# Geunwoo-Jeon/LarvaNet

Hardware: AMD Instinct MI355X
Metric: HR Mpixels/s (LarvaNet x4 multi-exit train step, 48x48 LR patches) (higher is better)
Workload: dtype f32; 1 GPU; LarvaNet x4 train_step_larva M4 B4,4,4,4 48ch, batch 16 of 3x48x48 -> 3x192x192 fp32 per GPU (BASELINE config 2); global_batch=16, parallelism=dp1, hip_graph=True

## Files before the change

### include/larva_hip.h

```cpp
#ifndef LARVA_HIP_H
#define LARVA_HIP_H

#include <stdint.h>

#ifdef __cplusplus
extern "C" {
#endif

int larva_abi_version(void);
const char* larva_error_string(int code);

long long larva_packed_weight_floats(int cout, int cin);
int larva_pack_weights(const float* w, float* wpk_fwd, float* wpk_bwd, int cout, int cin,
                       int w_cin_total, int w_cin_off, void* stream);

int larva_pack_weights_batch(const float* const* w, float* const* wpk_fwd, float* const* wpk_bwd,
                             const int* cout, const int* cin, const int* w_cin_total,
                             const int* w_cin_off, int njobs, void* stream);

int larva_step_prologue(const float* const* w, float* const* wpk_fwd, float* const* wpk_bwd, const int* cout,
                        const int* cin, const int* w_cin_total, const int* w_cin_off, int njobs, const float* x,
                        float* x16, float* base, int N, int C, int H, int W, void* stream);

int larva_conv3x3_fwd(const float* const* src, int n_src, int cin_per_src, const float* wpk,
                      const float* bias, const float* res0, const float* res1, const float* mask,
                      const float* base, float* out, int N, int cout, int H, int W, int relu,
                      int mode, void* stream);

int larva_conv3x3_fwd_pitched(const float* const* src, int n_src, int cin_per_src, const float* wpk,
                              const float* bias, const float* res0, const float* res1, const float* mask,
                              const float* base, float* out, int N, int cout, int H, int W, int pitch,
                              int relu, int mode, void* stream);

int larva_conv3x3_fwd_batch(int njobs, const float* const* src, int n_src, int cin_per_src,
                            const float* const* wpk, const float* const* bias, const float* const* res0,
                            const float* const* res1, const float* const* mask, const float* const* base,
                            float* const* out, int N, int cout, int H, int W, int pitch, int relu, int mode,
                            void* stream);

int larva_head_conv3_direct(const float* x, const float* w, const float* bias, float* out, int N, int cout,
                            int H, int W, int pitch, void* stream);

int larva_exit_l1_partials(int N, int H, int pitch);
int larva_conv3x3_exit_l1_batch(int njobs, const float* const* src, int n_src, int cin_per_src,
                                const float* const* wpk, const float* const* bias, const float* const* base,
                                const float* const* truth, float* const* out, float* const* grad,
                                float* const* partial, float gval, int N, int cout, int H, int W, int pitch,
                                void* stream);

int larva_strip_tile_table(int H, int W, int phase, unsigned* tab, int cap);
int larva_conv3x3_fwd_strips(const float* const* src, int n_src, int cin_per_src, const float* wpk,
                             const float* bias, const float* res0, const float* res1, const float* mask,
                             const float* base, float* out, int N, int cout, int H, int W, int pitch,
                             int relu, int mode, const unsigned* tile_tab, const unsigned* tile_tab_host,
                             int tiles_per_image, int plain_stores, void* stream);

int larva_conv3x3_fwd_tiled(const float* const* src, int n_src, int cin_per_src, const float* wpk,
                            const float* bias, const float* res0, const float* res1, const float* mask,
                            const float* base, float* out, int N, int cout, int H, int W, int pitch,
                            int relu, int mode, int tile_rows, void* stream);

long long larva_wgrad_partial_floats(int cout, int cin, int splits);
int larva_wgrad_cu_share(int cout, int cin);
int larva_conv3x3_wgrad(const float* const* dy, const float* const* x, float* const* partial,
                        float* const* dw, float* const* db, const int* cin_off,
                        const int* cin_valid, const int* w_cin_total, int njobs, int splits,
                        int N, int cout, int cin, int H, int W, void* stream);

int larva_wgrad_flat_max_splits(int njobs, int nwg, int tiles_per_layer);
int larva_conv3x3_wgrad_partial_flat(const float* const* dy, const float* const* x, float* const* partial,
                                     int njobs, int nwg, int N, int cout, int cin, int H, int W,
                                     int* splits_out, void* stream);
int larva_wgrad_flat_head_splits(int njobs, int nwg, int tiles_per_layer);
int larva_conv3x3_wgrad_partial_flat_head(const float* const* dy, const float* const* x, float* const* partial,
                                          int njobs, const float* head_dy, const float* head_x16, float* head_partial,
                                          int nwg, int N, int H, int W, int* splits_out, int* head_splits_out,
                                          void* stream);

int larva_conv3x3_wgrad_partial(const float* const* dy, const float* const* x, float* const* partial,
                                int njobs, int splits, int N, int cout, int cin, int H, int W,
                                int* splits_used, void* stream);
int larva_wgrad_reduce(const float* const* partial, float* const* dw, float* const* db,
                       const int* cin_off, const int* cin_valid, const int* w_cin_total,
                       const int* splits, const int* cout, const int* cin, int njobs, void* stream);

int larva_wgrad_reduce_with_loss(const float* const* partial, float* const* dw, float* const* db,
                                 const int* cin_off, const int* cin_valid, const int* w_cin_total,
                                 const int* splits, const int* cout, const int* cin, int njobs,
                                 const float* const* terms, const int* count, const float* scale, int nterms,
                                 float divisor, float* loss_out, void* stream);

int larva_bicubic4_fwd(const float* in, float* out, int N, int C, int H, int W, void* stream);
int larva_upsample4_fwd(const float* in, float* out, int N, int C, int H, int W, int mode, void* stream);

int larva_l1_workspace_floats(void);
int larva_l1_fwd(const float* a, const float* b, long long numel, float* partial, float* loss,
                 void* stream);
int larva_l1_bwd(const float* a, const float* b, const float* gout, long long numel, float* ga,
                 void* stream);
int larva_l1_bwd_unshuffle4(const float* a, const float* b, const float* gout, float gscale, float* ga, int N,
                            int C, int H, int W, void* stream);
int larva_sum_scalars(const float* const* terms, int n, float divisor, float* out, void* stream);
int larva_l1_partial(const float* a, const float* b, long long numel, float* partial, int* blocks_out,
                     void* stream);
int larva_loss_from_partials(const float* const* terms, const int* count, const float* scale, int n,
                             float divisor, float* out, void* stream);
int larva_loss_from_partials_to_host(const float* const* terms, const int* count, const float* scale, int n,
                                     float divisor, float* out, float* host_cell, void* stream);
int larva_loss_from_partials_to_host_seq(const float* const* terms, const int* count, const float* scale, int n,
                                         float divisor, float* out, float* host_cell, unsigned* dev_seq, void* stream);
int larva_host_cell_alloc(float** cell);
int larva_host_cell_free(float* cell);
int larva_l1_partial_grad(const float* a, const float* b, float gvalue, float gscale, float* partial,
                          int* blocks_out, float* grad, int N, int C, int H, int W, void* stream);
int larva_l1_partial_grad_batch(const float* const* a, const float* b, int n, float gvalue, float gscale,
                                float* const* partial, int* blocks_out, float* const* grad, int N, int C, int H,
                                int W, void* stream);

int larva_pixel_unshuffle4(const float* in, float* out, int N, int C, int H, int W, void* stream);

int larva_upsample_fwd(const float* in, float* out, int N, int C, int H, int W, int scale, int mode, void* stream);
int larva_pixel_shuffle_base(const float* y, const float* base, float* out, int N, int C, int cpad, int H, int W,
                             int pitch, int scale, void* stream);
int larva_pixel_unshuffle(const float* in, float* out, int N, int C, int cpad, int H, int W, int scale, void* stream);
int larva_l1_bwd_unshuffle(const float* a, const float* b, const float* gout, float gscale, float* ga, int N, int C,
                           int cpad, int H, int W, int scale, void* stream);
int larva_shuffle_l1_partial_grad(const float* y, const float* base, const float* truth, float gvalue, float gscale,
                                  float* partial, int* blocks_out, float* grad, float* out, int N, int C, int cpad, int H,
                                  int W, int scale, void* stream);

int larva_adamw_step(float* p, const float* g, float* m, float* v, const float* step_lr,
                     double beta1, double beta2, double eps, double weight_decay, float grad_scale,
                     long long n, void* stream);

int larva_adamw_step_host(float* p, const float* g, float* m, float* v, int step, double lr, double beta1,
                          double beta2, double eps, double weight_decay, float grad_scale, long long n,
                          void* stream);
int larva_adamw_step_host_copy(float* p, const float* g, float* m, float* v, int step, double lr, double beta1,
                               double beta2, double eps, double weight_decay, float grad_scale, long long n,
                               const float* copy_src, float* copy_dst, void* stream);

int larva_gather_patches(const unsigned char* data, const long long* offsets, const int* hw,
                         const int* draws, float* out, int B, int P, int mult, void* stream);

int larva_sqerr_u8(const float* out, const unsigned char* truth, int C, int H, int W, int TH, int TW,
                   unsigned long long* acc, void* stream);

int larva_u8_hwc_to_f32_chw(const unsigned char* in, float* out, int N, int H, int W, void* stream);
int larva_f32_chw_to_u8_hwc(const float* in, unsigned char* out, int N, int H, int W, void* stream);

long long larva_u8_metrics_workspace_bytes(int h, int w, int mode);
int larva_u8_metrics(const unsigned char* out, long long out_pitch, const unsigned char* truth, long long truth_pitch,
                     int y0, int x0, int h, int w, int mode, int want_ssim, void* workspace,
                     unsigned long long* result, void* stream);

long long larva_f16_packed_weight_halves(int cout, int cin);
int larva_f16_pack_weights(const float* w, uint16_t* wpk, int cout, int cin, void* stream);

int larva_f16_head(const float* x, const float* w, const float* bias, uint16_t* out, unsigned* flag, int N, int H,
                   int W, void* stream);

int larva_f16_conv3x3(const uint16_t* const* srcs, int nsrc, const uint16_t* wpk, const float* bias,
                      const uint16_t* res0, const uint16_t* res1, int relu, uint16_t* out, unsigned* flag, int N, int H,
                      int W, void* stream);

int larva_f16_conv3x3_shuffle_base(const uint16_t* src, const uint16_t* wpk, const float* bias, const float* base,
                                   float* out, int N, int H, int W, void* stream);

int larva_f16_conv3x3_shuffle_base_u8(const uint16_t* src, const uint16_t* wpk, const float* bias, const float* base,
                                      unsigned char* out, unsigned* flag, int N, int H, int W, void* stream);

int larva_dihedral_inputs_u8(const unsigned char* in, float* a, float* b, int N, int H, int W, void* stream);
int larva_dihedral_inputs_f32(const float* in, float* a, float* b, int N, int H, int W, void* stream);
int larva_dihedral_mean(const float* a, const float* b, float* out_f32, unsigned char* out_u8, int N, int H, int W,
                        void* stream);

#ifdef __cplusplus
}
#endif
#endif
```

### larvanet_amd/autograd.py

```python
import contextlib
import os

import numpy as np
import torch

from . import kernels as K

_WGRAD_WORKGROUPS = 256


class PaddedWidth:

    current = None

    def __init__(self, w):
        self.w = int(w)

    def __enter__(self):
        self._prev = PaddedWidth.current
        PaddedWidth.current = self.w
        return self

    def __exit__(self, *exc):
        PaddedWidth.current = self._prev
# ... 266 lines not shown
    def intact(self, module=None):
        return all(p.grad is view for p, view in self._pairs)

    def span(self, tensors):
        base = self.flat.data_ptr()
        lo, hi = self.flat.numel(), 0
        for t in tensors:
            off = (t.data_ptr() - base) // 4
            if off < 0 or off + t.numel() > self.flat.numel():
                return None
            lo, hi = min(lo, off), max(hi, off + t.numel())
        return (lo, hi) if hi > lo else None


def _targets(pc):
    if pc is not None and pc.grad_inplace and pc.weight.grad is not None and pc.bias.grad is not None:
        return pc.weight.grad, pc.bias.grad
    return None, None


def _splits(njobs, cout=48, cin=48):
    return max(1, _WGRAD_WORKGROUPS * K.wgrad_cu_share(cout, cin) // njobs)


class DeferredWgrad:

    active = False
    jobs_per_launch = 32
    _pending = {}

    @classmethod
    def push(cls, cout, cin, jobs):
        cls._pending.setdefault((cout, cin), []).extend(jobs)

    _late = []

    @classmethod
    def _launches(cls, split=False):
        pending, cls._pending = cls._pending, {}
        cap = max(1, min(cls.jobs_per_launch, K.max_wgrad_jobs())) if split else K.max_wgrad_jobs()
        out = []
        for (cout, cin), jobs in pending.items():
            jobs = sorted(jobs, key=lambda j: -j["dw"].data_ptr())
            out += [(cout, cin, jobs[i:i + cap]) for i in range(0, len(jobs), cap)]
        out.sort(key=lambda l: -max(j["dw"].data_ptr() for j in l[2]))
        return out

    pending_loss = None

    @classmethod
    def finish_loss(cls):
        job, cls.pending_loss = cls.pending_loss, None
        if job is not None:
            terms, scales, divisor, out = job
            out.copy_(K.loss_from_partials(terms, scales, divisor))

    @staticmethod
    def _issue(launches):
        reduce_jobs = []
        head = host = None
        heads = [l for l in launches if (l[0], l[1]) == (48, 16) and len(l[2]) == 1]
        hosts = [l for l in launches if (l[0], l[1]) == (48, 48)]
        if len(heads) == 1 and hosts and hosts[-1][2][0]["dy"].shape == heads[0][2][0]["dy"].shape:
            head, host = heads[0], hosts[-1]
        todo = [l for l in launches if l is not head]
        for launch in todo:
            cout, cin, chunk = launch
            extra = head[2][0] if launch is host else None
            res = K.conv3x3_wgrad_partial_flat(chunk, cout, cin, _WGRAD_WORKGROUPS, head=extra)
            if res is None and extra is not None:
                todo.append(head)
                extra = None
            if res is not None:
                reduce_jobs += [dict(j, partial=p, splits=s, cout=cout, cin=cin) for j, p, s in zip(chunk, *res)]
                if extra is not None:
                    reduce_jobs.append(dict(extra, partial=res[0][-1], splits=res[1][-1], cout=48, cin=16))
                continue
            parts, used = K.conv3x3_wgrad_partial(chunk, cout, cin, _splits(len(chunk), cout, cin))
            reduce_jobs += [dict(j, partial=p, splits=used, cout=cout, cin=cin) for j, p in zip(chunk, parts)]
        for i in range(0, len(reduce_jobs), 64):
            last = i + 64 >= len(reduce_jobs)
            loss, DeferredWgrad.pending_loss = (DeferredWgrad.pending_loss, None) if last else (None, DeferredWgrad.pending_loss)
            K.wgrad_reduce(reduce_jobs[i:i + 64], loss=loss)

    @classmethod
    def flush(cls, split=False):
        launches = cls._launches(split)
        n_early = max(1, len(launches) // 2) if split else len(launches)
        cls._issue(launches[:n_early])
        cls._late = launches[n_early:]
        if not split:
            return None
        return [t for _, _, chunk in launches[:n_early] for j in chunk for t in (j["dw"], j["db"]) if t is not None]

    @classmethod
    def has_late(cls):
        return bool(cls._late)

    @classmethod
    def late_targets(cls):
        return [t for _, _, chunk in cls._late for j in chunk for t in (j["dw"], j["db"]) if t is not None]

    @classmethod
    def flush_late(cls):
        late, cls._late = cls._late, []
        cls._issue(late)

    @classmethod
    def drop(cls):
        cls._pending = {}
        cls._late = []
        cls.pending_loss = None


class StepScope:

    depth = 0
    _padded = {}
    seed_grad = None
    early_loss = False

    @classmethod
    def padded_input(cls, shape, device):
        if cls.depth == 0:
            return torch.zeros(shape, device=device, dtype=torch.float32)
        key = (tuple(shape), str(device))
        buf = cls._padded.get(key)
        if buf is None:
            buf = cls._padded[key] = torch.zeros(shape, device=device, dtype=torch.float32)
        return buf

    def __init__(self, defer_wgrad=True, split_flush=False, joint_input_grads=True,
                 seed_grad=None, dual_chain=False, lazy_chain_joins=(False, False), early_loss=False):
        self.seed_grad_value = seed_grad
        self.early_loss_value = early_loss or False
        self.dual_chain = dual_chain
        self.lazy_chain_joins = lazy_chain_joins
        self.defer_wgrad = defer_wgrad
        self.split_flush = split_flush
        self.joint_input_grads = joint_input_grads
        self.early_targets = None

    def __enter__(self):
        gpu = torch.cuda.is_available()
        DeferredWgrad.active = bool(self.defer_wgrad) and gpu
        DeferredWgrad.drop()
        JointInputGrad.active = bool(self.joint_input_grads) and gpu
        JointInputGrad.reset()
        DualChain.enabled = bool(self.dual_chain) and gpu
        DualChain.lazy_fwd, DualChain.lazy_bwd = (bool(v) and DualChain.enabled for v in self.lazy_chain_joins)
        StepScope.depth += 1
        StepScope.seed_grad = self.seed_grad_value
        StepScope.early_loss = self.early_loss_value
        return self

    def __exit__(self, exc_type, *exc):
        try:
            DualChain.join()
            if exc_type is None:
                self.early_targets = DeferredWgrad.flush(split=self.split_flush)
                DeferredWgrad.finish_loss()
            else:
                DeferredWgrad.drop()
            if exc_type is None and JointInputGrad._parked:
                raise RuntimeError("larvanet_amd: an exit parked its input gradient but the next body never ran backward")
        finally:
            DualChain.reset()
            StepScope.depth -= 1
            StepScope.seed_grad = None
            StepScope.early_loss = False
            DeferredWgrad._pending = {}
            DualChain.enabled = DualChain.lazy_fwd = DualChain.lazy_bwd = False
            DeferredWgrad.active = False
            JointInputGrad.active = False
            JointInputGrad.reset()
        return False


def _wgrad(jobs, cout, cin, inplace=False):
    defer = inplace and DeferredWgrad.active
    out, batch = [], []
    for job in jobs:
        (dy, x, wshape, cin_off, cin_valid, dw_shared) = job[:6]
        db_shared = job[6] if len(job) > 6 else None
        dw = dw_shared if dw_shared is not None else torch.empty(wshape, device=dy.device, dtype=torch.float32)
        if db_shared is not None or not defer:
            db = db_shared if db_shared is not None else torch.empty((cout,), device=dy.device,
                                                                     dtype=torch.float32)
        else:
            db = None
        batch.append({"dy": dy, "x": x, "dw": dw, "db": db, "cin_off": cin_off, "cin_valid": cin_valid})
        out.append((dw, db))
    if defer:
        DeferredWgrad.push(cout, cin, batch)
        batch = []
    for i in range(0, len(batch), 16):
        chunk = batch[i:i + 16]
        K.conv3x3_wgrad(chunk, cout, cin, _splits(len(chunk), cout, cin))
    return out


LARGE_INFERENCE_PIXELS = 100000


def is_large_inference(n, h, w):
    return int(n) * int(h) * int(w) > LARGE_INFERENCE_PIXELS


def _head_direct_setting():
    v = os.environ.get("LARVA_HEAD_DIRECT", "auto")
    if v not in ("auto", "0", "1"):
        raise RuntimeError("larvanet_amd: LARVA_HEAD_DIRECT=%r (auto, 0 or 1)" % v)
    return {"0": False, "1": True}.get(v, "auto")


class HeadFn(torch.autograd.Function):

    direct = _head_direct_setting()
    rule_batch = None

    @staticmethod
    @contextlib.contextmanager
    def rule_batch_as(n):
        before, HeadFn.rule_batch = HeadFn.rule_batch, int(n)
        try:
            yield
        finally:
            HeadFn.rule_batch = before

    @staticmethod
    def forward(ctx, x, weight, bias, pc, x16=None, training=True):
        N, C, H, W = x.shape
        P = PaddedWidth.pitch_of(W) if _lw() is not None else W
        cout = int(weight.shape[0])
        training = bool(training) and bool(ctx.needs_input_grad[1] or ctx.needs_input_grad[2])
        want = HeadFn.direct if HeadFn.direct != "auto" else (not training and is_large_inference(HeadFn.rule_batch or N, H, W))
        use_direct = want and C == 3 and cout % 16 == 0
        if x16 is not None:
            pass
        elif training or not use_direct:
            x16 = StepScope.padded_input((N, 16, H, P), x.device)
            x16[:, :C, :, :W] = x
        if use_direct:
            out = K.head_conv3_direct(x, weight.detach(), bias.detach(), pitch=P)
        else:
            (fwd, _), = pc.get()
            out = DualChain.conv(x16, fwd, cout, forward=True, bias=bias.detach(), logical_w=_lw())
            DualChain.end_of_node(False)
        if x16 is not None:
            ctx.save_for_backward(x16)
        ctx.wshape = tuple(weight.shape)
        ctx.pc = pc
        return out

    @staticmethod
    def backward(ctx, dy):
        (x16,) = ctx.saved_tensors
        dy = dy.contiguous()
        cout, cin = ctx.wshape[0], ctx.wshape[1]
        tw, tb = _targets(ctx.pc)
        if not (tw is not None and DeferredWgrad.active):
            DualChain.join()
        (dw, db), = _wgrad([(dy, x16, ctx.wshape, 0, cin, tw, tb)], cout, 16, inplace=tw is not None)
        if tw is not None:
            return None, None, None, None, None, None
        return None, dw, db, None, None, None


class BodyFn(torch.autograd.Function):

    @staticmethod
    def forward(ctx, x, pcs, *params):
        nb = len(params) // 4
        keep = [x]
        fea = x
        for j in range(nb):
            w1, b1, w2, b2 = params[4 * j:4 * j + 4]
            (f1, _), = pcs[2 * j].get()
            (f2, _), = pcs[2 * j + 1].get()
            c = int(w1.shape[0])
            h = DualChain.conv(fea, f1, c, forward=True, bias=b1.detach(), relu=True, logical_w=_lw())
            if j == nb - 1:
                nxt = DualChain.conv(h, f2, c, forward=True, bias=b2.detach(), res0=fea, res1=x, logical_w=_lw())
            else:
                nxt = DualChain.conv(h, f2, c, forward=True, bias=b2.detach(), res0=fea, logical_w=_lw())
            keep.append(h)
            if j < nb - 1:
                keep.append(nxt)
            fea = nxt
        DualChain.end_of_node(False)
        ctx.save_for_backward(*keep)
        ctx.pcs = pcs
        ctx.nb = nb
        ctx.wshape = tuple(params[0].shape)
        return fea

    @staticmethod
    def backward(ctx, dy):
        nb, pcs = ctx.nb, ctx.pcs
        keep = ctx.saved_tensors[:2 * nb]
        dy = dy.contiguous()
        c = ctx.wshape[0]
        g = dy
        jobs = [None] * (2 * nb)
        dx = None
        for j in reversed(range(nb)):
            fea_j = keep[0] if j == 0 else keep[2 * j]
            h_j = keep[2 * j + 1]
            (_, bw1), = pcs[2 * j].get()
            (_, bw2), = pcs[2 * j + 1].get()
            dh = DualChain.conv(g, bw2, c, mask=h_j)
            jobs[2 * j + 1] = (g, h_j, ctx.wshape, 0, c) + _targets(pcs[2 * j + 1])
            jobs[2 * j] = (dh, fea_j, ctx.wshape, 0, c) + _targets(pcs[2 * j])
            if j > 0:
                g = DualChain.conv(dh, bw1, c, res0=g)
            else:
                dh_leg = JointInputGrad.take(keep[0], pcs[0])
                if dh_leg is None:
                    dx = DualChain.conv(dh, bw1, c, res0=g, res1=dy)
                else:
                    dx = DualChain.conv([dh, dh_leg], pcs[0].joint.arena(dh.device), c, res0=g, res1=dy)
        inplace = all(_targets(pc)[0] is not None for pc in pcs)
        if not (inplace and DeferredWgrad.active):
            DualChain.join()
        DualChain.end_of_node(True)
        grads = _wgrad(jobs, c, c, inplace=inplace)
        flat = []
        for pc, (dw, db) in zip(pcs, grads):
            flat += [None, None] if _targets(pc)[0] is not None else [dw, db]
        return (dx, None) + tuple(flat)


def _leg_forward(fea, base, pcs, params, scale, lw=None):
    w1, b1, w2, b2 = params
    (f1, _), = pcs[0].get()
    (f2, _), = pcs[1].get()
    h = K.conv3x3(fea, f1, int(w1.shape[0]), bias=b1.detach(), relu=True, logical_w=lw)
    if scale == 4:
        return h, K.conv3x3(h, f2, int(w2.shape[0]), bias=b2.detach(), shuffle=True, base=base, logical_w=lw)
    return h, K.conv3x3(h, f2, pcs[1].cout_pad, bias=pcs[1].padded_bias(), logical_w=lw)


def _leg_backward(ctx, fea, h, dyl):
    pcs = ctx.pcs
    c = ctx.wshape[0]
    (_, bw1), = pcs[0].get()
    (_, bw2), = pcs[1].get()
    dh = K.conv3x3(dyl, bw2, c, mask=h)
    dfea = K.conv3x3(dh, bw1, c)
    first = [(dh, fea, ctx.wshape, 0, c) + _targets(pcs[0])]
    if ctx.scale == 4:
        ((dw1, db1),), ((dw2, db2),) = _leg_wgrad(first, [(dyl, h, ctx.wshape2, 0, c) + _targets(pcs[1])], c, ctx.wshape2[0])
        if _targets(pcs[1])[0] is not None:
            dw2 = db2 = None
    else:
        ((dw1, db1),) = _wgrad(first, c, c, inplace=_targets(pcs[0])[0] is not None)
        dw2, db2 = padded_wgrad(dyl, h, pcs[1], ctx.wshape2)
    if _targets(pcs[0])[0] is not None:
        dw1 = db1 = None
    return dfea, dw1, db1, dw2, db2


def _leg_wgrad(first, second, c, c2):
    inplace = all(j[5] is not None for j in list(first) + list(second))
    if c2 == c:
        res = _wgrad([j for pair in zip(first, second) for j in pair], c, c, inplace=inplace)
        return res[0::2], res[1::2]
    return _wgrad(list(first), c, c, inplace=inplace), _wgrad(list(second), c2, c, inplace=inplace)


def padded_wgrad(dyl, h, pc, wshape):
    cp, cin, rows = pc.cout_pad, int(wshape[1]), int(wshape[0])
    dw = torch.empty((cp,) + tuple(wshape[1:]), device=dyl.device, dtype=torch.float32)
    db = torch.empty((cp,), device=dyl.device, dtype=torch.float32)
    K.conv3x3_wgrad([{"dy": dyl, "x": h, "dw": dw, "db": db, "cin_off": 0, "cin_valid": cin}], cp, cin,
                    _splits(1, cp, cin))
    tw, tb = _targets(pc)
    if tw is None:
        return dw[:rows], db[:rows]
    tw.copy_(dw[:rows])
    tb.copy_(db[:rows])
    return None, None


class LegFn(torch.autograd.Function):

    @staticmethod
    def forward(ctx, fea, base, pcs, scale, w1, b1, w2, b2):
        h, y = _leg_forward(fea, base, pcs, (w1, b1, w2, b2), scale, _lw())
        out = y if scale == 4 else K.pixel_shuffle_base(y, base, scale, logical_w=_lw())
        ctx.save_for_backward(fea, h)
        ctx.pcs, ctx.scale = pcs, scale
        ctx.wshape, ctx.wshape2 = tuple(w1.shape), tuple(w2.shape)
        return out

    @staticmethod
    def backward(ctx, dout):
        fea, h = ctx.saved_tensors
        dout = dout.contiguous()
        dyl = K.pixel_unshuffle4(dout) if ctx.scale == 4 else K.pixel_unshuffle(dout, ctx.scale, ctx.pcs[1].cout_pad)
        dfea, *dparams = _leg_backward(ctx, fea, h, dyl)
        return (dfea, None, None, None) + tuple(dparams)


class ExitFn(torch.autograd.Function):

    @staticmethod
    def forward(ctx, fea, base, truth, pcs, scale, divisor, w1, b1, w2, b2):
        h, y = _leg_forward(fea, base, pcs, (w1, b1, w2, b2), scale)
        ctx.gscale = 1.0 if divisor is None else float(np.float32(1.0) / np.float32(divisor))
        dyl = None
        fused = divisor is not None and StepScope.seed_grad is not None
        if scale == 4:
            out = y
            if fused:
                term, _, dyl = K.l1_partial_grad(out, truth, StepScope.seed_grad, ctx.gscale)
        elif fused:
            term, _, dyl, out = K.shuffle_l1_partial_grad(y, base, truth, StepScope.seed_grad, ctx.gscale, scale)
        else:
            out = K.pixel_shuffle_base(y, base, scale)
        if dyl is None:
            term = K.l1_fwd(out, truth) if divisor is None else K.l1_partial(out, truth)[0]
        ctx.have_dyl = dyl is not None
        ctx.save_for_backward(fea, h, *((dyl,) if dyl is not None else (out, truth)))
        ctx.pcs, ctx.scale = pcs, scale
        ctx.wshape, ctx.wshape2 = tuple(w1.shape), tuple(w2.shape)
        ctx.mark_non_differentiable(out)
        ctx.set_materialize_grads(False)
        return out, term

    @staticmethod
    def backward(ctx, _dout, gterm):
        if gterm is None:
            return (None,) * 10
        saved = ctx.saved_tensors
        fea, h = saved[:2]
        if ctx.have_dyl:
            dyl = saved[2]
        else:
            g0 = gterm.as_strided((), ()) if gterm.dim() else gterm.contiguous()
            out, truth = saved[2:4]
            dyl = K.l1_bwd_unshuffle4(out, truth, g0, ctx.gscale) if ctx.scale == 4 else \
                K.l1_bwd_unshuffle(out, truth, g0, ctx.scale, ctx.pcs[1].cout_pad, ctx.gscale)
        dfea, *dparams = _leg_backward(ctx, fea, h, dyl)
        return (dfea, None, None, None, None, None) + tuple(dparams)


def _conv_group(jobs, cout, **kw):
    outs = []
    for i in range(0, len(jobs), 4):
        chunk = jobs[i:i + 4]
        if len(chunk) == 1:
            j = chunk[0]
            outs.append(K.conv3x3(j["srcs"], j["wpk"], cout, bias=j.get("bias"), mask=j.get("mask"), base=j.get("base"),
                                  res0=j.get("res0"), res1=j.get("res1"), **kw))
        else:
            outs += K.conv3x3_batch(chunk, cout, **kw)
    return outs


class ExitsFn(torch.autograd.Function):

    @staticmethod
    def forward(ctx, base, truth, legs, divisor, *args):
        M = len(legs)
        feas, params = args[:M], args[M:]
        c = int(params[0].shape[0])
        c2 = int(params[2].shape[0])
        hs = _conv_group([{"srcs": feas[i], "wpk": legs[i][0].get()[0][0], "bias": params[4 * i + 1].detach()}
                          for i in range(M)], c, relu=True)
        ctx.gscale = float(np.float32(1.0) / np.float32(divisor))
        ctx.have_dyl = StepScope.seed_grad is not None
        shuffle_jobs = [{"srcs": hs[i], "wpk": legs[i][1].get()[0][0], "bias": params[4 * i + 3].detach(), "base": base}
                        for i in range(M)]
        outs, parts, third = [None] * M, [None] * M, [None] * M
        fused = ctx.have_dyl
        if fused:
            i = 0
            while i < M and fused:
                n = 3 if M - i == 5 else min(4, M - i)
                res = K.conv3x3_exit_l1_batch(shuffle_jobs[i:i + n], c2, truth, StepScope.seed_grad, ctx.gscale,
                                              [i + k == M - 1 for k in range(n)]) if n > 1 else None
                if res is None:
                    fused = False
                else:
                    outs[i:i + n], parts[i:i + n], third[i:i + n] = res
                    i += n
        if not fused:
            outs = _conv_group(shuffle_jobs, c2, shuffle=True)
            parts, third = [], []
            if ctx.have_dyl:
                for i in range(0, M, 8):
                    p8, _, g8 = K.l1_partial_grad_batch(outs[i:i + 8], truth, StepScope.seed_grad, ctx.gscale)
                    parts += p8
                    third += g8
            else:
                for out in outs:
                    part, _ = K.l1_partial(out, truth)
                    parts.append(part)
                    third.append(out)
        ctx.save_for_backward(truth, *feas, *hs, *third)
        ctx.legs, ctx.M = legs, M
        ctx.wshape, ctx.wshape2 = tuple(params[0].shape), tuple(params[2].shape)
        ctx.mark_non_differentiable(outs[-1])
        ctx.set_materialize_grads(False)
        return (outs[-1],) + tuple(parts)

    @staticmethod
    def backward(ctx, _dout, *gterms):
        M, legs = ctx.M, ctx.legs
        saved = ctx.saved_tensors
        truth, feas, hs, third = saved[0], saved[1:1 + M], saved[1 + M:1 + 2 * M], saved[1 + 2 * M:1 + 3 * M]
        c = ctx.wshape[0]
        live = [i for i in range(M) if gterms[i] is not None]
        dyls = {}
        for i in live:
            if ctx.have_dyl:
                dyls[i] = third[i]
            else:
                g0 = gterms[i].as_strided((), ())
                dyls[i] = K.l1_bwd_unshuffle4(third[i], truth, g0, ctx.gscale)
        dhs = dict(zip(live, _conv_group([{"srcs": dyls[i], "wpk": legs[i][1].get()[0][1], "mask": hs[i]} for i in live], c))) if live else {}
        dfeas = [None] * M
        grads = [None] * (4 * M)
        jobs1, jobs2 = [], []
        for i in live:
            pc1, pc2 = legs[i]
            if JointInputGrad.can_park(pc1):
                JointInputGrad.park(feas[i], dhs[i], pc1)
            else:
                dfeas[i] = DualChain.conv(dhs[i], pc1.get()[0][1], c)
            jobs1.append((dhs[i], feas[i], ctx.wshape, 0, c) + _targets(pc1))
            jobs2.append((dyls[i], hs[i], ctx.wshape2, 0, c) + _targets(pc2))
        DualChain.end_of_node(True)
        for which, res in enumerate(_leg_wgrad(jobs1, jobs2, c, ctx.wshape2[0]) if jobs1 else ()):
            for i, (dw, db) in zip(live, res):
                if _targets(legs[i][which])[0] is None:
                    grads[4 * i + 2 * which], grads[4 * i + 2 * which + 1] = dw, db
        return (None, None, None, None) + tuple(dfeas) + tuple(grads)


class LossTerm:

    __slots__ = ("tensor", "scale", "prescaled")

    def __init__(self, tensor, scale=1.0, prescaled=False):
        self.tensor, self.scale, self.prescaled = tensor, float(scale), bool(prescaled)


class MeanTermsFn(torch.autograd.Function):

    @staticmethod
    def forward(ctx, meta, *tensors):
        ctx.meta = meta
        ctx.shapes = [tuple(t.shape) for t in tensors]
        ts, scales = [t.contiguous() for t in tensors], [m[0] for m in meta]
        if (len(ts) <= 8 and DeferredWgrad.active and StepScope.depth > 0 and not StepScope.early_loss
                and DeferredWgrad.pending_loss is None):
            out = torch.empty((), device=ts[0].device, dtype=torch.float32)
            DeferredWgrad.pending_loss = (ts, scales, float(len(ts)), out)
            return out
        cell = StepScope.early_loss if isinstance(StepScope.early_loss, K.HostCell) else None
        if len(ts) <= 8:
            return K.loss_from_partials(ts, scales, float(len(ts)), host_cell=cell)
        groups = [K.loss_from_partials(ts[i:i + 8], scales[i:i + 8], 1.0) for i in range(0, len(ts), 8)]
        return K.loss_from_partials(groups, [1.0] * len(groups), float(len(ts)), host_cell=cell)

    @staticmethod
    def backward(ctx, g):
        n = len(ctx.meta)
        gm = None
        grads = []
        for (scale, prescaled), shape in zip(ctx.meta, ctx.shapes):
            if prescaled:
                grads.append(g.expand(shape))
            else:
                gm = g / n if gm is None else gm
                grads.append(gm if scale == 1.0 else gm * scale)
        return (None,) + tuple(grads)


def mean_of_terms(terms):
    terms = [t if isinstance(t, LossTerm) else LossTerm(t) for t in terms]
    return MeanTermsFn.apply([(t.scale, t.prescaled) for t in terms], *[t.tensor for t in terms])


class MergeFn(torch.autograd.Function):

    @staticmethod
    def forward(ctx, pc, weight, bias, *feats):
        packs = pc.get()
        cout = int(weight.shape[0])
        out = K.conv3x3(list(feats), packs[0][0], cout, bias=bias.detach(), logical_w=_lw())
        ctx.save_for_backward(*feats)
        ctx.pc = pc
        ctx.wshape = tuple(weight.shape)
        return out

    @staticmethod
    def backward(ctx, dy):
        feats = ctx.saved_tensors
        packs = ctx.pc.get()
        dy = dy.contiguous()
        cout = ctx.wshape[0]
        c = int(feats[0].shape[1])
        dfeats = [K.conv3x3(dy, packs[1 + i][1], c) for i in range(len(feats))]
        tw, tb = _targets(ctx.pc)
        dw = tw if tw is not None else torch.empty(ctx.wshape, device=dy.device, dtype=torch.float32)
        jobs = [(dy, f, ctx.wshape, i * c, c, dw, tb if i == 0 else None) for i, f in enumerate(feats)]
        res = _wgrad(jobs, cout, c, inplace=tw is not None)
        db = res[0][1]
        if tw is not None:
            return (None, None, None) + tuple(dfeats)
        return (None, dw, db) + tuple(dfeats)


class L1LossFn(torch.autograd.Function):

    @staticmethod
    def forward(ctx, out, truth):
        out = out.contiguous()
        truth = truth.contiguous()
        ctx.save_for_backward(out, truth)
        return K.l1_fwd(out, truth)

    @staticmethod
    def backward(ctx, g):
        out, truth = ctx.saved_tensors
        return K.l1_bwd(out, truth, g.contiguous()), None
```

### larvanet_amd/captured_step.py

```python
import contextlib

import torch

from .autograd import DeferredWgrad, DualChain


class LossCopy:

    def __init__(self):
        self.host = torch.empty((), dtype=torch.float32).pin_memory()
        self.stream = torch.cuda.Stream()
        self.done, self.fwd_done = torch.cuda.Event(), torch.cuda.Event()

    def start(self, loss):
        self.fwd_done.record()
        with torch.cuda.stream(self.stream):
            self.stream.wait_event(self.fwd_done)
            self.host.copy_(loss, non_blocking=True)
            self.done.record()

    def result(self):
        self.done.synchronize()
        return self.host.item()


class CapturedStep:

    def __init__(self, plugin, key, mode, handoff, input_tensor, truth_tensor):
        x, truth = input_tensor.clone(), truth_tensor.clone()
        side = torch.cuda.Stream()
        side.wait_stream(torch.cuda.current_stream())
        with torch.cuda.stream(side):
            for _ in range(2):
                plugin._zero_grad()
                plugin._step_body(x, truth)
                DeferredWgrad.flush_late()
        torch.cuda.current_stream().wait_stream(side)
        plugin._zero_grad()
        graph = torch.cuda.CUDAGraph()
        back = torch.cuda.CUDAGraph() if mode == "split" else None
        with contextlib.ExitStack() as capturing:
            capturing.enter_context(torch.cuda.graph(graph, capture_error_mode="thread_local"))

            def cut():
                DualChain.join()
                capturing.close()
                capturing.enter_context(torch.cuda.graph(back, pool=graph.pool(), capture_error_mode="thread_local"))
            loss, out, early_lo = plugin._step_body(x, truth, early_loss=handoff if mode == "poll" else bool(mode),
                                                    cut=cut if back is not None else None)
        late = None
        if DeferredWgrad.has_late():
            late = torch.cuda.CUDAGraph()
            with torch.cuda.graph(late, pool=graph.pool(), capture_error_mode="thread_local"):
                DeferredWgrad.flush_late()
        self.key, self.mode, self.handoff = key, mode, handoff
        self.static_in, self.static_truth = x, truth
        self.graph, self.back, self.late = graph, back, late
        self.loss, self.out, self.early_lo = loss, out, early_lo

    def stage(self, input_tensor, truth_tensor):
        for dst, src in ((self.static_in, input_tensor), (self.static_truth, truth_tensor)):
            if src.data_ptr() != dst.data_ptr():
                dst.copy_(src)

    def replay(self):
        if self.mode == "poll":
            self.handoff.expect()
        self.graph.replay()
        if self.back is not None:
            self.handoff.start(self.loss)
            self.back.replay()
        return self.loss, self.out, self.late.replay if self.late is not None else None

    def buffers(self, input_shape, truth_shape):
        fits = tuple(self.static_in.shape) == tuple(input_shape) and tuple(self.static_truth.shape) == tuple(truth_shape)
        return (self.static_in, self.static_truth) if fits else None
```

### larvanet_amd/csrc/conv3x3_mfma.hip

```cpp
#include "larva_common.h"
#include "larva_bicubic.h"
#include <hip/hip_ext.h>
#include <cstdlib>
#include <type_traits>

#ifndef LARVA_DIAG
#define LARVA_DIAG 0
#endif
constexpr int kWgPerCu = 2;
constexpr int kOperandDepth = 2;


#ifndef LARVA_DIAG_ONLY48
#define LARVA_DIAG_ONLY48 0
#endif

namespace larva {

#if defined(LARVA_DIAG) && (LARVA_DIAG & 32)
__device__ unsigned long long* g_stamps = nullptr;
#if LARVA_DIAG & 512
constexpr int kDiagWgPerSlot = 256;
__device__ int g_slot_of_launch = 0;
__device__ __forceinline__ void stamp_slot(unsigned long long* area, int k) {
  if (!area || threadIdx.x != 0 || blockIdx.x >= kDiagWgPerSlot) return;
  const int idx = k == 0 ? 0 : k == 2 ? 1 : k == 3 ? 2 : k == 5 ? 3
                  : !(LARVA_DIAG & 2048) ? -1 : k == 6 ? 5 : k == 7 ? 6 : k == 14 ? 7 : k == 15 ? 8 : k == 1 ? 9 : -1;
  if (idx < 0) return;
  unsigned long long* p = area + (size_t)blockIdx.x * 16;
  p[idx] = __builtin_amdgcn_s_memrealtime();
  if (k == 0) {
    const unsigned hw = __builtin_amdgcn_s_getreg((31 << 11) | 4);
    const unsigned xcc = __builtin_amdgcn_s_getreg((31 << 11) | 20);
    p[4] = (unsigned long long)hw | ((unsigned long long)xcc << 32);
  }
}
#define stamp(k) stamp_slot(a.diag_area, (k))
#else
__device__ __forceinline__ void stamp(int k) {
  if (g_stamps && threadIdx.x == 0)
    g_stamps[blockIdx.x * 16 + k] = (LARVA_DIAG & 64) ? __builtin_amdgcn_s_memtime() : __builtin_amdgcn_s_memrealtime();
}
#endif
#else
__device__ __forceinline__ void stamp(int) {}
#endif

constexpr int kCh = 8;

template <int ROWS_, int COLS_>
struct TileGeo {
  static constexpr int ROWS = ROWS_, COLS = COLS_;
  static constexpr int HALO = ROWS + 2;
  static constexpr int PC = COLS / 16;
  static constexpr int RS = COLS + 8;
  static constexpr int PS = ((HALO * RS + 15) / 32) * 32 + 16;
  static_assert(COLS % 16 == 0 && PS >= HALO * RS && PS % 32 == 16, "tile geometry");
};
using GeoWide = TileGeo<kTileRows, kTileCols>;
using GeoWide4 = TileGeo<4, kTileCols>;
using GeoS5 = TileGeo<5, 16>;
using GeoS4 = TileGeo<4, 16>;
static_assert(GeoWide::RS == kRS && GeoWide::PS == 304, "the 3 x 48 tile of larva_common.h");

struct ConvArgs {
  const float* src[kMaxSrc];
  const float* wpk;
  const float* bias;
  const float* res0;
  const float* res1;
  const float* mask;
  const float* base;
  float* out;
  int cin_per_src;
  int n_chunks;
  int N, H, W;
  int pitch;
  int tiles_x, tiles_y;
  int nwg;
  const unsigned* tile_tab;
  const float* truth;
  float* grad;
  float* partial;
  int plain_stores;
  int tab_n;
  alignas(64) int tab16[32];
  float gval;
  unsigned long long magic_tx, magic_ty, magic_cps;
#if LARVA_DIAG & 512
  unsigned long long* diag_area;
#endif
};

__host__ __device__ __forceinline__ unsigned long long div_magic(int d) { return ((1ull << 40) + d - 1) / (unsigned)d; }
__device__ __forceinline__ int div_by_magic(int n, unsigned long long magic) {
  return (int)(((unsigned long long)(unsigned)n * magic) >> 40);
}

enum Epi : int {
  kEpiPlain = 0,
  kEpiRelu = 1,
  kEpiMask = 2,
  kEpiRes1 = 3,
  kEpiRes2 = 4,
  kEpiShuffle = 5,
  kEpiShuffleBase = 6,
  kEpiShuffleL1 = 7,
  kEpiCount = 8
};

template <int COUT, typename G = GeoWide>
struct ConvCfg {
  static constexpr int CT = COUT / 16;
  static constexpr int CS = cout_stride(COUT);
  static constexpr int PS = G::PS;
  static constexpr int IN_PIECES = (kCh * PS + 255) / 256;
  static constexpr int IN_FLOATS = IN_PIECES * 256;
  static constexpr int IN_SLOTS_PER_PLANE = PS / 4;
  static constexpr int W_USED = 9 * kCh * CS;
  static constexpr int W_PIECES = (W_USED + 255) / 256;
  static constexpr int W_FLOATS = W_PIECES * 256;
  static constexpr int PIECES = IN_PIECES + W_PIECES;
  static constexpr int NPW = (PIECES + 3) / 4;
  static constexpr int STAGE_FLOATS = IN_FLOATS + W_FLOATS;
  static constexpr int STEPS = 9 * (kCh / 4);
  static constexpr int NST = 3;
  static constexpr int AHEAD = NST - 1;
  static constexpr size_t LDS_BYTES_DMA = NST * STAGE_FLOATS * sizeof(float);
  static constexpr bool LOADER = 2 * PIECES <= 63;
  static constexpr int THREADS_DMA = LOADER ? 320 : 256;
  static constexpr size_t LDS_BYTES_REG = 2 * STAGE_FLOATS * sizeof(float);
  static constexpr int RIN_SLOTS = kCh * G::HALO * (G::RS / 4);
  static constexpr int RIN_ITERS = (RIN_SLOTS + 255) / 256;
  static constexpr int RW_SLOTS = W_USED / 4;
  static constexpr int RW_ITERS = (RW_SLOTS + 255) / 256;
  static_assert(kCh * PS <= IN_FLOATS, "input planes must fit their pieces");
};

template <int COUT, typename G>
struct DmaPlan {
  unsigned voff[ConvCfg<COUT, G>::NPW];
};

template <int COUT, typename G, bool WEIGHTS>
__device__ __forceinline__ void make_plan(const ConvArgs& a, int wave, int lane, int y0, int x0,
                                          DmaPlan<COUT, G>& pl) {
  using C = ConvCfg<COUT, G>;
#pragma unroll
  for (int i = 0; i < C::NPW; ++i) {
    const int p = min(wave + 4 * i, C::PIECES - 1);
    const bool isw = p >= C::IN_PIECES;
    if constexpr (WEIGHTS) {
      if (4 * i + 3 < C::IN_PIECES) continue;
      const int ws = (p - C::IN_PIECES) * 64 + lane;
// ... 90 lines not shown
    const int nstage = (stage + C::AHEAD) % C::NST;
    const unsigned dst = lds_addr_of(smem + nstage * C::STAGE_FLOATS);
    const ChunkSrc cs = chunk_src<COUT, G>(a, min(chunk + C::AHEAD, last), n);
#pragma unroll
    for (int p = 0; p < C::PIECES; ++p)
      lds_dma16_buf(p < C::IN_PIECES ? cs.img : cs.wgt, pl.voff[p], 0, dst + 1024u * (unsigned)p);
    stage = stage == C::NST - 1 ? 0 : stage + 1;
  }
  asm volatile("s_waitcnt vmcnt(0)" ::: "memory");
}

template <int COUT, typename G>
struct RegStaging {
  f32x4 in[ConvCfg<COUT, G>::RIN_ITERS];
  f32x4 w[ConvCfg<COUT, G>::RW_ITERS];
};

template <int COUT, typename G>
__device__ __forceinline__ void reg_load(const ConvArgs& a, const ChunkSrc& cs, int y0, int x0, int tid,
                                         RegStaging<COUT, G>& st) {
  using C = ConvCfg<COUT, G>;
  const size_t plane = (size_t)a.H * a.pitch;
#pragma unroll
  for (int i = 0; i < C::RIN_ITERS; ++i) {
    const int s = min(tid + i * 256, C::RIN_SLOTS - 1);
    const int ci = s / (G::HALO * (G::RS / 4));
    const int rem = s - ci * (G::HALO * (G::RS / 4));
    const int r = rem / (G::RS / 4);
    const int q = rem - r * (G::RS / 4);
    const int gy = y0 - 1 + r, gx = x0 - 4 + 4 * q;
    const bool row_ok = gy >= 0 && gy < a.H;
    const float* row = cs.img_ptr + (size_t)ci * plane + (size_t)min(max(gy, 0), a.H - 1) * a.pitch;
    f32x4 v;
#pragma unroll
    for (int e = 0; e < 4; ++e) {
      const int x = gx + e;
      const float t = row[min(max(x, 0), a.W - 1)];
      v[e] = (row_ok && x >= 0 && x < a.W) ? t : 0.f;
    }
    st.in[i] = v;
  }
#pragma unroll
  for (int i = 0; i < C::RW_ITERS; ++i) {
    const int s = min(tid + i * 256, C::RW_SLOTS - 1);
    const float* p = cs.wgt_ptr + 4 * s;
    st.w[i] = f32x4{p[0], p[1], p[2], p[3]};
  }
}

template <int COUT, typename G>
__device__ __forceinline__ void reg_store(float* stage, int tid, const RegStaging<COUT, G>& st) {
  using C = ConvCfg<COUT, G>;
#pragma unroll
  for (int i = 0; i < C::RIN_ITERS; ++i) {
    const int s = tid + i * 256;
    if (s < C::RIN_SLOTS) {
      const int ci = s / (G::HALO * (G::RS / 4));
      const int rem = s - ci * (G::HALO * (G::RS / 4));
      const int r = rem / (G::RS / 4);
      const int q = rem - r * (G::RS / 4);
      *reinterpret_cast<f32x4*>(stage + ci * C::PS + r * G::RS + 4 * q) = st.in[i];
    }
  }
#pragma unroll
  for (int i = 0; i < C::RW_ITERS; ++i) {
    const int s = tid + i * 256;
    if (s < C::RW_SLOTS) *reinterpret_cast<f32x4*>(stage + C::IN_FLOATS + 4 * s) = st.w[i];
  }
}

template <int COUT, typename G, int NCT, int PG0, int NPG>
__device__ __forceinline__ void read_operands(const float* const (&a_base)[NCT], const float* b_base, int step,
                                              float (&av)[NCT], float (&bv)[NPG]) {
  using C = ConvCfg<COUT, G>;
  if constexpr ((LARVA_DIAG & 128) != 0) {
#pragma unroll
    for (int c = 0; c < NCT; ++c) av[c] = (float)step;
#pragma unroll
    for (int p = 0; p < NPG; ++p) bv[p] = (float)(step + p);
    return;
  }
  const int tap = step / (kCh / 4), kk = step % (kCh / 4);
  const int ky = tap / 3, kx = tap % 3;
#pragma unroll
  for (int c = 0; c < NCT; ++c) av[c] = a_base[c][(tap * kCh + kk * 4) * C::CS];
#pragma unroll
  for (int p = 0; p < NPG; ++p) {
    const int pg = PG0 + p, prow = pg / G::PC, pcol = pg % G::PC;
    bv[p] = b_base[kk * 4 * C::PS + (prow + ky) * G::RS + pcol * 16 + kx];
  }
}

template <int NMF, int NRD, int M>
__device__ __forceinline__ void shadow_groups() {
  if constexpr (M < NMF) {
    __builtin_amdgcn_sched_group_barrier(0x8, 1, 0);
    constexpr int share = (NRD + NMF - 1 - M) / NMF;
    if constexpr (share > 0) __builtin_amdgcn_sched_group_barrier(0x100, share, 0);
    shadow_groups<NMF, NRD, M + 1>();
  }
}

template <int COUT, typename G, int NCT, int PG0, int NPG, bool SWAP>
__device__ __forceinline__ void mfma_chunk(const float* stage, int ct0, int lane, f32x4 (&acc)[NCT][NPG],
                                           const float* wstage = nullptr) {
  using C = ConvCfg<COUT, G>;
  const int lr = lane & 15, lq = lane >> 4;
  const float* const wrows = wstage ? wstage : stage + C::IN_FLOATS;
  const float* a_base[NCT];
#pragma unroll
  for (int c = 0; c < NCT; ++c)
    a_base[c] = wrows + lq * C::CS + lr + (cout_swizzled(COUT) ? (((ct0 + c) ^ (lq & 1)) * 16) : (ct0 + c) * 16);
  const float* b_base = stage + lq * C::PS + lr + 3;
  constexpr int D = kOperandDepth;
  float av[D + 1][NCT], bv[D + 1][NPG];
#pragma unroll
  for (int d = 0; d < D; ++d)
    if (d < C::STEPS) read_operands<COUT, G, NCT, PG0, NPG>(a_base, b_base, d, av[d], bv[d]);
#pragma unroll
  for (int step = 0; step < C::STEPS; ++step) {
    __builtin_amdgcn_sched_barrier(0);
    if (step + D < C::STEPS)
      read_operands<COUT, G, NCT, PG0, NPG>(a_base, b_base, step + D, av[(step + D) % (D + 1)], bv[(step + D) % (D + 1)]);
    constexpr int NMF = NCT * NPG;
    constexpr int NRD = NCT + NPG;
#pragma unroll
    for (int m = 0; m < NMF; ++m) {
      const float wv = av[step % (D + 1)][m / NPG], xv = bv[step % (D + 1)][m % NPG];
      acc[m / NPG][m % NPG] = __builtin_amdgcn_mfma_f32_16x16x4f32(SWAP ? xv : wv, SWAP ? wv : xv, acc[m / NPG][m % NPG], 0, 0, 0);
    }
    shadow_groups<NMF, NRD, 0>();
    __builtin_amdgcn_sched_barrier(0);
  }
}

template <int KEEP, int PIECES, int AUX>
__device__ __forceinline__ void wait_and_barrier() {
  static_assert(KEEP == PIECES + AUX, "a ring wait keeps exactly the next chunk's pieces and the operand loads in flight");
  asm volatile("; LARVA_RING pieces=%1 aux=%2\n\ts_waitcnt vmcnt(%0)\n\ts_barrier" ::"n"(KEEP), "n"(PIECES), "n"(AUX) : "memory");
  __builtin_amdgcn_sched_barrier(0);
}

template <typename G>
__device__ __forceinline__ void decode_tile(const ConvArgs& a, int vb, int& n, int& y0, int& x0) {
  const int tile = xcd_remap(vb, a.nwg);
  const int t2 = div_by_magic(tile, a.magic_tx);
  const int tx = tile - t2 * a.tiles_x;
  n = div_by_magic(t2, a.magic_ty);
  const int ty = t2 - n * a.tiles_y;
  x0 = tx * G::COLS;
  y0 = ty * G::ROWS;
}

template <int COUT, typename G, bool VEC, int EPI, int NCT, int PG0, int NPG, bool PERSIST = false>
__device__ __forceinline__ void run_role(const ConvArgs& a, float* smem, int ct0, int wave, int n, int y0, int x0, int tid) {
  using C = ConvCfg<COUT, G>;
  static_assert(!VEC || C::LOADER, "the 16-byte path runs with a loader wave (2 * PIECES <= 63 for every instantiated shape)");
  static_assert(!PERSIST || VEC, "persistent tiles: the loader-wave path");
  const int lane = tid & 63;
  const int lr = lane & 15, lq = lane >> 4;
  float* const out_ptr = a.out;
  struct { int H, W, pitch, plain; } k = {a.H, a.W, a.pitch, a.plain_stores};
  asm volatile("" : "+s"(k.H), "+s"(k.W), "+s"(k.pitch), "+s"(k.plain));

  constexpr bool kShuffleEpi = (EPI == kEpiShuffle || EPI == kEpiShuffleBase || EPI == kEpiShuffleL1);
  constexpr bool kPixMajor = VEC && !kShuffleEpi;
  f32x4 bias[NCT];
#pragma unroll
  for (int c = 0; c < NCT; ++c) bias[c] = f32x4{0.f, 0.f, 0.f, 0.f};
  auto load_bias = [&]() {
    if (a.bias) {
#pragma unroll
      for (int c = 0; c < NCT; ++c)
#pragma unroll
        for (int r = 0; r < 4; ++r) bias[c][r] = a.bias[(ct0 + c) * 16 + (kPixMajor ? lr : lq * 4 + r)];
    }
  };

  constexpr int NAUX = (EPI == kEpiMask || EPI == kEpiRes1 || EPI == kEpiShuffleBase)
                           ? 1 : ((EPI == kEpiRes2 || EPI == kEpiShuffleL1) ? 2 : 0);
  f32x4 aux[NAUX > 0 ? NAUX : 1][NAUX > 0 ? NCT : 1][NAUX > 0 ? NPG : 1];
  constexpr int NU = NCT * NPG;
  constexpr int kEarlyPairs = PERSIST && COUT == 48 ? (NAUX * NU < 7 ? NAUX * NU : 7) : NAUX * NU;
  constexpr int kLatePart = 4, kEarlyAll = 5;
  auto load_aux = [&](int part = -1) {
#pragma unroll
    for (int c = 0; c < NCT; ++c)
#pragma unroll
      for (int p = 0; p < NPG; ++p) {
        const int pg = PG0 + p, prow = pg / G::PC, pcol = pg % G::PC;
        const int y = min(y0 + prow, a.H - 1), x = min(x0 + pcol * 16 + lr, a.W - 1);
        auto want = [&](int op) {
          const int q = op * NU + c * NPG + p;
          return part < 0 ? true : part == kLatePart ? q >= kEarlyPairs : q < kEarlyPairs;
        };
        if constexpr (kShuffleEpi) {
          const int HH = 4 * a.H, WW = 4 * a.W;
          const size_t idx = (((size_t)n * C::CT + (ct0 + c)) * HH + (4 * y + lq)) * WW + 4 * x;
          if (want(0)) aux[0][c][p] = *reinterpret_cast<const f32x4*>(a.base + idx);
          if constexpr (EPI == kEpiShuffleL1) {
            if (want(1)) aux[1][c][p] = *reinterpret_cast<const f32x4*>(a.truth + idx);
          }
        } else if constexpr (kPixMajor && (PERSIST || G::COLS == 16)) {
          const unsigned plane = (unsigned)a.H * (unsigned)a.pitch;
          const unsigned lane_off = 4u * ((unsigned)lr * plane + (unsigned)lq * 4u);
          const int soff = __builtin_amdgcn_readfirstlane(
              (int)(4u * ((unsigned)((ct0 + c) * 16) * plane + (unsigned)(y0 + prow) * (unsigned)a.pitch + (unsigned)(x0 + pcol * 16))));
          auto image = [&](const float* t) {
            const unsigned long long b = reinterpret_cast<unsigned long long>(t + (size_t)n * COUT * plane);
            const unsigned lo = (unsigned)__builtin_amdgcn_readfirstlane((int)(unsigned)b);
            const unsigned hi = (unsigned)__builtin_amdgcn_readfirstlane((int)(unsigned)(b >> 32));
            return __builtin_amdgcn_make_buffer_rsrc(reinterpret_cast<void*>(((unsigned long long)hi << 32) | lo), 0,
                                                     (int)(COUT * plane * 4u), 0x00020000);
          };
          if constexpr (EPI == kEpiMask) {
            if (want(0)) aux[0][c][p] = __builtin_bit_cast(f32x4, __builtin_amdgcn_raw_buffer_load_b128(image(a.mask), lane_off, soff, 0));
          }
          if constexpr (EPI == kEpiRes1 || EPI == kEpiRes2) {
            if (want(0)) aux[0][c][p] = __builtin_bit_cast(f32x4, __builtin_amdgcn_raw_buffer_load_b128(image(a.res0), lane_off, soff, 0));
          }
          if constexpr (EPI == kEpiRes2) {
            if (want(1)) aux[1][c][p] = __builtin_bit_cast(f32x4, __builtin_amdgcn_raw_buffer_load_b128(image(a.res1), lane_off, soff, 0));
          }
        } else if constexpr (kPixMajor) {
          const size_t plane = (size_t)a.H * a.pitch;
          const int xb = min(x0 + pcol * 16 + lq * 4, a.pitch - 4);
          const size_t idx = ((size_t)n * COUT + (ct0 + c) * 16 + lr) * plane + (size_t)y * a.pitch + xb;
          if constexpr (EPI == kEpiMask) {
            if (want(0)) aux[0][c][p] = *reinterpret_cast<const f32x4*>(a.mask + idx);
          }
          if constexpr (EPI == kEpiRes1 || EPI == kEpiRes2) {
            if (want(0)) aux[0][c][p] = *reinterpret_cast<const f32x4*>(a.res0 + idx);
          }
          if constexpr (EPI == kEpiRes2) {
            if (want(1)) aux[1][c][p] = *reinterpret_cast<const f32x4*>(a.res1 + idx);
          }
        } else {
          const size_t plane = (size_t)a.H * a.pitch;
          const size_t idx0 = ((size_t)n * COUT + (ct0 + c) * 16 + lq * 4) * plane + (size_t)y * a.pitch + x;
#pragma unroll
          for (int r = 0; r < 4; ++r) {
            if constexpr (EPI == kEpiMask) aux[0][c][p][r] = a.mask[idx0 + r * plane];
            if constexpr (EPI == kEpiRes1 || EPI == kEpiRes2) aux[0][c][p][r] = a.res0[idx0 + r * plane];
            if constexpr (EPI == kEpiRes2) aux[1][c][p][r] = a.res1[idx0 + r * plane];
          }
        }
      }
  };
  constexpr bool kAuxLate = VEC && !kShuffleEpi && !(LARVA_DIAG & 6) && NAUX > 0 && !PERSIST;
  constexpr int kAuxLoads = kAuxLate ? NAUX * NCT * NPG : 0;
  auto load_early = [&]() {
    load_bias();
    if constexpr (NAUX > 0 && !kAuxLate && !(LARVA_DIAG & 4)) load_aux();
  };
  int pstage = 0;
  for (int vb = blockIdx.x;; vb += gridDim.x) {
  if constexpr (PERSIST) {
    if (vb >= a.nwg) break;
    decode_tile<G>(a, vb, n, y0, x0);
  }
  if constexpr (!VEC || (LARVA_DIAG & 2)) load_early();

  f32x4 acc[NCT][NPG];
#pragma unroll
  for (int c = 0; c < NCT; ++c)
#pragma unroll
    for (int p = 0; p < NPG; ++p) acc[c][p] = f32x4{0.f, 0.f, 0.f, 0.f};

  if constexpr (PERSIST) {
    load_bias();
    const int my_chunk = a.n_chunks >= 4 ? (wave & 3) : 0;
    __builtin_amdgcn_sched_barrier(0);
    for (int chunk = 0; chunk < a.n_chunks; ++chunk) {
      asm volatile("s_barrier" ::: "memory");
      __builtin_amdgcn_sched_barrier(0);
      if constexpr (NAUX > 0) {
        if (chunk == my_chunk) load_aux(kEarlyAll);
        __builtin_amdgcn_sched_barrier(0);
      }
      mfma_chunk<COUT, G, NCT, PG0, NPG, kPixMajor>(smem + pstage * C::STAGE_FLOATS, ct0, lane, acc);
      pstage = pstage == C::NST - 1 ? 0 : pstage + 1;
    }
    asm volatile("s_waitcnt vmcnt(0)" ::: "memory");
    __builtin_amdgcn_sched_barrier(0);
    if constexpr (kEarlyPairs < NAUX * NU) {
      load_aux(kLatePart);
      __builtin_amdgcn_sched_barrier(0);
    }
  } else if constexpr (VEC) {
    DmaPlan<COUT, G> pl;
    const int last = a.n_chunks - 1;
    if constexpr (!(LARVA_DIAG & 2)) {
      const ChunkSrc cs0 = chunk_src<COUT, G>(a, 0, n);
      const unsigned st0 = lds_addr_of(smem), st1 = lds_addr_of(smem + C::STAGE_FLOATS);
      stamp(6);
      make_plan<COUT, G, true>(a, wave, lane, y0, x0, pl);
#pragma unroll
      for (int i = 0; i < C::NPW; ++i)
        if (wave + 4 * i >= C::IN_PIECES) dma_piece<COUT, G>(pl, i, wave, cs0, st0);
      __builtin_amdgcn_sched_barrier(0);
      stamp(7);
      load_early();
      stamp(14);
      make_plan<COUT, G, false>(a, wave, lane, y0, x0, pl);
#pragma unroll
      for (int i = 0; i < C::NPW; ++i)
        if (wave + 4 * i < C::IN_PIECES) dma_piece<COUT, G>(pl, i, wave, cs0, st0);
      stamp(15);
      const ChunkSrc cs1 = chunk_src<COUT, G>(a, min(1, last), n);
#pragma unroll
      for (int i = 0; i < C::NPW; ++i) dma_piece<COUT, G>(pl, i, wave, cs1, st1);
      if constexpr (kAuxLate) {
        __builtin_amdgcn_sched_barrier(0);
        load_aux();
        __builtin_amdgcn_sched_barrier(0);
      }
    }
    stamp(1);
    int stage = 0;
    for (int chunk = 0; chunk <= last; ++chunk) {
      if constexpr ((LARVA_DIAG & 256) != 0) {
      } else if (chunk == 0) wait_and_barrier<((LARVA_DIAG & 2) ? 0 : C::NPW) + kAuxLoads, ((LARVA_DIAG & 2) ? 0 : C::NPW), kAuxLoads>();
      else wait_and_barrier<kAuxLoads, 0, kAuxLoads>();
      if (chunk == 0) stamp(2);
      stamp(8 + (chunk < 7 ? chunk : 7));
      if constexpr (!(LARVA_DIAG & 1)) mfma_chunk<COUT, G, NCT, PG0, NPG, kPixMajor>(smem + stage * C::STAGE_FLOATS, ct0, lane, acc);
      stage = stage == C::NST - 1 ? 0 : stage + 1;
    }
    asm volatile("s_waitcnt vmcnt(0)" ::: "memory");
    stamp(3);
  } else {
    RegStaging<COUT, G> st;
    if constexpr (!(LARVA_DIAG & 2)) {
      reg_load<COUT, G>(a, chunk_src<COUT, G>(a, 0, n), y0, x0, tid, st);
      reg_store<COUT, G>(smem, tid, st);
    }
    __syncthreads();
    for (int chunk = 0; chunk < a.n_chunks; ++chunk) {
      float* cur = smem + (chunk & 1) * C::STAGE_FLOATS;
      float* nxt = smem + ((chunk & 1) ^ 1) * C::STAGE_FLOATS;
      const bool more = chunk + 1 < a.n_chunks;
      if constexpr (!(LARVA_DIAG & 2)) {
        if (more) reg_load<COUT, G>(a, chunk_src<COUT, G>(a, chunk + 1, n), y0, x0, tid, st);
      }
      if constexpr (!(LARVA_DIAG & 1)) mfma_chunk<COUT, G, NCT, PG0, NPG, kPixMajor>(cur, ct0, lane, acc);
      if constexpr (!(LARVA_DIAG & 2)) {
        if (more) reg_store<COUT, G>(nxt, tid, st);
      }
      __syncthreads();
    }
  }

  if constexpr ((LARVA_DIAG & 4) != 0) {
#pragma unroll
    for (int c = 0; c < NCT; ++c)
#pragma unroll
      for (int p = 0; p < NPG; ++p) asm volatile("" ::"v"(acc[c][p]));
    return;
  }

  if constexpr (EPI == kEpiShuffleL1) {
    const int HH = 4 * k.H, WW = 4 * k.W;
    const size_t plane = (size_t)k.H * k.pitch;
    const float g = a.gval;
    float s = 0.f;
#pragma unroll
    for (int c = 0; c < NCT; ++c)
#pragma unroll
      for (int p = 0; p < NPG; ++p) {
        const int pg = PG0 + p, prow = pg / G::PC, pcol = pg % G::PC;
        const int y = y0 + prow, x = x0 + pcol * 16 + lr;
        const f32x4 v = (acc[c][p] + bias[c]) + aux[0][c][p];
        if (y < k.H && x < k.W) {
          if (out_ptr) {
            const size_t idx = (((size_t)n * C::CT + (ct0 + c)) * HH + (4 * y + lq)) * WW + 4 * x;
            __builtin_nontemporal_store(v, reinterpret_cast<f32x4*>(out_ptr + idx));
          }
          const f32x4 d = v - aux[1][c][p];
          s += fabsf(d[0]) + fabsf(d[1]) + fabsf(d[2]) + fabsf(d[3]);
          const size_t idx0 = ((size_t)n * COUT + (ct0 + c) * 16 + lq * 4) * plane + (size_t)y * k.pitch + x;
#pragma unroll
          for (int r = 0; r < 4; ++r)
            __builtin_nontemporal_store(d[r] > 0.f ? g : (d[r] < 0.f ? -g : 0.f), &a.grad[idx0 + r * plane]);
        }
      }
#pragma unroll
    for (int o = 32; o > 0; o >>= 1) s += __shfl_xor(s, o);
    if (lane == 0) a.partial[4 * blockIdx.x + wave] = s;
  } else if constexpr (EPI == kEpiShuffle || EPI == kEpiShuffleBase) {
    const int HH = 4 * k.H, WW = 4 * k.W;
#pragma unroll
    for (int c = 0; c < NCT; ++c)
#pragma unroll
      for (int p = 0; p < NPG; ++p) {
        const int pg = PG0 + p, prow = pg / G::PC, pcol = pg % G::PC;
        const int y = y0 + prow, x = x0 + pcol * 16 + lr;
        const size_t idx = (((size_t)n * C::CT + (ct0 + c)) * HH + (4 * y + lq)) * WW + 4 * x;
        f32x4 v = acc[c][p] + bias[c];
        if constexpr (EPI == kEpiShuffleBase) v += aux[0][c][p];
        if (y < k.H && x < k.W) __builtin_nontemporal_store(v, reinterpret_cast<f32x4*>(out_ptr + idx));
      }
  } else if constexpr (kPixMajor) {
    const size_t plane = (size_t)k.H * k.pitch;
    auto store_all = [&](auto plain_tag, auto interior_tag) {
      constexpr bool kPlain = decltype(plain_tag)::value;
      constexpr bool kInterior = decltype(interior_tag)::value;
#pragma unroll
      for (int c = 0; c < NCT; ++c)
#pragma unroll
        for (int p = 0; p < NPG; ++p) {
          const int pg = PG0 + p, prow = pg / G::PC, pcol = pg % G::PC;
          const int y = y0 + prow, xb = x0 + pcol * 16 + lq * 4;
          const size_t idx = ((size_t)n * COUT + (ct0 + c) * 16 + lr) * plane + (size_t)y * k.pitch + xb;
          f32x4 v = acc[c][p] + bias[c];
          if (kInterior || (y < k.H && xb < k.pitch)) {
#pragma unroll
            for (int r = 0; r < 4; ++r) {
              float o = v[r];
              if constexpr (EPI == kEpiRelu) o = fmaxf(o, 0.f);
              if constexpr (EPI == kEpiMask) o = (aux[0][c][p][r] > 0.f) ? o : 0.f;
              if constexpr (EPI == kEpiRes1 || EPI == kEpiRes2) o += aux[0][c][p][r];
              if constexpr (EPI == kEpiRes2) o += aux[1][c][p][r];
              v[r] = (kInterior || xb + r < k.W) ? o : 0.f;
            }
            if constexpr (kPlain) *reinterpret_cast<f32x4*>(out_ptr + idx) = v;
            else __builtin_nontemporal_store(v, reinterpret_cast<f32x4*>(out_ptr + idx));
          }
        }
    };
    constexpr bool kFastPath = EPI == kEpiPlain || EPI == kEpiRelu || EPI == kEpiRes1;
    const bool interior = kFastPath && y0 + G::ROWS <= k.H && x0 + G::COLS <= k.W;
    auto store_policy = [&](auto plain_tag) {
      if constexpr (kFastPath) {
        if (interior) {
          store_all(plain_tag, std::true_type{});
          return;
        }
      }
      store_all(plain_tag, std::false_type{});
    };
    if constexpr ((LARVA_DIAG & 16) != 0) {
      store_policy(std::true_type{});
    } else if constexpr (G::COLS == 16) {
      if (k.plain) store_policy(std::true_type{});
      else store_policy(std::false_type{});
    } else {
      store_policy(std::false_type{});
    }
  } else {
    const size_t plane = (size_t)k.H * k.pitch;
#pragma unroll
    for (int c = 0; c < NCT; ++c)
#pragma unroll
      for (int p = 0; p < NPG; ++p) {
        const int pg = PG0 + p, prow = pg / G::PC, pcol = pg % G::PC;
        const int y = y0 + prow, x = x0 + pcol * 16 + lr;
        const size_t idx0 = ((size_t)n * COUT + (ct0 + c) * 16 + lq * 4) * plane + (size_t)y * k.pitch + x;
        const f32x4 v = acc[c][p] + bias[c];
        if (y < k.H && x < k.pitch) {
          const bool real = x < k.W;
#pragma unroll
          for (int r = 0; r < 4; ++r) {
            float o = v[r];
            if constexpr (EPI == kEpiRelu) o = fmaxf(o, 0.f);
            if constexpr (EPI == kEpiMask) o = (aux[0][c][p][r] > 0.f) ? o : 0.f;
            if constexpr (EPI == kEpiRes1 || EPI == kEpiRes2) o += aux[0][c][p][r];
            if constexpr (EPI == kEpiRes2) o += aux[1][c][p][r];
            o = real ? o : 0.f;
            if constexpr ((LARVA_DIAG & 16) != 0) out_ptr[idx0 + r * plane] = o;
            else __builtin_nontemporal_store(o, &out_ptr[idx0 + r * plane]);
          }
        }
      }
  }
#if LARVA_DIAG & 32
  stamp(4);
  asm volatile("s_waitcnt vmcnt(0)" ::: "memory");
  stamp(5);
#endif
  if constexpr (!PERSIST) break;
  }
}

__device__ __forceinline__ void fetch_args(const ConvArgs& a) {
  asm volatile("" ::"s"(a.src[0]), "s"(a.wpk), "s"(a.bias), "s"(a.out), "s"(a.cin_per_src), "s"(a.n_chunks), "s"(a.N),
               "s"(a.H), "s"(a.W), "s"(a.pitch), "s"(a.tiles_x), "s"(a.tiles_y), "s"(a.magic_tx), "s"(a.magic_ty),
               "s"(a.magic_cps), "s"(a.nwg), "s"(a.tile_tab), "s"(a.plain_stores), "s"(a.tab_n),
               "s"(a.tab16[0]), "s"(a.tab16[16]));
}

template <int COUT, bool VEC, int EPI, typename G = GeoWide>
__device__ __forceinline__ void conv_tile(const ConvArgs& a, float* smem) {
  if constexpr ((LARVA_DIAG & 8) != 0) return;
  stamp(0);
  fetch_args(a);
  const int tile = xcd_remap(blockIdx.x, a.nwg);
  const int t2 = div_by_magic(tile, a.magic_tx);
  const int tx = tile - t2 * a.tiles_x;
  const int n = div_by_magic(t2, a.magic_ty);
  const int ty = t2 - n * a.tiles_y;
  const int x0 = tx * G::COLS, y0 = ty * G::ROWS;
  const int tid = threadIdx.x;
  const int wave = __builtin_amdgcn_readfirstlane(tid >> 6);
  __builtin_amdgcn_s_setprio(1);

  if constexpr (VEC) {
    if (wave == 4) {
      if constexpr (!(LARVA_DIAG & 2)) run_loader<COUT, G>(a, smem, tid & 63, n, y0, x0);
      return;
    }
  }
  if constexpr (G::ROWS == 4) {
    static_assert(VEC && (COUT == 48 || COUT == 32), "4 x 48 tiles: the 16-byte path at 48 / 32 channels");
    if constexpr (COUT == 48) {
      if (wave < 3) run_role<COUT, G, VEC, EPI, 1, 0, 9>(a, smem, wave, wave, n, y0, x0, tid);
      else run_role<COUT, G, VEC, EPI, 3, 9, 3>(a, smem, 0, wave, n, y0, x0, tid);
    } else {
      if (wave < 2) run_role<COUT, G, VEC, EPI, 1, 0, 6>(a, smem, wave, wave, n, y0, x0, tid);
      else run_role<COUT, G, VEC, EPI, 1, 6, 6>(a, smem, wave - 2, wave, n, y0, x0, tid);
    }
  } else if constexpr (COUT == 48) {
    if (wave < 3) run_role<COUT, G, VEC, EPI, 1, 0, 7>(a, smem, wave, wave, n, y0, x0, tid);
    else run_role<COUT, G, VEC, EPI, 3, 7, 2>(a, smem, 0, wave, n, y0, x0, tid);
  } else if constexpr (COUT == 32) {
    if (wave < 2) run_role<COUT, G, VEC, EPI, 1, 0, 5>(a, smem, wave, wave, n, y0, x0, tid);
    else run_role<COUT, G, VEC, EPI, 1, 5, 4>(a, smem, wave - 2, wave, n, y0, x0, tid);
  } else {
    static_assert(COUT == 64, "unsupported channel count");
    run_role<COUT, G, VEC, EPI, 1, 0, 9>(a, smem, wave, wave, n, y0, x0, tid);
  }
}

template <int COUT, bool VEC, int EPI>
__global__ __launch_bounds__(VEC ? ConvCfg<COUT>::THREADS_DMA : 256, VEC ? kWgPerCu : 1) void conv3x3_mfma_kernel(ConvArgs a) {
  extern __shared__ __attribute__((aligned(16))) float smem[];
  conv_tile<COUT, VEC, EPI>(a, smem);
}

template <int COUT, int EPI>
__global__ __launch_bounds__((ConvCfg<COUT, GeoWide4>::THREADS_DMA), kWgPerCu) void conv3x3_mfma_rows4_kernel(ConvArgs a) {
  extern __shared__ __attribute__((aligned(16))) float smem[];
  conv_tile<COUT, true, EPI, GeoWide4>(a, smem);
}
static_assert(2 * ConvCfg<48, GeoWide4>::LDS_BYTES_DMA <= 160 * 1024, "two 4 x 48 workgroups per CU");

template <int COUT, typename G>
__device__ __forceinline__ void run_loader_persist(const ConvArgs& a, float* smem, int lane) {
  using C = ConvCfg<COUT, G>;
  static_assert(C::NST == 3 && 2 * C::PIECES <= 63, "three stages, two chunks in flight");
  LoaderPlan<COUT, G> pl;
  int vb_i = blockIdx.x, n_i, y0, x0, c_i = 0, s_i = 0;
  decode_tile<G>(a, vb_i, n_i, y0, x0);
  make_loader_plan<COUT, G>(a, lane, y0, x0, pl);
  bool more = true;
  auto issue = [&]() {
    const ChunkSrc cs = chunk_src<COUT, G>(a, c_i, n_i);
    const unsigned dst = lds_addr_of(smem + s_i * C::STAGE_FLOATS);
#pragma unroll
    for (int p = 0; p < C::PIECES; ++p)
      lds_dma16_buf(p < C::IN_PIECES ? cs.img : cs.wgt, pl.voff[p], 0, dst + 1024u * (unsigned)p);
    s_i = s_i == C::NST - 1 ? 0 : s_i + 1;
    if (++c_i == a.n_chunks) {
      c_i = 0;
      vb_i += gridDim.x;
      more = vb_i < a.nwg;
      if (more) {
        decode_tile<G>(a, vb_i, n_i, y0, x0);
        make_loader_plan<COUT, G>(a, lane, y0, x0, pl);
      }
    }
  };
  int ahead = 0;
  issue();
  ++ahead;
  if (more) {
    issue();
    ++ahead;
  }
  while (ahead > 0) {
    if (ahead == 2) asm volatile("s_waitcnt vmcnt(%0)" ::"n"(C::PIECES) : "memory");
    else asm volatile("s_waitcnt vmcnt(0)" ::: "memory");
    asm volatile("s_barrier" ::: "memory");
    __builtin_amdgcn_sched_barrier(0);
    --ahead;
    if (more) {
      issue();
      ++ahead;
    }
  }
}

template <int COUT, int EPI>
__global__ __launch_bounds__((ConvCfg<COUT>::THREADS_DMA), kWgPerCu) void conv3x3_mfma_persist_kernel(ConvArgs a) {
  extern __shared__ __attribute__((aligned(16))) float smem[];
  using G = GeoWide;
  stamp(0);
  fetch_args(a);
  const int tid = threadIdx.x;
  const int wave = __builtin_amdgcn_readfirstlane(tid >> 6);
  __builtin_amdgcn_s_setprio(1);
  if (wave == 4) {
    run_loader_persist<COUT, G>(a, smem, tid & 63);
    return;
  }
  if constexpr (COUT == 48) {
    if (wave < 3) run_role<COUT, G, true, EPI, 1, 0, 7, true>(a, smem, wave, wave, 0, 0, 0, tid);
    else run_role<COUT, G, true, EPI, 3, 7, 2, true>(a, smem, 0, wave, 0, 0, 0, tid);
  } else if constexpr (COUT == 32) {
    if (wave < 2) run_role<COUT, G, true, EPI, 1, 0, 5, true>(a, smem, wave, wave, 0, 0, 0, tid);
    else run_role<COUT, G, true, EPI, 1, 5, 4, true>(a, smem, wave - 2, wave, 0, 0, 0, tid);
  } else {
    static_assert(COUT == 64, "unsupported channel count");
    run_role<COUT, G, true, EPI, 1, 0, 9, true>(a, smem, wave, wave, 0, 0, 0, tid);
  }
}

template <int COUT, int EPI, typename G>
__device__ __forceinline__ void strip_roles(const ConvArgs& a, float* smem, int wave, int n, int y0, int x0, int tid) {
  static_assert(ConvCfg<COUT, G>::LOADER, "the strip kernel is launched with a loader wave");
  static_assert(COUT == 48 || COUT == 32 || COUT == 64, "strip tiles: 32, 48 or 64 output channels");
  if (wave == 4) {
    run_loader<COUT, G>(a, smem, tid & 63, n, y0, x0);
    return;
  }
  if constexpr (COUT == 64) {
    run_role<COUT, G, true, EPI, 1, 0, G::ROWS>(a, smem, wave, wave, n, y0, x0, tid);
  } else if constexpr (COUT == 48) {
    if (wave < 3) run_role<COUT, G, true, EPI, 1, 0, G::ROWS - 1>(a, smem, wave, wave, n, y0, x0, tid);
    else run_role<COUT, G, true, EPI, 3, G::ROWS - 1, 1>(a, smem, 0, wave, n, y0, x0, tid);
  } else if constexpr (G::ROWS == 5) {
    if (wave < 2) run_role<COUT, G, true, EPI, 1, 0, 3>(a, smem, wave, wave, n, y0, x0, tid);
    else if (wave == 2) run_role<COUT, G, true, EPI, 2, 3, 1>(a, smem, 0, wave, n, y0, x0, tid);
    else run_role<COUT, G, true, EPI, 2, 4, 1>(a, smem, 0, wave, n, y0, x0, tid);
  } else {
    if (wave < 2) run_role<COUT, G, true, EPI, 1, 0, 2>(a, smem, wave, wave, n, y0, x0, tid);
    else run_role<COUT, G, true, EPI, 1, 2, 2>(a, smem, wave - 2, wave, n, y0, x0, tid);
  }
}

template <int COUT, int EPI>
__global__ __launch_bounds__(320, kWgPerCu) void conv3x3_mfma_strip_kernel(ConvArgs a) {
  extern __shared__ __attribute__((aligned(16))) float smem[];
  stamp(0);
  fetch_args(a);
  const int tile = xcd_remap(blockIdx.x, a.nwg);
  const int n = div_by_magic(tile, a.magic_tx);
  const int slot = tile - n * a.tiles_x;
  unsigned e;
  if (a.tab_n) {
    const unsigned pair = (unsigned)a.tab16[slot >> 1];
    const unsigned h = (slot & 1) ? pair >> 16 : pair & 0xffffu;
    e = (h & 0xffu) | (((h >> 8) & 0x7fu) << 16) | ((h >> 15) << 31);
  } else {
    e = a.tile_tab[slot];
  }
  const int y0 = (int)(e & 0xfffu), x0 = (int)((e >> 12) & 0xfffu);
  const int tid = threadIdx.x;
  const int wave = __builtin_amdgcn_readfirstlane(tid >> 6);
  __builtin_amdgcn_s_setprio(1);
  if (e >> 31) strip_roles<COUT, EPI, GeoS5>(a, smem, wave, n, y0, x0, tid);
  else strip_roles<COUT, EPI, GeoS4>(a, smem, wave, n, y0, x0, tid);
}
template <int COUT>
constexpr size_t kStripLdsBytes = ConvCfg<COUT, GeoS5>::LDS_BYTES_DMA > ConvCfg<COUT, GeoS4>::LDS_BYTES_DMA ? ConvCfg<COUT, GeoS5>::LDS_BYTES_DMA
                                                                                                            : ConvCfg<COUT, GeoS4>::LDS_BYTES_DMA;
static_assert(kWgPerCu * kStripLdsBytes<48> <= 160 * 1024 && kWgPerCu * kStripLdsBytes<64> <= 160 * 1024, "strip workgroups per CU");

constexpr int kMaxConvJobs = 4;
struct ConvBatch {
  ConvArgs job[kMaxConvJobs];
};

template <int COUT, int EPI>
__global__ __launch_bounds__(ConvCfg<COUT>::THREADS_DMA, kWgPerCu) void conv3x3_mfma_batch_kernel(ConvBatch b) {
  extern __shared__ __attribute__((aligned(16))) float smem[];
  conv_tile<COUT, true, EPI>(b.job[blockIdx.y], smem);
}

constexpr int kMaxPackJobs = 64;

struct PackJob {
  const float* w;
  float* fwd;
  float* bwd;
  int cout, cin, w_cin_total, w_cin_off;
};

struct PackBatch {
  PackJob job[kMaxPackJobs];
};

__host__ __device__ constexpr int packed_floats(int cout, int cin) {
  return (cin / kCh) * 9 * kCh * cout_stride(cout);
}

constexpr int kPackTileCols = 64;
constexpr int kPackLd = kPackTileCols + 1;
constexpr int kPackTileFloats = 9 * kCh * kPackLd;

__host__ __device__ constexpr int pack_slots(int cout, int cin) { return cin / kCh + cout / kCh; }

__device__ __forceinline__ void pack_block(const PackJob& j, int slot, float* __restrict__ tile) {
  const int nfc = j.cin / kCh;
  const bool fwd = slot < nfc;
  const int chunk = fwd ? slot : slot - nfc;
  float* __restrict__ out = fwd ? j.fwd : j.bwd;
  if ((!fwd && chunk >= j.cout / kCh) || !out) return;
  const int cols = fwd ? j.cout : j.cin;
  const int cs = cout_stride(cols);
  const int tid = threadIdx.x;
  out += (size_t)chunk * 72 * cs;
  for (int c0 = 0; c0 < cs; c0 += kPackTileCols) {
    const int ncol = min(kPackTileCols, cols - c0);
    if (fwd) {
      for (int idx = tid; idx < ncol * 72; idx += 256) {
        const int c = idx / 72, r = idx - c * 72, k = r / 9, tap = r - k * 9;
        const int cin_abs = j.w_cin_off + chunk * kCh + k;
        tile[(tap * kCh + k) * kPackLd + c] =
            cin_abs < j.w_cin_total ? j.w[((size_t)(c0 + c) * j.w_cin_total + cin_abs) * 9 + tap] : 0.f;
      }
    } else {
      const int row = ncol * 9;
      for (int idx = tid; idx < kCh * row; idx += 256) {
        const int k = idx / row, rem = idx - k * row, c = rem / 9, tap = rem - c * 9;
        tile[((8 - tap) * kCh + k) * kPackLd + c] =
            j.w_cin_off + c0 + c < j.w_cin_total
                ? j.w[((size_t)(chunk * kCh + k) * j.w_cin_total + j.w_cin_off + c0) * 9 + rem] : 0.f;
      }
    }
    __syncthreads();
    const int wcols = min(kPackTileCols, cs - c0);
    const bool swz = cout_swizzled(cols);
    for (int idx = tid; idx < 72 * wcols; idx += 256) {
      const int r = idx / wcols, c = idx - r * wcols;
      const int col = swz ? ((c0 + c) ^ ((r & 1) << 4)) : c0 + c;
      out[r * cs + col] = c < ncol ? tile[r * kPackLd + c] : 0.f;
    }
    __syncthreads();
  }
}

__global__ __launch_bounds__(256) void pack_weights_batch_kernel(PackBatch b) {
  __shared__ float tile[kPackTileFloats];
  pack_block(b.job[blockIdx.y], blockIdx.x, tile);
}

constexpr int kPrologueBlocks = 192;
constexpr int kProloguePadSlices = 2, kPrologueBicSlices = 8;
struct PrologueArgs {
  PackBatch packs;
  int npack, slots;
  const float* x;
  float* x16;
  float* base;
  int N, C, H, W;
};

__global__ __launch_bounds__(256) void step_prologue_kernel(PrologueArgs a) {
  __shared__ float tile[kPackTileFloats];
  int blk = blockIdx.x;
  if (blk < a.npack * a.slots) {
    const int job = blk / a.slots;
    pack_block(a.packs.job[job], blk - job * a.slots, tile);
    return;
  }
  blk -= a.npack * a.slots;
  constexpr int nthr = kPrologueBlocks * 256;
  const int slice = blk / kPrologueBlocks, tid = (blk - slice * kPrologueBlocks) * 256 + threadIdx.x;
  const int nbic = a.base ? kPrologueBicSlices : 0;
  if (slice < nbic) {
    bicubic4_body(a.x, a.base, a.N * a.C, a.H, a.W, (long long)slice * nthr + tid, (long long)nthr * kPrologueBicSlices);
  } else {
    const int plane = a.H * a.W, per_img = a.C * plane, total = a.N * per_img;
    for (int i = (slice - nbic) * nthr + tid; i < total; i += nthr * kProloguePadSlices) {
      const int n = i / per_img, r = i - n * per_img;
      a.x16[(size_t)n * 16 * plane + r] = a.x[i];
    }
  }
}

struct LaunchTiming {
  hipEvent_t start, stop;
};

template <auto Kernel, typename Args>
static hipError_t launch(dim3 grid, dim3 block, size_t lds, hipStream_t stream, const LaunchTiming* tm, const Args& a) {
  static PerDeviceOnce lds_set;
  if (const hipError_t e = ensure_dynamic_lds(lds_set, reinterpret_cast<const void*>(Kernel), lds); e != hipSuccess) return e;
  if (tm)
    hipExtLaunchKernelGGL(Kernel, grid, block, lds, stream, tm->start, tm->stop, 0, a);
  else
    hipLaunchKernelGGL(Kernel, grid, block, lds, stream, a);
  return hipGetLastError();
}

template <int... E>
struct EpiSet {
  static constexpr bool has(int epi) { return ((epi == E) || ...); }
};
using EpiAll = EpiSet<kEpiPlain, kEpiRelu, kEpiMask, kEpiRes1, kEpiRes2, kEpiShuffle, kEpiShuffleBase>;
using EpiBatch48 = EpiSet<kEpiPlain, kEpiRelu, kEpiMask, kEpiRes1, kEpiRes2, kEpiShuffle, kEpiShuffleBase, kEpiShuffleL1>;
using EpiInference = EpiSet<kEpiPlain, kEpiRelu, kEpiRes1, kEpiRes2, kEpiShuffle, kEpiShuffleBase>;
using EpiRows4 = EpiInference;
using EpiPersist = EpiInference;

template <int... E, typename F>
static hipError_t with_epi(EpiSet<E...>, int epi, hipError_t absent, F&& f) {
  hipError_t r = absent;
  (void)((epi == E && (r = f(std::integral_constant<int, E>{}), true)) || ...);
  return r;
}

template <typename F>
static hipError_t with_cout(int cout, hipError_t absent, F&& f) {
  switch (cout) {
#if !LARVA_DIAG_ONLY48
    case 32: return f(std::integral_constant<int, 32>{});
    case 64: return f(std::integral_constant<int, 64>{});
#endif
    case 48: return f(std::integral_constant<int, 48>{});
    default: return absent;
  }
}

static int conv_slots() { return kWgPerCu * device_cu_count(); }

template <int COUT>
static hipError_t launch_conv(const ConvArgs& a, bool vec, int epi, hipStream_t stream, const LaunchTiming* tm) {
  using C = ConvCfg<COUT>;
// ... 118 lines not shown
int larva_diag_next_slot(void) { return g_diag_next_slot; }
#endif

static int conv_build(const float* const* src, int n_src, int cin_per_src, const float* wpk, const float* bias,
                      const float* res0, const float* res1, const float* mask, const float* base, float* out,
                      int N, int H, int W, int pitch, int relu, int mode, ConvArgs& a, bool& aligned, int& epi) {
  if (pitch == 0) pitch = W;
  if (pitch < W) return (int)hipErrorInvalidValue;
  if (n_src < 1 || n_src > kMaxSrc || cin_per_src % kCh || cin_per_src <= 0 || N <= 0 || H <= 0 || W <= 0)
    return (int)hipErrorInvalidValue;
  if (mode != 0 && mode != 1) return (int)hipErrorInvalidValue;
  if ((long long)cin_per_src * H * pitch >= (1ll << 31)) return (int)hipErrorInvalidValue;
  if (!wpk || !out) return (int)hipErrorInvalidValue;
  a = ConvArgs{};
#if LARVA_DIAG & 512
  {
    const int slot = diag_take_slot();
    a.diag_area = (slot >= 0 && g_diag_host_base) ? g_diag_host_base + (size_t)slot * kDiagWgPerSlot * 16 : nullptr;
  }
#endif
  aligned = (pitch % 4 == 0) && ((reinterpret_cast<uintptr_t>(wpk) & 15) == 0);
  for (int i = 0; i < n_src; ++i) {
    if (!src[i]) return (int)hipErrorInvalidValue;
    a.src[i] = src[i];
    aligned = aligned && ((reinterpret_cast<uintptr_t>(src[i]) & 15) == 0);
  }
  aligned = aligned && (((reinterpret_cast<uintptr_t>(out) | reinterpret_cast<uintptr_t>(res0) |
                          reinterpret_cast<uintptr_t>(res1) | reinterpret_cast<uintptr_t>(mask)) & 15) == 0);
  a.wpk = wpk; a.bias = bias; a.res0 = res0; a.res1 = res1; a.mask = mask; a.base = base;
  a.out = out;
  a.cin_per_src = cin_per_src;
  a.n_chunks = n_src * cin_per_src / kCh;
  a.N = N; a.H = H; a.W = W; a.pitch = pitch;
  a.tiles_x = (pitch + kTileCols - 1) / kTileCols;
  a.tiles_y = (H + kTileRows - 1) / kTileRows;
  if ((long long)N * a.tiles_x * a.tiles_y >= (1ll << 20)) return (int)hipErrorInvalidValue;
  a.magic_tx = div_magic(a.tiles_x);
  a.magic_ty = div_magic(a.tiles_y);
  a.magic_cps = div_magic(cin_per_src / kCh);
  a.nwg = N * a.tiles_x * a.tiles_y;
  if (mode == 1) {
    if (relu || mask || res0 || res1) return (int)hipErrorInvalidValue;
    epi = base ? kEpiShuffleBase : kEpiShuffle;
  } else {
    if (base) return (int)hipErrorInvalidValue;
    const int code = (relu ? 1 : 0) | (mask ? 2 : 0) | (res0 ? 4 : 0) | (res1 ? 8 : 0);
    switch (code) {
      case 0: epi = kEpiPlain; break;
      case 1: epi = kEpiRelu; break;
      case 2: epi = kEpiMask; break;
      case 4: epi = kEpiRes1; break;
      case 12: epi = kEpiRes2; break;
      default: return (int)hipErrorInvalidValue;
    }
  }
  return 0;
}

static int conv_tile_rows(int N, int H, int pitch, int cout, int epi, bool aligned, int forced) {
  const bool can4 = aligned && (cout == 48 || cout == 32) && EpiRows4::has(epi);
  if (forced == 3 || !can4) return 3;
  if (forced == 4) return 4;
  const long long tiles3 = (long long)N * ((pitch + kTileCols - 1) / kTileCols) * ((H + 2) / 3);
  return (cout == 32 && tiles3 > conv_slots()) ? 4 : 3;
}

static int conv_dispatch(const float* const* src, int n_src, int cin_per_src, const float* wpk,
                         const float* bias, const float* res0, const float* res1, const float* mask,
                         const float* base, float* out, int N, int cout, int H, int W, int pitch, int relu,
                         int mode, void* stream, const LaunchTiming* tm, int tile_rows = 0) {
  ConvArgs a;
  bool aligned;
  int epi;
  const int rc = conv_build(src, n_src, cin_per_src, wpk, bias, res0, res1, mask, base, out, N, H, W, pitch, relu,
                            mode, a, aligned, epi);
  if (rc) return rc;
  hipStream_t s = (hipStream_t)stream;
  if (tile_rows != 0 && tile_rows != 3 && tile_rows != 4) return (int)hipErrorInvalidValue;
  if (conv_tile_rows(N, H, a.pitch, cout, epi, aligned, tile_rows) == 4) {
    a.tiles_y = (H + 3) / 4;
    a.magic_ty = div_magic(a.tiles_y);
    a.nwg = N * a.tiles_x * a.tiles_y;
    return (int)with_cout(cout, hipErrorInvalidValue, [&](auto c) {
      if constexpr (decltype(c)::value == 64) return hipErrorNotSupported;
      else return launch_rows4<decltype(c)::value>(a, epi, s, tm);
    });
  }
  if (tile_rows == 4) return (int)hipErrorNotSupported;
  const char* pe = getenv("LARVA_PERSIST");
  const bool persist_on = !(pe && pe[0] == '0');
  if (persist_on && aligned && a.nwg > conv_slots()) {
    const hipError_t e = with_cout(cout, hipErrorNotSupported, [&](auto c) {
      return launch_persist<decltype(c)::value>(a, epi, s, tm);
    });
    if (e != hipErrorNotSupported) return (int)e;
  }
  return (int)with_cout(cout, hipErrorInvalidValue, [&](auto c) {
    return launch_conv<decltype(c)::value>(a, aligned, epi, s, tm);
  });
}

int larva_conv3x3_fwd(const float* const* src, int n_src, int cin_per_src, const float* wpk,
                      const float* bias, const float* res0, const float* res1, const float* mask,
                      const float* base, float* out, int N, int cout, int H, int W, int relu,
                      int mode, void* stream) {
  return conv_dispatch(src, n_src, cin_per_src, wpk, bias, res0, res1, mask, base, out, N, cout, H, W, 0, relu,
                       mode, stream, nullptr);
}

int larva_conv3x3_fwd_pitched(const float* const* src, int n_src, int cin_per_src, const float* wpk,
                              const float* bias, const float* res0, const float* res1, const float* mask,
                              const float* base, float* out, int N, int cout, int H, int W, int pitch,
                              int relu, int mode, void* stream) {
  return conv_dispatch(src, n_src, cin_per_src, wpk, bias, res0, res1, mask, base, out, N, cout, H, W, pitch,
                       relu, mode, stream, nullptr);
}

int larva_conv3x3_fwd_tiled(const float* const* src, int n_src, int cin_per_src, const float* wpk,
                            const float* bias, const float* res0, const float* res1, const float* mask,
                            const float* base, float* out, int N, int cout, int H, int W, int pitch,
                            int relu, int mode, int tile_rows, void* stream) {
  return conv_dispatch(src, n_src, cin_per_src, wpk, bias, res0, res1, mask, base, out, N, cout, H, W, pitch,
                       relu, mode, stream, nullptr, tile_rows);
}

int larva_conv3x3_fwd_batch(int njobs, const float* const* src, int n_src, int cin_per_src,
                            const float* const* wpk, const float* const* bias, const float* const* res0,
                            const float* const* res1, const float* const* mask, const float* const* base,
                            float* const* out, int N, int cout, int H, int W, int pitch, int relu, int mode,
                            void* stream) {
  if (njobs < 2 || njobs > kMaxConvJobs || !src || !wpk || !out) return (int)hipErrorInvalidValue;
  ConvBatch b{};
  int epi0 = -1;
  for (int j = 0; j < njobs; ++j) {
    bool aligned;
    int epi;
    const int rc = conv_build(src + (size_t)j * n_src, n_src, cin_per_src, wpk[j], bias ? bias[j] : nullptr,
                              res0 ? res0[j] : nullptr, res1 ? res1[j] : nullptr, mask ? mask[j] : nullptr,
                              base ? base[j] : nullptr, out[j], N, H, W, pitch, relu, mode, b.job[j], aligned, epi);
    if (rc) return rc;
    if (!aligned) return (int)hipErrorNotSupported;
    if (j > 0 && epi != epi0) return (int)hipErrorInvalidValue;
    epi0 = epi;
  }
  return (int)with_cout(cout, hipErrorInvalidValue, [&](auto c) {
    return launch_batch<decltype(c)::value>(b, njobs, epi0, (hipStream_t)stream);
  });
}

int larva_exit_l1_partials(int N, int H, int pitch) {
  return 4 * N * ((pitch + kTileCols - 1) / kTileCols) * ((H + kTileRows - 1) / kTileRows);
}

int larva_conv3x3_exit_l1_batch(int njobs, const float* const* src, int n_src, int cin_per_src,
                                const float* const* wpk, const float* const* bias, const float* const* base,
                                const float* const* truth, float* const* out, float* const* grad,
                                float* const* partial, float gval, int N, int cout, int H, int W, int pitch,
                                void* stream) {
  if (njobs < 2 || njobs > kMaxConvJobs || !src || !wpk || !base || !truth || !out || !grad || !partial)
    return (int)hipErrorInvalidValue;
  if (cout != 48) return (int)hipErrorNotSupported;
  ConvBatch b{};
  for (int j = 0; j < njobs; ++j) {
    bool aligned;
    int epi;
    if (!base[j] || !truth[j] || !grad[j] || !partial[j]) return (int)hipErrorInvalidValue;
    const int rc = conv_build(src + (size_t)j * n_src, n_src, cin_per_src, wpk[j], bias ? bias[j] : nullptr, nullptr,
                              nullptr, nullptr, base[j], grad[j], N, H, W, pitch, 0, 1, b.job[j], aligned, epi);
    if (rc) return rc;
    if (!aligned || ((reinterpret_cast<uintptr_t>(truth[j]) | reinterpret_cast<uintptr_t>(base[j])) & 15))
      return (int)hipErrorNotSupported;
    b.job[j].out = out[j];
    b.job[j].truth = truth[j];
    b.job[j].grad = grad[j];
    b.job[j].partial = partial[j];
    b.job[j].gval = gval;
  }
  return (int)launch_batch<48>(b, njobs, kEpiShuffleL1, (hipStream_t)stream);
}

int larva_strip_tile_table(int H, int W, int phase, unsigned* tab, int cap) {
  if (H <= 0 || W <= 0 || H >= 4096 || W >= 4096 || !tab || cap < 0) return -1;
  int n5 = 0, n4 = 0;
  for (int pass = 0; pass < 2; ++pass) {
    int fives = 0, fours = 0, i5 = 0, i4 = 0;
    for (int x0 = 0; x0 < W; x0 += 16) {
      int best_a = -1, best_gap = 1 << 30;
      for (int a5 = 0; 5 * a5 <= H; ++a5) {
        if ((H - 5 * a5) % 4) continue;
        const int b4 = (H - 5 * a5) / 4;
        const int gap = (fives + a5) - (fours + b4);
        const int g = gap < 0 ? -gap : gap;
        if (g < best_gap) { best_gap = g; best_a = a5; }
      }
      if (best_a < 0) return -2;
      const int a5 = best_a, b4 = (H - 5 * a5) / 4;
      fives += a5; fours += b4;
      if (pass == 0) continue;
      int y = 0, ra = a5, rb = b4;
      while (ra > 0 || rb > 0) {
        const bool five = ra > 0 && (rb == 0 || (long long)ra * b4 >= (long long)rb * a5);
        const int k = five ? i5++ : i4++;
        const int mine = five ? n5 : n4, other = five ? n4 : n5;
        const bool first = five == (phase == 0);
        int slot;
        if (k < other) slot = 2 * k + (first ? 0 : 1);
        else slot = 2 * other + (k - other);
        (void)mine;
        if (slot < cap) tab[slot] = (unsigned)y | ((unsigned)x0 << 12) | (five ? 0x80000000u : 0u);
        y += five ? 5 : 4;
        if (five) --ra; else --rb;
      }
    }
    n5 = fives; n4 = fours;
  }
  return n5 + n4;
}

static int strips_dispatch(const float* const* src, int n_src, int cin_per_src, const float* wpk,
                           const float* bias, const float* res0, const float* res1, const float* mask,
                           const float* base, float* out, int N, int cout, int H, int W, int pitch,
                           int relu, int mode, const unsigned* tile_tab, const unsigned* tile_tab_host,
                           int tiles_per_image, int plain_stores, void* stream, const LaunchTiming* tm) {
  if (cout != 48 && cout != 32 && cout != 64) return (int)hipErrorNotSupported;
  if (!tile_tab || tiles_per_image < 1) return (int)hipErrorInvalidValue;
  ConvArgs a;
  bool aligned;
  int epi;
  const int rc = conv_build(src, n_src, cin_per_src, wpk, bias, res0, res1, mask, base, out, N, H, W, pitch, relu,
                            mode, a, aligned, epi);
  if (rc) return rc;
  if (!aligned) return (int)hipErrorNotSupported;
  if ((long long)N * tiles_per_image >= (1ll << 20)) return (int)hipErrorInvalidValue;
  if ((long long)cout * H * a.pitch * 4 >= (1ll << 31)) return (int)hipErrorNotSupported;
  a.tile_tab = tile_tab;
  if (tile_tab_host && tiles_per_image <= 64 && H <= 256 && pitch <= 2048) {
    a.tab_n = tiles_per_image;
    for (int t = 0; t < tiles_per_image; ++t) {
      const unsigned e = tile_tab_host[t];
      const unsigned y0 = e & 0xfffu, x0 = (e >> 12) & 0xfffu;
      if (y0 > 255u || (x0 & 15u) || (x0 >> 4) > 127u) { a.tab_n = 0; break; }
      const unsigned h = y0 | ((x0 >> 4) << 8) | ((e >> 31) << 15);
      a.tab16[t >> 1] |= (int)(h << ((t & 1) * 16));
    }
  }
  a.plain_stores = plain_stores ? 1 : 0;
  a.tiles_x = tiles_per_image;
  a.tiles_y = 1;
  a.magic_tx = div_magic(tiles_per_image);
  a.magic_ty = div_magic(1);
  a.nwg = N * tiles_per_image;
  return (int)with_cout(cout, hipErrorNotSupported, [&](auto c) {
    return launch_strip<decltype(c)::value>(a, epi, (hipStream_t)stream, tm);
  });
}

int larva_conv3x3_fwd_strips(const float* const* src, int n_src, int cin_per_src, const float* wpk,
                             const float* bias, const float* res0, const float* res1, const float* mask,
                             const float* base, float* out, int N, int cout, int H, int W, int pitch,
                             int relu, int mode, const unsigned* tile_tab, const unsigned* tile_tab_host,
                             int tiles_per_image, int plain_stores, void* stream) {
  return strips_dispatch(src, n_src, cin_per_src, wpk, bias, res0, res1, mask, base, out, N, cout, H, W, pitch, relu, mode,
                         tile_tab, tile_tab_host, tiles_per_image, plain_stores, stream, nullptr);
}

#if LARVA_DIAG & 32
int larva_diag_set_stamps(unsigned long long* buf) {
#if LARVA_DIAG & 512
  g_diag_host_base = buf;
#endif
  return (int)hipMemcpyToSymbol(HIP_SYMBOL(larva::g_stamps), &buf, sizeof(buf));
}
#endif

}
```

### larvanet_amd/csrc/larva_loss.h

```cpp
#pragma once
#include "larva_common.h"

namespace larva {

struct TermList {
  const float* p[8];
  int count[8];
  float scale[8];
  int n;
};

__device__ __forceinline__ void loss_terms_block(const TermList& l, float divisor, float* __restrict__ out,
                                                 float* __restrict__ host_cell = nullptr, unsigned* __restrict__ dev_seq = nullptr) {
  unsigned long long seq = 0ull;
  if (host_cell && threadIdx.x == 0) {
    if (dev_seq) seq = dev_seq[0];
    else seq = __hip_atomic_load(reinterpret_cast<unsigned long long*>(host_cell), __ATOMIC_RELAXED, __HIP_MEMORY_SCOPE_SYSTEM) >> 32;
  }
  float sv[8];
#pragma unroll
  for (int i = 0; i < 8; ++i) {
    float s_ = 0.f;
    if (i < l.n)
      for (int k = threadIdx.x; k < l.count[i]; k += 256) s_ += l.p[i][k];
    sv[i] = s_;
  }
#pragma unroll
  for (int i = 0; i < 8; ++i)
#pragma unroll
    for (int o = 32; o > 0; o >>= 1) sv[i] += __shfl_xor(sv[i], o);
  __shared__ float wsa[8][4];
  if ((threadIdx.x & 63) == 0) {
#pragma unroll
    for (int i = 0; i < 8; ++i) wsa[i][threadIdx.x >> 6] = sv[i];
  }
  __syncthreads();
  float total = 0.f;
  for (int i = 0; i < l.n; ++i) total += ((wsa[i][0] + wsa[i][1]) + (wsa[i][2] + wsa[i][3])) * l.scale[i];
  if (threadIdx.x == 0) {
    const float v = total / divisor;
    out[0] = v;
    if (host_cell) {
      if (dev_seq) dev_seq[0] = (unsigned)(seq + 1ull);
      __hip_atomic_store(reinterpret_cast<unsigned long long*>(host_cell),
                         ((seq + 1ull) << 32) | (unsigned long long)__float_as_uint(v), __ATOMIC_RELAXED,
                         __HIP_MEMORY_SCOPE_SYSTEM);
    }
  }
}

}
```

### larvanet_amd/csrc/larva_pointwise.hip

```cpp
#include "larva_common.h"
#include "larva_bicubic.h"
#include "larva_loss.h"

namespace larva {

__global__ void bicubic4_kernel(const float* __restrict__ in, float* __restrict__ out, int planes,
                                int H, int W) {
  bicubic4_body(in, out, planes, H, W, (long long)blockIdx.x * blockDim.x + threadIdx.x,
                (long long)gridDim.x * blockDim.x);
}

__global__ __launch_bounds__(256) void bicubic4_block_kernel(const float* __restrict__ in, float* __restrict__ out,
                                                              unsigned planes, unsigned H, unsigned W) {
  const unsigned total = planes * H * W;
  const unsigned i = blockIdx.x * 256u + threadIdx.x;
  if (i >= total) return;
  const unsigned x = i % W, t2 = i / W, y = t2 % H, p = t2 / H;
  const float* src = in + (size_t)p * H * W;
  int col[5];
#pragma unroll
  for (int c = 0; c < 5; ++c) col[c] = min(max((int)x - 2 + c, 0), (int)W - 1);
  float v[5][5];
#pragma unroll
  for (int r = 0; r < 5; ++r) {
// ... 401 lines not shown
  return x;
}

struct AdamwBetas {
  float beta2, omb1, omb2;
};

__device__ __forceinline__ void adamw_update(float& param, float& mi, float& vi, float grad, const AdamwCoef& c,
                                             const AdamwBetas& b, float eps) {
  mi = __fmaf_rn(b.omb1, rounded(grad - mi), mi);
  vi = __fmaf_rn(rounded(b.omb2 * grad), grad, rounded(vi * b.beta2));
  const float denom = rounded(__fdiv_rn(__fsqrt_rn(vi), c.bc2_sqrt)) + eps;
  param = rounded(param * c.decay) + rounded(__fdiv_rn(rounded(-c.step_size * mi), denom));
}

__global__ __launch_bounds__(256) void adamw_kernel(float* __restrict__ p, const float* __restrict__ g,
                                                    float* __restrict__ m, float* __restrict__ v,
                                                    const float* __restrict__ step_lr, AdamwCoef coef, double beta1,
                                                    double beta2, float eps, float wd, float gscale, long long n, int vec,
                                                    const float* __restrict__ copy_src, float* __restrict__ copy_dst) {
  if (copy_dst && blockIdx.x == 0 && threadIdx.x == 0) copy_dst[0] = copy_src[0];
  if (step_lr) coef = adamw_coef_device(step_lr[0], step_lr[1], beta1, beta2, wd);
  const AdamwBetas bt{(float)beta2, (float)(1.0 - beta1), (float)(1.0 - beta2)};
  const long long n4 = vec ? n >> 2 : 0;
  for (long long i = (long long)blockIdx.x * blockDim.x + threadIdx.x; i < n4; i += (long long)gridDim.x * blockDim.x) {
    f32x4 pp = reinterpret_cast<f32x4*>(p)[i], mm = reinterpret_cast<f32x4*>(m)[i], vv = reinterpret_cast<f32x4*>(v)[i];
    const f32x4 gg = reinterpret_cast<const f32x4*>(g)[i];
#pragma unroll
    for (int e = 0; e < 4; ++e) {
      float pe = pp[e], me = mm[e], ve = vv[e];
      adamw_update(pe, me, ve, __fmul_rn(gg[e], gscale), coef, bt, eps);
      pp[e] = pe; mm[e] = me; vv[e] = ve;
    }
    reinterpret_cast<f32x4*>(p)[i] = pp;
    reinterpret_cast<f32x4*>(m)[i] = mm;
    reinterpret_cast<f32x4*>(v)[i] = vv;
  }
  for (long long i = (n4 << 2) + (long long)blockIdx.x * blockDim.x + threadIdx.x; i < n;
       i += (long long)gridDim.x * blockDim.x) {
    float pp = p[i], mm = m[i], vv = v[i];
    adamw_update(pp, mm, vv, __fmul_rn(g[i], gscale), coef, bt, eps);
    p[i] = pp; m[i] = mm; v[i] = vv;
  }
}

static int adamw_vec_ok(const void* p, const void* g, const void* m, const void* v) {
  return ((reinterpret_cast<uintptr_t>(p) | reinterpret_cast<uintptr_t>(g) | reinterpret_cast<uintptr_t>(m) |
           reinterpret_cast<uintptr_t>(v)) & 15) == 0;
}

__global__ void gather_patches_kernel(const unsigned char* __restrict__ data,
                                      const long long* __restrict__ offsets, const int* __restrict__ hw,
                                      const int* __restrict__ draws, float* __restrict__ out, int B, int P,
                                      int mult) {
  const long long total = (long long)B * 3 * P * P;
  for (long long idx = (long long)blockIdx.x * blockDim.x + threadIdx.x; idx < total;
       idx += (long long)gridDim.x * blockDim.x) {
    const int j = (int)(idx % P);
    long long t = idx / P;
    const int i = (int)(t % P); t /= P;
    const int c = (int)(t % 3);
    const int b = (int)(t / 3);
    const int* d = draws + 5 * b;
    const int img = d[0], x0 = d[1] * mult, y0 = d[2] * mult, k = d[3] & 3, flip = d[4];
    const int H = hw[2 * img], W = hw[2 * img + 1];
    const int jj = flip ? P - 1 - j : j;
    int si, sj;
    if (k == 0) { si = i; sj = jj; }
    else if (k == 1) { si = jj; sj = P - 1 - i; }
    else if (k == 2) { si = P - 1 - i; sj = P - 1 - jj; }
    else { si = P - 1 - jj; sj = i; }
    out[idx] = (float)data[offsets[img] + ((long long)c * H + (y0 + si)) * W + (x0 + sj)];
  }
}

__global__ __launch_bounds__(256) void sqerr_u8_kernel(const float* __restrict__ out,
                                                       const unsigned char* __restrict__ truth, int C, int H,
                                                       int W, int TH, int TW,
                                                       unsigned long long* __restrict__ acc) {
  const long long total = (long long)C * H * W;
  unsigned long long s = 0;
  for (long long i = (long long)blockIdx.x * blockDim.x + threadIdx.x; i < total;
       i += (long long)gridDim.x * blockDim.x) {
    const int x = (int)(i % W);
    const long long t = i / W;
    const int y = (int)(t % H);
    const int c = (int)(t / H);
    const float q = fminf(fmaxf(rintf(out[i]), 0.f), 255.f);
    const int d = (int)truth[((size_t)c * TH + y) * TW + x] - (int)q;
    s += (unsigned long long)(d * d);
  }
#pragma unroll
  for (int o = 32; o > 0; o >>= 1) s += __shfl_xor(s, o);
  if ((threadIdx.x & 63) == 0) atomicAdd(acc, s);
}

static inline int grid_for(long long work, int block) {
  long long g = (work + block - 1) / block;
  if (g > 2048) g = 2048;
  if (g < 1) g = 1;
  return (int)g;
}

template <bool VEC>
__global__ __launch_bounds__(256) void u8_hwc_to_f32_chw_kernel(const unsigned char* __restrict__ in,
                                                                float* __restrict__ out, long long HW,
                                                                long long total) {
  for (long long i = (long long)blockIdx.x * blockDim.x + threadIdx.x; i < total;
       i += (long long)gridDim.x * blockDim.x) {
    if constexpr (VEC) {
      const long long per = HW >> 2, n = i / per, q = i - n * per;
      const unsigned* src = reinterpret_cast<const unsigned*>(in) + 3 * i;
      const unsigned d0 = src[0], d1 = src[1], d2 = src[2];
      const unsigned b[12] = {d0 & 255u, (d0 >> 8) & 255u, (d0 >> 16) & 255u, d0 >> 24,
                              d1 & 255u, (d1 >> 8) & 255u, (d1 >> 16) & 255u, d1 >> 24,
                              d2 & 255u, (d2 >> 8) & 255u, (d2 >> 16) & 255u, d2 >> 24};
      float* dst = out + n * 3 * HW + 4 * q;
#pragma unroll
      for (int c = 0; c < 3; ++c)
        *reinterpret_cast<f32x4*>(dst + c * HW) = f32x4{(float)b[c], (float)b[3 + c], (float)b[6 + c], (float)b[9 + c]};
    } else {
      const long long n = i / HW, p = i - n * HW;
      const unsigned char* src = in + 3 * i;
      float* dst = out + n * 3 * HW + p;
#pragma unroll
      for (int c = 0; c < 3; ++c) dst[c * HW] = (float)src[c];
    }
  }
}

template <bool VEC>
__global__ __launch_bounds__(256) void f32_chw_to_u8_hwc_kernel(const float* __restrict__ in,
                                                                unsigned char* __restrict__ out, long long HW,
                                                                long long total) {
  for (long long i = (long long)blockIdx.x * blockDim.x + threadIdx.x; i < total;
       i += (long long)gridDim.x * blockDim.x) {
    if constexpr (VEC) {
      const long long per = HW >> 2, n = i / per, q = i - n * per;
      const float* src = in + n * 3 * HW + 4 * q;
      const f32x4 r = *reinterpret_cast<const f32x4*>(src);
      const f32x4 g = *reinterpret_cast<const f32x4*>(src + HW);
      const f32x4 b = *reinterpret_cast<const f32x4*>(src + 2 * HW);
      *reinterpret_cast<rgb4_bytes*>(out + 12 * i) = pack_rgb4(r, g, b);
    } else {
      const long long n = i / HW, p = i - n * HW;
      const float* src = in + n * 3 * HW + p;
      unsigned char* dst = out + 3 * i;
#pragma unroll
      for (int c = 0; c < 3; ++c) dst[c] = (unsigned char)quantize_u8(src[c * HW]);
    }
  }
}

static inline bool u8_vec_ok(const void* a, const void* b, long long HW) {
  return HW % 4 == 0 && ((reinterpret_cast<uintptr_t>(a) | reinterpret_cast<uintptr_t>(b)) & 15u) == 0;
}

}

using namespace larva;

extern "C" {

int larva_bicubic4_fwd(const float* in, float* out, int N, int C, int H, int W, void* stream) {
  if (!in || !out || N <= 0 || C <= 0 || H <= 0 || W <= 0) return (int)hipErrorInvalidValue;
  const long long px = (long long)N * C * H * W;
  if (px < (1ll << 31) - 256 && !(reinterpret_cast<uintptr_t>(out) & 15)) {
    hipLaunchKernelGGL(bicubic4_block_kernel, dim3((unsigned)((px + 255) / 256)), dim3(256), 0, (hipStream_t)stream, in, out,
                       (unsigned)(N * C), (unsigned)H, (unsigned)W);
    return (int)hipGetLastError();
  }
  const long long work = (long long)N * C * 4 * H * W;
  hipLaunchKernelGGL(bicubic4_kernel, dim3(grid_for(work, 256)), dim3(256), 0, (hipStream_t)stream, in, out,
                     N * C, H, W);
  return (int)hipGetLastError();
}

int larva_upsample4_fwd(const float* in, float* out, int N, int C, int H, int W, int mode, void* stream) {
  if (mode == 0) return larva_bicubic4_fwd(in, out, N, C, H, W, stream);
  if (!in || !out || N <= 0 || C <= 0 || H <= 0 || W <= 0 || mode != 1 || (reinterpret_cast<uintptr_t>(out) & 15))
    return (int)hipErrorInvalidValue;
  const long long work = (long long)N * C * 4 * H * W;
  hipLaunchKernelGGL(bilinear4_kernel, dim3(grid_for(work, 256)), dim3(256), 0, (hipStream_t)stream, in, out, N * C, H, W);
  return (int)hipGetLastError();
}

int larva_head_conv3_direct(const float* x, const float* w, const float* bias, float* out, int N, int cout,
                            int H, int W, int pitch, void* stream) {
  if (pitch == 0) pitch = W;
  if (!x || !w || !out || N <= 0 || cout <= 0 || cout % kHeadCoutsPerThread || H <= 0 || W <= 0 || pitch < W)
    return (int)hipErrorInvalidValue;
  const long long total = (long long)N * H * pitch;
  if (total >= (1ll << 31) - 256 || (long long)N * 3 * H * W >= (1ll << 31)) return (int)hipErrorInvalidValue;
  if (pitch % 4 == 0 && cout % kHead4Couts == 0 && !(reinterpret_cast<uintptr_t>(out) & 15)) {
    hipLaunchKernelGGL(head_conv3_direct4_kernel, dim3((unsigned)((total / 4 + 255) / 256), cout / kHead4Couts), dim3(256), 0,
                       (hipStream_t)stream, x, w, bias, out, N, cout, H, W, pitch);
    return (int)hipGetLastError();
  }
  hipLaunchKernelGGL(head_conv3_direct_kernel, dim3((unsigned)((total + 255) / 256), cout / kHeadCoutsPerThread), dim3(256),
                     0, (hipStream_t)stream, x, w, bias, out, N, cout, H, W, pitch);
  return (int)hipGetLastError();
}

int larva_l1_workspace_floats(void) { return kL1Blocks; }

int larva_l1_fwd(const float* a, const float* b, long long numel, float* workspace, float* loss,
                 void* stream) {
  if (!a || !b || !workspace || !loss || numel <= 0) return (int)hipErrorInvalidValue;
  if ((reinterpret_cast<uintptr_t>(a) | reinterpret_cast<uintptr_t>(b)) & 15) return (int)hipErrorInvalidValue;
  int blocks = grid_for(numel / 4, 256);
  if (blocks > kL1Blocks) blocks = kL1Blocks;
  hipLaunchKernelGGL(l1_partial_kernel, dim3(blocks), dim3(256), 0, (hipStream_t)stream, a, b, numel, workspace);
  hipLaunchKernelGGL(l1_finish_kernel, dim3(1), dim3(256), 0, (hipStream_t)stream, workspace, blocks,
                     1.0f / (float)numel, loss);
  return (int)hipGetLastError();
}

int larva_l1_partial(const float* a, const float* b, long long numel, float* partial, int* blocks_out,
                     void* stream) {
  if (!a || !b || !partial || !blocks_out || numel <= 0) return (int)hipErrorInvalidValue;
  if ((reinterpret_cast<uintptr_t>(a) | reinterpret_cast<uintptr_t>(b)) & 15) return (int)hipErrorInvalidValue;
  int blocks = grid_for(numel / 4, 256);
  if (blocks > kL1Blocks) blocks = kL1Blocks;
  *blocks_out = blocks;
  hipLaunchKernelGGL(l1_partial_kernel, dim3(blocks), dim3(256), 0, (hipStream_t)stream, a, b, numel, partial);
  return (int)hipGetLastError();
}

int larva_l1_partial_grad(const float* a, const float* b, float gvalue, float gscale, float* partial,
                          int* blocks_out, float* grad, int N, int C, int H, int W, void* stream) {
  if (!a || !b || !partial || !blocks_out || !grad || N <= 0 || C <= 0 || H <= 0 || W <= 0)
    return (int)hipErrorInvalidValue;
  if ((reinterpret_cast<uintptr_t>(a) | reinterpret_cast<uintptr_t>(b)) & 15) return (int)hipErrorInvalidValue;
  const long long numel = (long long)N * C * 16 * H * W;
  int blocks = grid_for(numel / 4, 256);
  if (blocks > kL1Blocks) blocks = kL1Blocks;
  *blocks_out = blocks;
  const float g = (gvalue * gscale) * (1.0f / (float)numel);
  hipLaunchKernelGGL(l1_partial_grad_kernel, dim3(blocks), dim3(256), 0, (hipStream_t)stream, a, b, numel, g, partial,
                     grad, H, W);
  return (int)hipGetLastError();
}

int larva_l1_partial_grad_batch(const float* const* a, const float* b, int n, float gvalue, float gscale,
                                float* const* partial, int* blocks_out, float* const* grad, int N, int C, int H,
                                int W, void* stream) {
  if (!a || !b || !partial || !blocks_out || !grad || n < 1 || n > 8 || N <= 0 || C <= 0 || H <= 0 || W <= 0)
    return (int)hipErrorInvalidValue;
  L1Jobs jobs{};
  uintptr_t bits = reinterpret_cast<uintptr_t>(b);
  for (int i = 0; i < n; ++i) {
    if (!a[i] || !partial[i] || !grad[i]) return (int)hipErrorInvalidValue;
    jobs.a[i] = a[i]; jobs.partial[i] = partial[i]; jobs.grad[i] = grad[i];
    bits |= reinterpret_cast<uintptr_t>(a[i]);
  }
  if (bits & 15) return (int)hipErrorInvalidValue;
  const long long numel = (long long)N * C * 16 * H * W;
  int blocks = grid_for(numel / 4, 256);
  if (blocks > kL1Blocks) blocks = kL1Blocks;
  *blocks_out = blocks;
  const float g = (gvalue * gscale) * (1.0f / (float)numel);
  hipLaunchKernelGGL(l1_partial_grad_batch_kernel, dim3(blocks, n), dim3(256), 0, (hipStream_t)stream, jobs, b, numel,
                     g, H, W);
  return (int)hipGetLastError();
}

int larva_loss_from_partials_to_host_seq(const float* const* terms, const int* count, const float* scale, int n,
                                         float divisor, float* out, float* host_cell, unsigned* dev_seq, void* stream) {
  if (!terms || !count || !scale || n < 1 || n > 8 || !out || (dev_seq && !host_cell)) return (int)hipErrorInvalidValue;
  TermList l{};
  for (int i = 0; i < n; ++i) {
    if (!terms[i] || count[i] < 1) return (int)hipErrorInvalidValue;
    l.p[i] = terms[i];
    l.count[i] = count[i];
    l.scale[i] = scale[i];
  }
  l.n = n;
  hipLaunchKernelGGL(loss_from_partials_kernel, dim3(1), dim3(256), 0, (hipStream_t)stream, l, divisor, out, host_cell, dev_seq);
  return (int)hipGetLastError();
}

int larva_loss_from_partials_to_host(const float* const* terms, const int* count, const float* scale, int n,
                                     float divisor, float* out, float* host_cell, void* stream) {
  return larva_loss_from_partials_to_host_seq(terms, count, scale, n, divisor, out, host_cell, nullptr, stream);
}

int larva_loss_from_partials(const float* const* terms, const int* count, const float* scale, int n,
                             float divisor, float* out, void* stream) {
  return larva_loss_from_partials_to_host(terms, count, scale, n, divisor, out, nullptr, stream);
}

int larva_host_cell_alloc(float** cell) {
  if (!cell) return (int)hipErrorInvalidValue;
  void* p = nullptr;
  hipError_t e = hipHostMalloc(&p, 64, hipHostMallocCoherent | hipHostMallocMapped);
  if (e != hipSuccess) return (int)e;
  *cell = static_cast<float*>(p);
  (*cell)[0] = __builtin_nanf("");
  reinterpret_cast<unsigned*>(p)[1] = 0u;
  return 0;
}

int larva_host_cell_free(float* cell) {
  if (!cell) return 0;
  (void)hipDeviceSynchronize();
  return (int)hipHostFree(cell);
}

int larva_l1_bwd_unshuffle4(const float* a, const float* b, const float* gout, float gscale, float* ga, int N,
                            int C, int H, int W, void* stream) {
  if (!a || !b || !gout || !ga || N <= 0 || C <= 0 || H <= 0 || W <= 0) return (int)hipErrorInvalidValue;
  if ((reinterpret_cast<uintptr_t>(a) | reinterpret_cast<uintptr_t>(b)) & 15) return (int)hipErrorInvalidValue;
  const long long work = (long long)N * C * 4 * H * W;
  const float inv = 1.0f / (float)(work * 4);
  hipLaunchKernelGGL(l1_bwd_unshuffle4_kernel, dim3(grid_for(work, 256)), dim3(256), 0, (hipStream_t)stream, a, b,
                     gout, gscale, inv, ga, N * C, H, W);
  return (int)hipGetLastError();
}


int larva_sum_scalars(const float* const* terms, int n, float divisor, float* out, void* stream) {
  if (!terms || n < 1 || n > 8 || !out) return (int)hipErrorInvalidValue;
  ScalarList l{};
  for (int i = 0; i < n; ++i) {
    if (!terms[i]) return (int)hipErrorInvalidValue;
    l.p[i] = terms[i];
  }
  l.n = n;
  hipLaunchKernelGGL(sum_scalars_kernel, dim3(1), dim3(64), 0, (hipStream_t)stream, l, divisor, out);
  return (int)hipGetLastError();
}

int larva_l1_bwd(const float* a, const float* b, const float* gout, long long numel, float* ga,
                 void* stream) {
  if (!a || !b || !gout || !ga || numel <= 0) return (int)hipErrorInvalidValue;
  if ((reinterpret_cast<uintptr_t>(a) | reinterpret_cast<uintptr_t>(b) | reinterpret_cast<uintptr_t>(ga)) & 15)
    return (int)hipErrorInvalidValue;
  hipLaunchKernelGGL(l1_bwd_kernel, dim3(grid_for(numel / 4, 256)), dim3(256), 0, (hipStream_t)stream, a, b,
                     gout, 1.0f / (float)numel, numel, ga);
  return (int)hipGetLastError();
}

int larva_pixel_unshuffle4(const float* in, float* out, int N, int C, int H, int W, void* stream) {
  if (!in || !out || N <= 0 || C <= 0 || H <= 0 || W <= 0) return (int)hipErrorInvalidValue;
  const long long work = (long long)N * C * 4 * H * W;
  hipLaunchKernelGGL(pixel_unshuffle4_kernel, dim3(grid_for(work, 256)), dim3(256), 0, (hipStream_t)stream, in,
                     out, N * C, H, W);
  return (int)hipGetLastError();
}

int larva_adamw_step(float* p, const float* g, float* m, float* v, const float* step_lr, double beta1,
                     double beta2, double eps, double weight_decay, float grad_scale, long long n,
                     void* stream) {
  if (!p || !g || !m || !v || !step_lr || n <= 0) return (int)hipErrorInvalidValue;
  hipLaunchKernelGGL(adamw_kernel, dim3(grid_for((n + 3) / 4, 256)), dim3(256), 0, (hipStream_t)stream, p, g, m, v,
                     step_lr, AdamwCoef{}, beta1, beta2, (float)eps, (float)weight_decay, grad_scale, n, adamw_vec_ok(p, g, m, v),
                     (const float*)nullptr,
                     (float*)nullptr);
  return (int)hipGetLastError();
}

int larva_adamw_step_host_copy(float* p, const float* g, float* m, float* v, int step, double lr, double beta1,
                               double beta2, double eps, double weight_decay, float grad_scale, long long n,
                               const float* copy_src, float* copy_dst, void* stream);

int larva_adamw_step_host(float* p, const float* g, float* m, float* v, int step, double lr, double beta1,
                          double beta2, double eps, double weight_decay, float grad_scale, long long n,
                          void* stream) {
  return larva_adamw_step_host_copy(p, g, m, v, step, lr, beta1, beta2, eps, weight_decay, grad_scale, n, nullptr, nullptr,
                                    stream);
}

int larva_adamw_step_host_copy(float* p, const float* g, float* m, float* v, int step, double lr, double beta1,
                               double beta2, double eps, double weight_decay, float grad_scale, long long n,
                               const float* copy_src, float* copy_dst, void* stream) {
  if (!p || !g || !m || !v || n <= 0 || step < 1 || (copy_dst && !copy_src)) return (int)hipErrorInvalidValue;
  const double bc1 = 1.0 - pow(beta1, (double)step), bc2 = 1.0 - pow(beta2, (double)step);
  const AdamwCoef coef{(float)(lr / bc1), (float)sqrt(bc2), (float)(1.0 - lr * weight_decay)};
  hipLaunchKernelGGL(adamw_kernel, dim3(grid_for((n + 3) / 4, 256)), dim3(256), 0, (hipStream_t)stream, p, g, m, v,
                     (const float*)nullptr, coef, beta1, beta2, (float)eps, (float)weight_decay, grad_scale, n, adamw_vec_ok(p, g, m, v),
                     copy_src, copy_dst);
  return (int)hipGetLastError();
}

int larva_gather_patches(const unsigned char* data, const long long* offsets, const int* hw,
                         const int* draws, float* out, int B, int P, int mult, void* stream) {
  if (!data || !offsets || !hw || !draws || !out || B <= 0 || P <= 0 || mult <= 0) return (int)hipErrorInvalidValue;
  hipLaunchKernelGGL(gather_patches_kernel, dim3(grid_for((long long)B * 3 * P * P, 256)), dim3(256), 0,
                     (hipStream_t)stream, data, offsets, hw, draws, out, B, P, mult);
  return (int)hipGetLastError();
}

int larva_sqerr_u8(const float* out, const unsigned char* truth, int C, int H, int W, int TH, int TW,
                   unsigned long long* acc, void* stream) {
  if (!out || !truth || !acc || C <= 0 || H <= 0 || W <= 0 || TH < H || TW < W) return (int)hipErrorInvalidValue;
  hipLaunchKernelGGL(sqerr_u8_kernel, dim3(grid_for((long long)C * H * W, 256)), dim3(256), 0, (hipStream_t)stream,
                     out, truth, C, H, W, TH, TW, acc);
  return (int)hipGetLastError();
}

static bool image_shape_ok(int N, int H, int W) {
  return N > 0 && H > 0 && W > 0 && (long long)N * H * W * 3 < (1ll << 40);
}

int larva_u8_hwc_to_f32_chw(const unsigned char* in, float* out, int N, int H, int W, void* stream) {
  if (!in || !out || !image_shape_ok(N, H, W)) return (int)hipErrorInvalidValue;
  const long long HW = (long long)H * W;
  if (u8_vec_ok(in, out, HW)) {
    const long long total = N * (HW / 4);
    hipLaunchKernelGGL(u8_hwc_to_f32_chw_kernel<true>, dim3(grid_for(total, 256)), dim3(256), 0, (hipStream_t)stream, in,
                       out, HW, total);
  } else {
    const long long total = N * HW;
    hipLaunchKernelGGL(u8_hwc_to_f32_chw_kernel<false>, dim3(grid_for(total, 256)), dim3(256), 0, (hipStream_t)stream, in,
                       out, HW, total);
  }
  return (int)hipGetLastError();
}

// ... 21 lines not shown
```

### larvanet_amd/hip_lib.py

```python
import ctypes
import os

_HERE = os.path.dirname(os.path.abspath(__file__))
LIB_PATH = os.path.join(_HERE, "csrc", "liblarva_hip.so")

_c_float_p = ctypes.c_void_p
_c_pp = ctypes.POINTER(ctypes.c_void_p)
_c_int_p = ctypes.POINTER(ctypes.c_int)

SIGNATURES = {
    "larva_abi_version": (ctypes.c_int, []),
    "larva_error_string": (ctypes.c_char_p, [ctypes.c_int]),
    "larva_packed_weight_floats": (ctypes.c_longlong, [ctypes.c_int, ctypes.c_int]),
    "larva_pack_weights": (ctypes.c_int, [_c_float_p, _c_float_p, _c_float_p, ctypes.c_int, ctypes.c_int,
                                          ctypes.c_int, ctypes.c_int, ctypes.c_void_p]),
    "larva_pack_weights_batch": (ctypes.c_int, [_c_pp, _c_pp, _c_pp, _c_int_p, _c_int_p, _c_int_p, _c_int_p,
                                                ctypes.c_int, ctypes.c_void_p]),
    "larva_step_prologue": (ctypes.c_int, [_c_pp, _c_pp, _c_pp, _c_int_p, _c_int_p, _c_int_p, _c_int_p, ctypes.c_int,
                                           _c_float_p, _c_float_p, _c_float_p, ctypes.c_int, ctypes.c_int, ctypes.c_int,
                                           ctypes.c_int, ctypes.c_void_p]),
    "larva_conv3x3_fwd": (ctypes.c_int, [_c_pp, ctypes.c_int, ctypes.c_int, _c_float_p, _c_float_p,
                                         _c_float_p, _c_float_p, _c_float_p, _c_float_p, _c_float_p,
                                         ctypes.c_int, ctypes.c_int, ctypes.c_int, ctypes.c_int,
                                         ctypes.c_int, ctypes.c_int, ctypes.c_void_p]),
    "larva_conv3x3_fwd_pitched": (ctypes.c_int, [_c_pp, ctypes.c_int, ctypes.c_int, _c_float_p, _c_float_p,
                                                 _c_float_p, _c_float_p, _c_float_p, _c_float_p, _c_float_p,
                                                 ctypes.c_int, ctypes.c_int, ctypes.c_int, ctypes.c_int,
                                                 ctypes.c_int, ctypes.c_int, ctypes.c_int, ctypes.c_void_p]),
    "larva_conv3x3_fwd_batch": (ctypes.c_int, [ctypes.c_int, _c_pp, ctypes.c_int, ctypes.c_int, _c_pp, _c_pp, _c_pp, _c_pp,
                                               _c_pp, _c_pp, _c_pp, ctypes.c_int, ctypes.c_int, ctypes.c_int,
                                               ctypes.c_int, ctypes.c_int, ctypes.c_int, ctypes.c_int, ctypes.c_void_p]),
    "larva_conv3x3_fwd_tiled": (ctypes.c_int, [_c_pp, ctypes.c_int, ctypes.c_int, _c_float_p, _c_float_p,
                                               _c_float_p, _c_float_p, _c_float_p, _c_float_p, _c_float_p,
                                               ctypes.c_int, ctypes.c_int, ctypes.c_int, ctypes.c_int,
                                               ctypes.c_int, ctypes.c_int, ctypes.c_int, ctypes.c_int, ctypes.c_void_p]),
    "larva_conv3x3_fwd_strips": (ctypes.c_int, [_c_pp, ctypes.c_int, ctypes.c_int, _c_float_p, _c_float_p,
                                                _c_float_p, _c_float_p, _c_float_p, _c_float_p, _c_float_p,
                                                ctypes.c_int, ctypes.c_int, ctypes.c_int, ctypes.c_int,
                                                ctypes.c_int, ctypes.c_int, ctypes.c_int, ctypes.c_void_p,
                                                ctypes.POINTER(ctypes.c_uint), ctypes.c_int, ctypes.c_int, ctypes.c_void_p]),
    "larva_head_conv3_direct": (ctypes.c_int, [_c_float_p, _c_float_p, _c_float_p, _c_float_p, ctypes.c_int, ctypes.c_int,
                                               ctypes.c_int, ctypes.c_int, ctypes.c_int, ctypes.c_void_p]),
    "larva_exit_l1_partials": (ctypes.c_int, [ctypes.c_int, ctypes.c_int, ctypes.c_int]),
    "larva_conv3x3_exit_l1_batch": (ctypes.c_int, [ctypes.c_int, _c_pp, ctypes.c_int, ctypes.c_int, _c_pp, _c_pp, _c_pp, _c_pp,
                                                   _c_pp, _c_pp, _c_pp, ctypes.c_float, ctypes.c_int, ctypes.c_int,
                                                   ctypes.c_int, ctypes.c_int, ctypes.c_int, ctypes.c_void_p]),
    "larva_strip_tile_table": (ctypes.c_int, [ctypes.c_int, ctypes.c_int, ctypes.c_int, ctypes.POINTER(ctypes.c_uint),
                                              ctypes.c_int]),
    "larva_wgrad_partial_floats": (ctypes.c_longlong, [ctypes.c_int, ctypes.c_int, ctypes.c_int]),
    "larva_conv3x3_wgrad": (ctypes.c_int, [_c_pp, _c_pp, _c_pp, _c_pp, _c_pp, _c_int_p, _c_int_p, _c_int_p,
                                           ctypes.c_int, ctypes.c_int, ctypes.c_int, ctypes.c_int,
                                           ctypes.c_int, ctypes.c_int, ctypes.c_int, ctypes.c_void_p]),
    "larva_conv3x3_wgrad_partial": (ctypes.c_int, [_c_pp, _c_pp, _c_pp, ctypes.c_int, ctypes.c_int, ctypes.c_int,
                                                   ctypes.c_int, ctypes.c_int, ctypes.c_int, ctypes.c_int,
                                                   _c_int_p, ctypes.c_void_p]),
    "larva_wgrad_flat_head_splits": (ctypes.c_int, [ctypes.c_int, ctypes.c_int, ctypes.c_int]),
    "larva_conv3x3_wgrad_partial_flat_head": (ctypes.c_int, [_c_pp, _c_pp, _c_pp, ctypes.c_int, _c_float_p, _c_float_p,
                                                             _c_float_p, ctypes.c_int, ctypes.c_int, ctypes.c_int,
                                                             ctypes.c_int, _c_int_p, _c_int_p, ctypes.c_void_p]),
    "larva_wgrad_flat_max_splits": (ctypes.c_int, [ctypes.c_int, ctypes.c_int, ctypes.c_int]),
    "larva_conv3x3_wgrad_partial_flat": (ctypes.c_int, [_c_pp, _c_pp, _c_pp, ctypes.c_int, ctypes.c_int, ctypes.c_int,
                                                        ctypes.c_int, ctypes.c_int, ctypes.c_int, ctypes.c_int,
                                                        _c_int_p, ctypes.c_void_p]),
    "larva_wgrad_reduce": (ctypes.c_int, [_c_pp, _c_pp, _c_pp, _c_int_p, _c_int_p, _c_int_p, _c_int_p, _c_int_p,
                                          _c_int_p, ctypes.c_int, ctypes.c_void_p]),
    "larva_wgrad_reduce_with_loss": (ctypes.c_int, [_c_pp, _c_pp, _c_pp, _c_int_p, _c_int_p, _c_int_p, _c_int_p, _c_int_p,
                                                    _c_int_p, ctypes.c_int, _c_pp, _c_int_p, _c_float_p, ctypes.c_int,
                                                    ctypes.c_float, _c_float_p, ctypes.c_void_p]),
    "larva_adamw_step_host_copy": (ctypes.c_int, [_c_float_p, _c_float_p, _c_float_p, _c_float_p, ctypes.c_int,
                                                  ctypes.c_double, ctypes.c_double, ctypes.c_double, ctypes.c_double,
                                                  ctypes.c_double, ctypes.c_float, ctypes.c_longlong, _c_float_p, _c_float_p,
                                                  ctypes.c_void_p]),
    "larva_upsample4_fwd": (ctypes.c_int, [_c_float_p, _c_float_p, ctypes.c_int, ctypes.c_int, ctypes.c_int,
                                           ctypes.c_int, ctypes.c_int, ctypes.c_void_p]),
    "larva_bicubic4_fwd": (ctypes.c_int, [_c_float_p, _c_float_p, ctypes.c_int, ctypes.c_int, ctypes.c_int,
                                          ctypes.c_int, ctypes.c_void_p]),
    "larva_l1_workspace_floats": (ctypes.c_int, []),
    "larva_l1_fwd": (ctypes.c_int, [_c_float_p, _c_float_p, ctypes.c_longlong, _c_float_p, _c_float_p,
                                    ctypes.c_void_p]),
    "larva_l1_bwd": (ctypes.c_int, [_c_float_p, _c_float_p, _c_float_p, ctypes.c_longlong, _c_float_p,
                                    ctypes.c_void_p]),
    "larva_l1_bwd_unshuffle4": (ctypes.c_int, [_c_float_p, _c_float_p, _c_float_p, ctypes.c_float, _c_float_p,
                                               ctypes.c_int, ctypes.c_int, ctypes.c_int, ctypes.c_int, ctypes.c_void_p]),
    "larva_l1_partial": (ctypes.c_int, [_c_float_p, _c_float_p, ctypes.c_longlong, _c_float_p, _c_int_p,
                                        ctypes.c_void_p]),
    "larva_l1_partial_grad": (ctypes.c_int, [_c_float_p, _c_float_p, ctypes.c_float, ctypes.c_float, _c_float_p,
                                             _c_int_p, _c_float_p, ctypes.c_int, ctypes.c_int, ctypes.c_int,
                                             ctypes.c_int, ctypes.c_void_p]),
    "larva_l1_partial_grad_batch": (ctypes.c_int, [_c_pp, _c_float_p, ctypes.c_int, ctypes.c_float, ctypes.c_float, _c_pp,
                                                   _c_int_p, _c_pp, ctypes.c_int, ctypes.c_int, ctypes.c_int,
                                                   ctypes.c_int, ctypes.c_void_p]),
    "larva_loss_from_partials_to_host": (ctypes.c_int, [_c_pp, _c_int_p, _c_float_p, ctypes.c_int, ctypes.c_float,
                                                        _c_float_p, _c_float_p, ctypes.c_void_p]),
    "larva_loss_from_partials_to_host_seq": (ctypes.c_int, [_c_pp, _c_int_p, _c_float_p, ctypes.c_int, ctypes.c_float,
                                                            _c_float_p, _c_float_p, ctypes.c_void_p, ctypes.c_void_p]),
    "larva_host_cell_alloc": (ctypes.c_int, [ctypes.POINTER(ctypes.c_void_p)]),
    "larva_host_cell_free": (ctypes.c_int, [_c_float_p]),
    "larva_loss_from_partials": (ctypes.c_int, [_c_pp, _c_int_p, _c_float_p, ctypes.c_int, ctypes.c_float,
                                                _c_float_p, ctypes.c_void_p]),
    "larva_sum_scalars": (ctypes.c_int, [_c_pp, ctypes.c_int, ctypes.c_float, _c_float_p, ctypes.c_void_p]),
    "larva_upsample_fwd": (ctypes.c_int, [_c_float_p, _c_float_p, ctypes.c_int, ctypes.c_int, ctypes.c_int, ctypes.c_int,
                                          ctypes.c_int, ctypes.c_int, ctypes.c_void_p]),
    "larva_pixel_shuffle_base": (ctypes.c_int, [_c_float_p, _c_float_p, _c_float_p, ctypes.c_int, ctypes.c_int, ctypes.c_int,
                                                ctypes.c_int, ctypes.c_int, ctypes.c_int, ctypes.c_int, ctypes.c_void_p]),
    "larva_pixel_unshuffle": (ctypes.c_int, [_c_float_p, _c_float_p, ctypes.c_int, ctypes.c_int, ctypes.c_int, ctypes.c_int,
                                             ctypes.c_int, ctypes.c_int, ctypes.c_void_p]),
    "larva_l1_bwd_unshuffle": (ctypes.c_int, [_c_float_p, _c_float_p, _c_float_p, ctypes.c_float, _c_float_p, ctypes.c_int,
                                              ctypes.c_int, ctypes.c_int, ctypes.c_int, ctypes.c_int, ctypes.c_int,
                                              ctypes.c_void_p]),
    "larva_shuffle_l1_partial_grad": (ctypes.c_int, [_c_float_p, _c_float_p, _c_float_p, ctypes.c_float, ctypes.c_float,
                                                     _c_float_p, _c_int_p, _c_float_p, _c_float_p, ctypes.c_int, ctypes.c_int,
                                                     ctypes.c_int, ctypes.c_int, ctypes.c_int, ctypes.c_int, ctypes.c_void_p]),
    "larva_pixel_unshuffle4": (ctypes.c_int, [_c_float_p, _c_float_p, ctypes.c_int, ctypes.c_int,
                                              ctypes.c_int, ctypes.c_int, ctypes.c_void_p]),
    "larva_wgrad_cu_share": (ctypes.c_int, [ctypes.c_int, ctypes.c_int]),
    "larva_adamw_step_host": (ctypes.c_int, [_c_float_p, _c_float_p, _c_float_p, _c_float_p, ctypes.c_int,
                                             ctypes.c_double, ctypes.c_double, ctypes.c_double, ctypes.c_double,
                                             ctypes.c_double, ctypes.c_float, ctypes.c_longlong, ctypes.c_void_p]),
    "larva_gather_patches": (ctypes.c_int, [ctypes.c_void_p, ctypes.c_void_p, ctypes.c_void_p, ctypes.c_void_p,
                                            _c_float_p, ctypes.c_int, ctypes.c_int, ctypes.c_int, ctypes.c_void_p]),
    "larva_sqerr_u8": (ctypes.c_int, [_c_float_p, ctypes.c_void_p, ctypes.c_int, ctypes.c_int, ctypes.c_int,
                                      ctypes.c_int, ctypes.c_int, ctypes.c_void_p, ctypes.c_void_p]),
    "larva_adamw_step": (ctypes.c_int, [_c_float_p, _c_float_p, _c_float_p, _c_float_p, _c_float_p,
                                        ctypes.c_double, ctypes.c_double, ctypes.c_double, ctypes.c_double,
                                        ctypes.c_float, ctypes.c_longlong, ctypes.c_void_p]),
    "larva_f16_packed_weight_halves": (ctypes.c_longlong, [ctypes.c_int, ctypes.c_int]),
    "larva_f16_pack_weights": (ctypes.c_int, [_c_float_p, ctypes.c_void_p, ctypes.c_int, ctypes.c_int, ctypes.c_void_p]),
    "larva_f16_head": (ctypes.c_int, [_c_float_p, _c_float_p, _c_float_p, ctypes.c_void_p, ctypes.c_void_p, ctypes.c_int,
                                      ctypes.c_int, ctypes.c_int, ctypes.c_void_p]),
    "larva_f16_conv3x3": (ctypes.c_int, [_c_pp, ctypes.c_int, ctypes.c_void_p, _c_float_p, ctypes.c_void_p, ctypes.c_void_p,
                                         ctypes.c_int, ctypes.c_void_p, ctypes.c_void_p, ctypes.c_int, ctypes.c_int,
                                         ctypes.c_int, ctypes.c_void_p]),
    "larva_f16_conv3x3_shuffle_base": (ctypes.c_int, [ctypes.c_void_p, ctypes.c_void_p, _c_float_p, _c_float_p, _c_float_p,
                                                      ctypes.c_int, ctypes.c_int, ctypes.c_int, ctypes.c_void_p]),
    "larva_f16_conv3x3_shuffle_base_u8": (ctypes.c_int, [ctypes.c_void_p, ctypes.c_void_p, _c_float_p, _c_float_p,
                                                         ctypes.c_void_p, ctypes.c_void_p, ctypes.c_int, ctypes.c_int,
                                                         ctypes.c_int, ctypes.c_void_p]),
    "larva_u8_hwc_to_f32_chw": (ctypes.c_int, [ctypes.c_void_p, _c_float_p, ctypes.c_int, ctypes.c_int, ctypes.c_int,
                                               ctypes.c_void_p]),
    "larva_f32_chw_to_u8_hwc": (ctypes.c_int, [_c_float_p, ctypes.c_void_p, ctypes.c_int, ctypes.c_int, ctypes.c_int,
                                               ctypes.c_void_p]),
    "larva_u8_metrics_workspace_bytes": (ctypes.c_longlong, [ctypes.c_int, ctypes.c_int, ctypes.c_int]),
    "larva_u8_metrics": (ctypes.c_int, [ctypes.c_void_p, ctypes.c_longlong, ctypes.c_void_p, ctypes.c_longlong, ctypes.c_int,
                                        ctypes.c_int, ctypes.c_int, ctypes.c_int, ctypes.c_int, ctypes.c_int,
                                        ctypes.c_void_p, ctypes.c_void_p, ctypes.c_void_p]),
    "larva_dihedral_inputs_u8": (ctypes.c_int, [ctypes.c_void_p, _c_float_p, _c_float_p, ctypes.c_int, ctypes.c_int,
                                                ctypes.c_int, ctypes.c_void_p]),
    "larva_dihedral_inputs_f32": (ctypes.c_int, [_c_float_p, _c_float_p, _c_float_p, ctypes.c_int, ctypes.c_int,
                                                 ctypes.c_int, ctypes.c_void_p]),
    "larva_dihedral_mean": (ctypes.c_int, [_c_float_p, _c_float_p, _c_float_p, ctypes.c_void_p, ctypes.c_int, ctypes.c_int,
                                           ctypes.c_int, ctypes.c_void_p]),
}

_lib = None


def load():
    global _lib
    if _lib is not None:
        return _lib
    path = os.environ.get("LARVA_HIP_LIB") or LIB_PATH
    if not os.path.exists(path):
        raise RuntimeError(
            "larvanet_amd: %s is missing. Build it with `python -m larvanet_amd.build` "
            "(hipcc --offload-arch=gfx950); there is no CPU or PyTorch fallback." % path)
    import torch
    lib = ctypes.CDLL(path)
    for name, (res, args) in SIGNATURES.items():
        fn = getattr(lib, name)
        fn.restype = res
        fn.argtypes = args
    _lib = lib
    return lib


def check(code, what):
    if code != 0:
        lib = load()
        msg = lib.larva_error_string(code)
        raise RuntimeError("larvanet_amd: %s failed: hip error %d (%s)" %
                           (what, code, msg.decode() if msg else "?"))


def ptr_array(ptrs):
    arr = (ctypes.c_void_p * len(ptrs))()
    for i, p in enumerate(ptrs):
        arr[i] = p
    return arr


def int_array(vals):
    return (ctypes.c_int * len(vals))(*vals)
```

### larvanet_amd/kernels.py

```python
import ctypes
import os
import struct

import torch

from . import hip_lib

_SUPPORTED_COUT = (32, 48, 64)


def _stream():
    return torch.cuda.current_stream().cuda_stream


def _chk_tensor(t, name, shape, dtype, last=None):
    if not isinstance(t, torch.Tensor) or not t.is_cuda:
        raise RuntimeError("larvanet_amd: %s must be a tensor on a HIP device (no CPU path exists)" % name)
    kind = str(dtype).replace("torch.", "")
    if last is None:
        if t.dtype != dtype:
            raise RuntimeError("larvanet_amd: %s must be %s, got %s" % (name, kind, t.dtype))
        if not t.is_contiguous():
            raise RuntimeError("larvanet_amd: %s must be contiguous" % name)
    else:
# ... 61 lines not shown
    lib = hip_lib.load()
    for i in range(0, len(jobs), 64):
        code = lib.larva_pack_weights_batch(*_pack_job_args(jobs[i:i + 64]), _stream())
        hip_lib.check(code, "larva_pack_weights_batch")


_STRIP_TABLES = {}


def strip_tile_table(H, P, device, phase=0):
    key = (int(H), int(P), str(device), int(phase))
    hit = _STRIP_TABLES.get(key)
    if hit is None:
        lib = hip_lib.load()
        cap = 4 * ((H + 3) // 4) * ((P + 15) // 16) + 16
        buf = (ctypes.c_uint * cap)()
        n = int(lib.larva_strip_tile_table(int(H), int(P), int(phase), buf, cap))
        if n <= 0 or n > cap:
            hit = False
        else:
            if torch.cuda.is_current_stream_capturing():
                raise RuntimeError("larvanet_amd: strip-tile table for %dx%d requested during stream capture "
                                   "(run the step once outside the capture first)" % (H, P))
            import numpy as np
            hit = (torch.from_numpy(np.frombuffer(buf, dtype=np.int32, count=n).copy()).to(device), n, buf)
        _STRIP_TABLES[key] = hit
    return hit or None


def step_prologue(jobs, x, x16, base):
    lib = hip_lib.load()
    if len(jobs) > 64:
        raise RuntimeError("larvanet_amd: at most 64 pack jobs per prologue launch")
    N, C, H, W = (int(v) for v in x.shape)
    _chk(x, "x")
    _chk(x16, "x16", (N, 16, H, W))
    _chk(base, "base", (N, C, 4 * H, 4 * W))
    code = lib.larva_step_prologue(*_pack_job_args(jobs), x.data_ptr(), x16.data_ptr(), base.data_ptr(), N, C, H, W, _stream())
    hip_lib.check(code, "larva_step_prologue")


def conv3x3(srcs, wpk, cout, bias=None, relu=False, mask=None, res0=None, res1=None,
            shuffle=False, base=None, out=None, logical_w=None, images=None, strips=False, plain_stores=False,
            tile_rows=0):
    lib = hip_lib.load()
    if isinstance(srcs, torch.Tensor):
        srcs = [srcs]
    if not 1 <= len(srcs) <= 8:
        raise RuntimeError("larvanet_amd: 1..8 source tensors")
    if cout not in _SUPPORTED_COUT:
        raise RuntimeError("larvanet_amd: cout must be one of %s" % (_SUPPORTED_COUT,))
    N, cps, H, P = (int(v) for v in srcs[0].shape)
    W = P if logical_w is None else int(logical_w)
    if not 0 < W <= P:
        raise RuntimeError("larvanet_amd: logical width %d does not fit the row pitch %d" % (W, P))
    if cps % 8:
        raise RuntimeError("larvanet_amd: input channels per tensor must be a multiple of 8")
    ptrs = [_chk(s, "src[%d]" % i, (N, cps, H, P)) for i, s in enumerate(srcs)]
    cin = cps * len(srcs)
    _chk(wpk, "wpk", (packed_weight_floats(cout, cin),))
    full = (N, cout, H, P)
    hr = (N, cout // 16, 4 * H, 4 * W)
    if out is None:
        out = torch.empty(hr if shuffle else full, device=srcs[0].device, dtype=torch.float32)
    _chk(out, "out", hr if shuffle else full)
    lo, hi = (0, N) if images is None else (int(images[0]), int(images[1]))
    if not 0 <= lo < hi <= N:
        raise RuntimeError("larvanet_amd: image range [%d, %d) outside the batch of %d" % (lo, hi, N))

    def at(ptr, per_image_floats):
        return None if ptr is None else ptr + 4 * lo * per_image_floats

    lr_img, hr_img = H * P, 16 * H * W
    args = (hip_lib.ptr_array([at(p, cps * lr_img) for p in ptrs]), len(srcs), cps, wpk.data_ptr(),
            _opt(bias, "bias", (cout,)), at(_opt(res0, "res0", full), cout * lr_img),
            at(_opt(res1, "res1", full), cout * lr_img), at(_opt(mask, "mask", full), cout * lr_img),
            at(_opt(base, "base", hr), (cout // 16) * hr_img),
            at(out.data_ptr(), (cout // 16) * hr_img if shuffle else cout * lr_img),
            hi - lo, cout, H, W, P, 1 if relu else 0, 1 if shuffle else 0)
    if strips and cout in (48, 32, 64):
        tab = strip_tile_table(H, P, out.device, phase=1 if strips == 2 else 0)
        if tab is not None:
            code = lib.larva_conv3x3_fwd_strips(*args, tab[0].data_ptr(), tab[2], tab[1], 1 if plain_stores else 0, _stream())
            if code != 801:
                hip_lib.check(code, "larva_conv3x3_fwd_strips")
                return out
    if tile_rows:
        code = lib.larva_conv3x3_fwd_tiled(*args, int(tile_rows), _stream())
    else:
        code = lib.larva_conv3x3_fwd_pitched(*args, _stream())
    hip_lib.check(code, "larva_conv3x3_fwd")
    return out


def conv3x3_batch(jobs, cout, relu=False, shuffle=False, logical_w=None):
    lib = hip_lib.load()
    if not 2 <= len(jobs) <= 4:
        raise RuntimeError("larvanet_amd: 2..4 conv jobs per batched launch")
    norm = []
    for j in jobs:
        srcs = j["srcs"]
        norm.append(dict(j, srcs=[srcs] if isinstance(srcs, torch.Tensor) else list(srcs)))
    n_src = len(norm[0]["srcs"])
    N, cps, H, P = (int(v) for v in norm[0]["srcs"][0].shape)
    W = P if logical_w is None else int(logical_w)
    if cout not in _SUPPORTED_COUT or cps % 8 or not 0 < W <= P or not 1 <= n_src <= 8:
        raise RuntimeError("larvanet_amd: unsupported batched conv shape")
    cin = cps * n_src
    full, hr = (N, cout, H, P), (N, cout // 16, 4 * H, 4 * W)
    names = ("bias", "res0", "res1", "mask", "base")
    used = {k: norm[0].get(k) is not None for k in names}
    src_ptrs, cols, outs = [], {k: [] for k in names}, []
    for j in norm:
        if len(j["srcs"]) != n_src or any((j.get(k) is not None) != used[k] for k in names):
            raise RuntimeError("larvanet_amd: batched conv jobs must share one shape and one fusion")
        src_ptrs += [_chk(t, "src", (N, cps, H, P)) for t in j["srcs"]]
        _chk(j["wpk"], "wpk", (packed_weight_floats(cout, cin),))
        for k, shape in (("bias", (cout,)), ("res0", full), ("res1", full), ("mask", full), ("base", hr)):
            if used[k]:
                cols[k].append(_chk(j[k], k, shape))
        outs.append(torch.empty(hr if shuffle else full, device=j["srcs"][0].device, dtype=torch.float32))

    def arr(k):
        return hip_lib.ptr_array(cols[k]) if used[k] else None

    common = (len(norm), hip_lib.ptr_array(src_ptrs), n_src, cps, hip_lib.ptr_array([j["wpk"].data_ptr() for j in norm]),
              arr("bias"), arr("res0"), arr("res1"), arr("mask"), arr("base"),
              hip_lib.ptr_array([o.data_ptr() for o in outs]), N, cout, H, W, P, 1 if relu else 0, 1 if shuffle else 0)
    code = lib.larva_conv3x3_fwd_batch(*common, _stream())
    if code == 801:
        return [conv3x3(j["srcs"], j["wpk"], cout, bias=j.get("bias"), relu=relu, mask=j.get("mask"),
                        res0=j.get("res0"), res1=j.get("res1"), shuffle=shuffle, base=j.get("base"), out=o,
                        logical_w=logical_w)
                for j, o in zip(norm, outs)]
    hip_lib.check(code, "larva_conv3x3_fwd_batch")
    return outs


def head_conv3_direct(x, w, bias=None, pitch=None):
    lib = hip_lib.load()
    N, C, H, W = (int(v) for v in x.shape)
    cout = int(w.shape[0])
    if C != 3 or tuple(w.shape[1:]) != (3, 3, 3) or cout % 16:
        raise RuntimeError("larvanet_amd: the direct head conv takes a 3-channel image and [cout][3][3][3] weights")
    _chk(x, "x")
    _chk(w, "w")
    P = W if pitch is None else int(pitch)
    out = torch.empty((N, cout, H, P), device=x.device, dtype=torch.float32)
    hip_lib.check(lib.larva_head_conv3_direct(x.data_ptr(), w.data_ptr(), _opt(bias, "bias", (cout,)), out.data_ptr(),
                                              N, cout, H, W, P, _stream()), "larva_head_conv3_direct")
    return out


def conv3x3_exit_l1_batch(jobs, cout, truth, gvalue, gscale, want_image):
    lib = hip_lib.load()
    if not 2 <= len(jobs) <= 4 or cout != 48:
        return None
    norm = [dict(j, srcs=[j["srcs"]] if isinstance(j["srcs"], torch.Tensor) else list(j["srcs"])) for j in jobs]
    n_src = len(norm[0]["srcs"])
    N, cps, H, P = (int(v) for v in norm[0]["srcs"][0].shape)
    hr = (N, cout // 16, 4 * H, 4 * P)
    _chk(truth, "truth", hr)
    numel = float(truth.numel())
    import numpy as np
    gval = float((np.float32(gvalue) * np.float32(gscale)) * (np.float32(1.0) / np.float32(numel)))
    npart = int(lib.larva_exit_l1_partials(N, H, P))
    src_ptrs, outs, grads, parts = [], [], [], []
    for j, want in zip(norm, want_image):
        if len(j["srcs"]) != n_src:
            raise RuntimeError("larvanet_amd: batched exits must share one shape")
        src_ptrs += [_chk(t, "src", (N, cps, H, P)) for t in j["srcs"]]
        _chk(j["wpk"], "wpk", (packed_weight_floats(cout, cps * n_src),))
        _chk(j["bias"], "bias", (cout,))
        _chk(j["base"], "base", hr)
        outs.append(torch.empty(hr, device=truth.device, dtype=torch.float32) if want else None)
        grads.append(torch.empty((N, cout, H, P), device=truth.device, dtype=torch.float32))
        parts.append(torch.empty(npart, device=truth.device, dtype=torch.float32))
    code = lib.larva_conv3x3_exit_l1_batch(
        len(norm), hip_lib.ptr_array(src_ptrs), n_src, cps, hip_lib.ptr_array([j["wpk"].data_ptr() for j in norm]),
        hip_lib.ptr_array([j["bias"].data_ptr() for j in norm]), hip_lib.ptr_array([j["base"].data_ptr() for j in norm]),
        hip_lib.ptr_array([truth.data_ptr()] * len(norm)), hip_lib.ptr_array([None if o is None else o.data_ptr() for o in outs]),
        hip_lib.ptr_array([g.data_ptr() for g in grads]), hip_lib.ptr_array([p.data_ptr() for p in parts]),
        gval, N, cout, H, P, P, _stream())
    if code == 801:
        return None
    hip_lib.check(code, "larva_conv3x3_exit_l1_batch")
    return outs, parts, grads


def wgrad_partial_floats(cout, cin, splits):
    return int(hip_lib.load().larva_wgrad_partial_floats(cout, cin, splits))


def max_wgrad_jobs():
    return 64


def wgrad_cu_share(cout, cin):
    return int(hip_lib.load().larva_wgrad_cu_share(int(cout), int(cin)))


def conv3x3_wgrad(jobs, cout, cin, splits):
    lib = hip_lib.load()
    if not 1 <= len(jobs) <= max_wgrad_jobs():
        raise RuntimeError("larvanet_amd: 1..%d wgrad jobs per call" % max_wgrad_jobs())
    N, _, H, W = (int(v) for v in jobs[0]["dy"].shape)
    dys, xs, parts, dws, dbs, offs, valids, totals, keep = [], [], [], [], [], [], [], [], []
    nfl = wgrad_partial_floats(cout, cin, splits)
    for j in jobs:
        dys.append(_chk(j["dy"], "dy", (N, cout, H, W)))
        xs.append(_chk(j["x"], "x", (N, cin, H, W)))
        dw = j["dw"]
        _chk(dw, "dw")
        if dw.dim() != 4 or int(dw.shape[0]) != cout or tuple(dw.shape[2:]) != (3, 3):
            raise RuntimeError("larvanet_amd: dw must be [cout][cin_total][3][3]")
        total = int(dw.shape[1])
        off = int(j.get("cin_off", 0))
        valid = int(j.get("cin_valid", cin))
        if off < 0 or valid < 1 or valid > cin or off + valid > total:
            raise RuntimeError("larvanet_amd: wgrad channel slice out of range")
        part = j.get("partial")
        if part is None:
            part = torch.empty(nfl, device=dw.device, dtype=torch.float32)
        _chk(part, "partial", (nfl,))
        keep.append(part)
        parts.append(part.data_ptr())
        dws.append(dw.data_ptr())
        dbs.append(_opt(j.get("db"), "db", (cout,)))
        offs.append(off)
        valids.append(valid)
        totals.append(total)
    code = lib.larva_conv3x3_wgrad(
        hip_lib.ptr_array(dys), hip_lib.ptr_array(xs), hip_lib.ptr_array(parts), hip_lib.ptr_array(dws),
        hip_lib.ptr_array(dbs), hip_lib.int_array(offs), hip_lib.int_array(valids), hip_lib.int_array(totals),
        len(jobs), splits, N, cout, cin, H, W, _stream())
    hip_lib.check(code, "larva_conv3x3_wgrad")
    return keep


def conv3x3_wgrad_partial(jobs, cout, cin, splits):
    lib = hip_lib.load()
    if not 1 <= len(jobs) <= 64:
        raise RuntimeError("larvanet_amd: 1..64 wgrad jobs per call")
    N, _, H, W = (int(v) for v in jobs[0]["dy"].shape)
    splits = max(1, min(int(splits), N * ((H + 2) // 3) * ((W + 47) // 48)))
    nfl = wgrad_partial_floats(cout, cin, splits)
    dys = [_chk(j["dy"], "dy", (N, cout, H, W)) for j in jobs]
    xs = [_chk(j["x"], "x", (N, cin, H, W)) for j in jobs]
    parts = [torch.empty(nfl, device=jobs[0]["dy"].device, dtype=torch.float32) for _ in jobs]
    used = ctypes.c_int(0)
    code = lib.larva_conv3x3_wgrad_partial(
        hip_lib.ptr_array(dys), hip_lib.ptr_array(xs), hip_lib.ptr_array([p.data_ptr() for p in parts]),
        len(jobs), splits, N, cout, cin, H, W, ctypes.byref(used), _stream())
    hip_lib.check(code, "larva_conv3x3_wgrad_partial")
    return parts, int(used.value)


def conv3x3_wgrad_partial_flat(jobs, cout, cin, nwg, head=None):
    lib = hip_lib.load()
    if not 1 <= len(jobs) <= 64 or (cout, cin) not in ((48, 48), (32, 32), (64, 64)) or (head is not None and cout != 48):
        return None
    N, _, H, W = (int(v) for v in jobs[0]["dy"].shape)
    if W % 4:
        return None
    tiles = N * ((H + 2) // 3) * ((W + 47) // 48)
    cap = int(lib.larva_wgrad_flat_max_splits(len(jobs), int(nwg), tiles))
    nfl = wgrad_partial_floats(cout, cin, cap)
    dys = [_chk(j["dy"], "dy", (N, cout, H, W)) for j in jobs]
    xs = [_chk(j["x"], "x", (N, cin, H, W)) for j in jobs]
    dev = jobs[0]["dy"].device
    parts = [torch.empty(nfl, device=dev, dtype=torch.float32) for _ in jobs]
    used = (ctypes.c_int * len(jobs))()
    if head is None:
        code = lib.larva_conv3x3_wgrad_partial_flat(
            hip_lib.ptr_array(dys), hip_lib.ptr_array(xs), hip_lib.ptr_array([p.data_ptr() for p in parts]),
            len(jobs), int(nwg), N, cout, cin, H, W, used, _stream())
    else:
        hcap = int(lib.larva_wgrad_flat_head_splits(len(jobs), int(nwg), tiles))
        hper = wgrad_partial_floats(48, 16, 1)
        hpart = torch.empty(hper * hcap, device=dev, dtype=torch.float32)
        hused = ctypes.c_int(0)
        code = lib.larva_conv3x3_wgrad_partial_flat_head(
            hip_lib.ptr_array(dys), hip_lib.ptr_array(xs), hip_lib.ptr_array([p.data_ptr() for p in parts]), len(jobs),
            _chk(head["dy"], "head dy", (N, 48, H, W)), _chk(head["x"], "head x", (N, 16, H, W)), hpart.data_ptr(),
            int(nwg), N, H, W, used, ctypes.byref(hused), _stream())
    if code == 801:
        return None
    hip_lib.check(code, "larva_conv3x3_wgrad_partial_flat")
    splits = [int(v) for v in used]
    per = wgrad_partial_floats(cout, cin, 1)
    out = [p[:per * s] for p, s in zip(parts, splits)]
    if head is not None:
        out.append(hpart[:hper * int(hused.value)])
        splits.append(int(hused.value))
    return out, splits


def _loss_terms(terms, scales):
    ptrs, counts = [], []
    for t in terms:
        _chk(t, "term")
        if t.dim() > 1:
            raise RuntimeError("larvanet_amd: a loss term is a scalar or a vector of partial sums")
        ptrs.append(t.data_ptr())
        counts.append(max(1, int(t.numel())))
    sc = (ctypes.c_float * len(terms))(*[float(v) for v in scales])
    return hip_lib.ptr_array(ptrs), hip_lib.int_array(counts), sc


def wgrad_reduce(jobs, cout=None, cin=None, loss=None):
    lib = hip_lib.load()
    if not 1 <= len(jobs) <= 64:
        raise RuntimeError("larvanet_amd: 1..64 reduce jobs per call")
    parts, dws, dbs, offs, valids, totals, splits, couts, cins = [], [], [], [], [], [], [], [], []
    for j in jobs:
        co, ci = int(j.get("cout", cout)), int(j.get("cin", cin))
        dw = j["dw"]
        _chk(dw, "dw")
        if dw.dim() != 4 or int(dw.shape[0]) != co or tuple(dw.shape[2:]) != (3, 3):
            raise RuntimeError("larvanet_amd: dw must be [cout][cin_total][3][3]")
        total = int(dw.shape[1])
        off = int(j.get("cin_off", 0))
        valid = int(j.get("cin_valid", ci))
        if off < 0 or valid < 1 or valid > ci or off + valid > total:
            raise RuntimeError("larvanet_amd: wgrad channel slice out of range")
        sp = int(j["splits"])
        parts.append(_chk(j["partial"], "partial", (wgrad_partial_floats(co, ci, sp),)))
        dws.append(dw.data_ptr())
        dbs.append(_opt(j.get("db"), "db", (co,)))
        offs.append(off)
        valids.append(valid)
        totals.append(total)
        splits.append(sp)
        couts.append(co)
        cins.append(ci)
    common = (hip_lib.ptr_array(parts), hip_lib.ptr_array(dws), hip_lib.ptr_array(dbs), hip_lib.int_array(offs),
              hip_lib.int_array(valids), hip_lib.int_array(totals), hip_lib.int_array(splits), hip_lib.int_array(couts),
              hip_lib.int_array(cins), len(jobs))
    if loss is None:
        code = lib.larva_wgrad_reduce(*common, _stream())
# ... 80 lines not shown
                                             N, C, cpad, H, W, s, _stream()), "larva_l1_bwd_unshuffle")
    return out


def shuffle_l1_partial_grad(y, base, truth, gvalue, gscale, scale, want_image=True):
    lib = hip_lib.load()
    s = int(scale)
    _chk(truth, "truth")
    N, C, H, W = _lr_of(truth, s)
    cpad = int(y.shape[1])
    _chk(y, "y", (N, cpad, H, W))
    _chk(base, "base", truth.shape)
    part = torch.empty(int(lib.larva_l1_workspace_floats()), device=y.device, dtype=torch.float32)
    grad = torch.empty((N, cpad, H, W), device=y.device, dtype=torch.float32)
    out = torch.empty(truth.shape, device=y.device, dtype=torch.float32) if want_image else None
    blocks = ctypes.c_int(0)
    hip_lib.check(lib.larva_shuffle_l1_partial_grad(y.data_ptr(), base.data_ptr(), truth.data_ptr(), float(gvalue),
                                                    float(gscale), part.data_ptr(), ctypes.byref(blocks), grad.data_ptr(),
                                                    None if out is None else out.data_ptr(), N, C, cpad, H, W, s, _stream()),
                  "larva_shuffle_l1_partial_grad")
    return part[:int(blocks.value)], 1.0 / float(truth.numel()), grad, out


def bicubic4(x):
    lib = hip_lib.load()
    N, C, H, W = (int(v) for v in x.shape)
    _chk(x, "x")
    out = torch.empty((N, C, 4 * H, 4 * W), device=x.device, dtype=torch.float32)
    hip_lib.check(lib.larva_bicubic4_fwd(x.data_ptr(), out.data_ptr(), N, C, H, W, _stream()), "larva_bicubic4_fwd")
    return out


_L1_WORKSPACES = {}


def _l1_workspace(device):
    lib = hip_lib.load()
    key = (str(device), torch.cuda.current_stream().cuda_stream)
    ws = _L1_WORKSPACES.get(key)
    if ws is None:
        ws = torch.empty(int(lib.larva_l1_workspace_floats()), device=device, dtype=torch.float32)
        _L1_WORKSPACES[key] = ws
    return ws


def l1_fwd(a, b):
    lib = hip_lib.load()
    _chk(a, "a")
    _chk(b, "b", a.shape)
    ws = _l1_workspace(a.device)
    loss = torch.empty((), device=a.device, dtype=torch.float32)
    hip_lib.check(lib.larva_l1_fwd(a.data_ptr(), b.data_ptr(), a.numel(), ws.data_ptr(), loss.data_ptr(), _stream()),
                  "larva_l1_fwd")
    return loss


def l1_partial(a, b):
    lib = hip_lib.load()
    _chk(a, "a")
    _chk(b, "b", a.shape)
    part = torch.empty(int(lib.larva_l1_workspace_floats()), device=a.device, dtype=torch.float32)
    blocks = ctypes.c_int(0)
    hip_lib.check(lib.larva_l1_partial(a.data_ptr(), b.data_ptr(), a.numel(), part.data_ptr(), ctypes.byref(blocks),
                                       _stream()), "larva_l1_partial")
    return part[:int(blocks.value)], 1.0 / float(a.numel())


def l1_partial_grad(a, b, gvalue, gscale):
    lib = hip_lib.load()
    _chk(a, "a")
    _chk(b, "b", a.shape)
    N, C, HH, WW = (int(v) for v in a.shape)
    if HH % 4 or WW % 4:
        raise RuntimeError("larvanet_amd: spatial dims must be divisible by 4")
    part = torch.empty(int(lib.larva_l1_workspace_floats()), device=a.device, dtype=torch.float32)
    grad = torch.empty((N, 16 * C, HH // 4, WW // 4), device=a.device, dtype=torch.float32)
    blocks = ctypes.c_int(0)
    hip_lib.check(lib.larva_l1_partial_grad(a.data_ptr(), b.data_ptr(), float(gvalue), float(gscale), part.data_ptr(),
                                            ctypes.byref(blocks), grad.data_ptr(), N, C, HH // 4, WW // 4, _stream()),
                  "larva_l1_partial_grad")
    return part[:int(blocks.value)], 1.0 / float(a.numel()), grad


def l1_partial_grad_batch(outs, truth, gvalue, gscale):
    lib = hip_lib.load()
    if not 1 <= len(outs) <= 8:
        raise RuntimeError("larvanet_amd: 1..8 images per batched L1 sweep")
    _chk(truth, "truth")
    N, C, HH, WW = (int(v) for v in truth.shape)
    if HH % 4 or WW % 4:
        raise RuntimeError("larvanet_amd: spatial dims must be divisible by 4")
    ptrs = [_chk(o, "out", truth.shape) for o in outs]
    nws = int(lib.larva_l1_workspace_floats())
    parts = [torch.empty(nws, device=truth.device, dtype=torch.float32) for _ in outs]
    grads = [torch.empty((N, 16 * C, HH // 4, WW // 4), device=truth.device, dtype=torch.float32) for _ in outs]
    blocks = ctypes.c_int(0)
    hip_lib.check(lib.larva_l1_partial_grad_batch(
        hip_lib.ptr_array(ptrs), truth.data_ptr(), len(outs), float(gvalue), float(gscale),
        hip_lib.ptr_array([p.data_ptr() for p in parts]), ctypes.byref(blocks),
        hip_lib.ptr_array([g.data_ptr() for g in grads]), N, C, HH // 4, WW // 4, _stream()), "larva_l1_partial_grad_batch")
    nb = int(blocks.value)
    return [p[:nb] for p in parts], 1.0 / float(truth.numel()), grads


class HostCell:

    def __init__(self):
        p = ctypes.c_void_p()
        hip_lib.check(hip_lib.load().larva_host_cell_alloc(ctypes.byref(p)), "larva_host_cell_alloc")
        self.ptr = int(p.value)
        self._cell = ctypes.c_uint64.from_address(self.ptr)
        self.expected = 0
        self.dev_seq = torch.zeros(1, dtype=torch.int32, device="cuda") if torch.cuda.is_available() else None

    def expect(self):
        self.expected = (self.expected + 1) & 0xFFFFFFFF

    def take(self):
        raw = self._cell.value
        if (raw >> 32) != self.expected:
            return None
        return struct.unpack("<f", struct.pack("<I", raw & 0xFFFFFFFF))[0]

    @property
    def value(self):
        return struct.unpack("<f", struct.pack("<I", self._cell.value & 0xFFFFFFFF))[0]

    @property
    def sequence(self):
        return self._cell.value >> 32

    def __del__(self):
        ptr, self.ptr = getattr(self, "ptr", 0), 0
        if ptr:
            try:
                hip_lib.load().larva_host_cell_free(ptr)
            except Exception:
                pass


def loss_from_partials(terms, scales, divisor, host_cell=None):
    lib = hip_lib.load()
    if not 1 <= len(terms) <= 8:
        raise RuntimeError("larvanet_amd: 1..8 loss terms")
    out = torch.empty((), device=terms[0].device, dtype=torch.float32)
    hip_lib.check(lib.larva_loss_from_partials_to_host_seq(
        *_loss_terms(terms, scales), len(terms), float(divisor), out.data_ptr(),
        host_cell.ptr if host_cell is not None else None,
        host_cell.dev_seq.data_ptr() if host_cell is not None and host_cell.dev_seq is not None else None, _stream()),
        "larva_loss_from_partials_to_host")
    return out


def l1_bwd_unshuffle4(a, b, gout, gscale=1.0):
    lib = hip_lib.load()
    _chk(a, "a")
    _chk(b, "b", a.shape)
    _chk(gout, "gout", ())
    N, C, HH, WW = (int(v) for v in a.shape)
    if HH % 4 or WW % 4:
        raise RuntimeError("larvanet_amd: spatial dims must be divisible by 4")
    out = torch.empty((N, 16 * C, HH // 4, WW // 4), device=a.device, dtype=torch.float32)
    hip_lib.check(lib.larva_l1_bwd_unshuffle4(a.data_ptr(), b.data_ptr(), gout.data_ptr(), float(gscale),
                                              out.data_ptr(), N, C, HH // 4, WW // 4, _stream()),
                  "larva_l1_bwd_unshuffle4")
    return out


def sum_scalars(terms, divisor):
    lib = hip_lib.load()
    ptrs = [_chk(t, "term", ()) for t in terms]
    out = torch.empty((), device=terms[0].device, dtype=torch.float32)
    hip_lib.check(lib.larva_sum_scalars(hip_lib.ptr_array(ptrs), len(ptrs), float(divisor), out.data_ptr(), _stream()),
                  "larva_sum_scalars")
    return out


def l1_bwd(a, b, gout):
    lib = hip_lib.load()
    _chk(a, "a")
    _chk(b, "b", a.shape)
    _chk(gout, "gout", ())
    ga = torch.empty_like(a)
    hip_lib.check(lib.larva_l1_bwd(a.data_ptr(), b.data_ptr(), gout.data_ptr(), a.numel(), ga.data_ptr(), _stream()),
                  "larva_l1_bwd")
    return ga


def pixel_unshuffle4(g):
    lib = hip_lib.load()
    _chk(g, "g")
    N, C, HH, WW = (int(v) for v in g.shape)
    if HH % 4 or WW % 4:
        raise RuntimeError("larvanet_amd: pixel_unshuffle4 needs spatial dims divisible by 4")
    H, W = HH // 4, WW // 4
    out = torch.empty((N, 16 * C, H, W), device=g.device, dtype=torch.float32)
    hip_lib.check(lib.larva_pixel_unshuffle4(g.data_ptr(), out.data_ptr(), N, C, H, W, _stream()),
                  "larva_pixel_unshuffle4")
    return out


def adamw_step(p, g, m, v, step_lr, beta1, beta2, eps, weight_decay, grad_scale=1.0):
    lib = hip_lib.load()
    n = p.numel()
    for t, name in ((p, "p"), (g, "g"), (m, "m"), (v, "v")):
        _chk(t, name, (n,))
    _chk(step_lr, "step_lr", (2,))
    hip_lib.check(lib.larva_adamw_step(p.data_ptr(), g.data_ptr(), m.data_ptr(), v.data_ptr(), step_lr.data_ptr(),
                                       beta1, beta2, eps, weight_decay, grad_scale, n, _stream()),
                  "larva_adamw_step")


def gather_patches(data, offsets, hw, draws, batch, patch, mult, out=None):
    lib = hip_lib.load()
    for t, name, dt in ((data, "data", torch.uint8), (offsets, "offsets", torch.int64), (hw, "hw", torch.int32),
                        (draws, "draws", torch.int32)):
        if not t.is_cuda or t.dtype != dt or not t.is_contiguous():
            raise RuntimeError("larvanet_amd: %s must be a contiguous %s tensor on the HIP device" % (name, dt))
    if tuple(draws.shape) != (batch, 5):
        raise RuntimeError("larvanet_amd: draws must be [batch][5]")
    if out is None:
        out = torch.empty((batch, 3, patch, patch), device=data.device, dtype=torch.float32)
    _chk(out, "out", (batch, 3, patch, patch))
    hip_lib.check(lib.larva_gather_patches(data.data_ptr(), offsets.data_ptr(), hw.data_ptr(), draws.data_ptr(),
                                           out.data_ptr(), batch, patch, mult, _stream()), "larva_gather_patches")
    return out


def adamw_step_host(p, g, m, v, step, lr, beta1, beta2, eps, weight_decay, grad_scale=1.0, copy=None):
    lib = hip_lib.load()
    n = p.numel()
    for t, name in ((p, "p"), (g, "g"), (m, "m"), (v, "v")):
        _chk(t, name, (n,))
    if copy is not None:
        src, dst = copy
        _chk(src, "copy source", ())
        _chk(dst, "copy destination", ())
        hip_lib.check(lib.larva_adamw_step_host_copy(p.data_ptr(), g.data_ptr(), m.data_ptr(), v.data_ptr(), int(step),
                                                     float(lr), beta1, beta2, eps, weight_decay, grad_scale, n,
                                                     src.data_ptr(), dst.data_ptr(), _stream()), "larva_adamw_step_host_copy")
        return
    hip_lib.check(lib.larva_adamw_step_host(p.data_ptr(), g.data_ptr(), m.data_ptr(), v.data_ptr(), int(step),
                                            float(lr), beta1, beta2, eps, weight_decay, grad_scale, n, _stream()),
                  "larva_adamw_step_host")


def psnr_u8(out_chw, truth_u8):
    import math
    lib = hip_lib.load()
    _chk(out_chw, "out")
    if not truth_u8.is_cuda or truth_u8.dtype != torch.uint8 or not truth_u8.is_contiguous():
        raise RuntimeError("larvanet_amd: truth must be a contiguous uint8 tensor on the HIP device")
    C, H, W = (int(v) for v in out_chw.shape)
    TC, TH, TW = (int(v) for v in truth_u8.shape)
    if TC != C or TH < H or TW < W:
        raise RuntimeError("larvanet_amd: truth image smaller than the output")
    acc = torch.zeros(1, device=out_chw.device, dtype=torch.int64)
    hip_lib.check(lib.larva_sqerr_u8(out_chw.data_ptr(), truth_u8.data_ptr(), C, H, W, TH, TW, acc.data_ptr(),
                                     _stream()), "larva_sqerr_u8")
    sq = int(acc.item())
    mse = sq / float(C * H * W)
    return float("inf") if mse == 0 else 10.0 * math.log10(255.0 ** 2 / mse)


F16_CHANNELS = 48
F16_MAX_SOURCES = 8


def _chk16(t, name, shape=None):
    return _chk_tensor(t, name, shape, torch.float16, F16_CHANNELS)


def _chk_wpk16(wpk, n_src, what):
    if wpk.dtype != torch.float16 or not wpk.is_cuda or wpk.numel() != f16_packed_weight_halves(F16_CHANNELS, F16_CHANNELS * n_src):
        raise RuntimeError("larvanet_amd: wpk is not the fp16 image of a %s conv" % what)


def _chk_flag(flag):
    if not isinstance(flag, torch.Tensor) or not flag.is_cuda or flag.dtype != torch.int32 or flag.numel() < 1:
        raise RuntimeError("larvanet_amd: the overflow flag must be an int32 device tensor")
    return flag.data_ptr()


def f16_packed_weight_halves(cout, cin):
    return int(hip_lib.load().larva_f16_packed_weight_halves(cout, cin))


def f16_pack_weights(w, out=None):
    lib = hip_lib.load()
    _chk(w, "w")
    if w.dim() != 4 or tuple(w.shape[2:]) != (3, 3):
        raise RuntimeError("larvanet_amd: only [cout][cin][3][3] weights are supported")
    cout, cin = int(w.shape[0]), int(w.shape[1])
    n = f16_packed_weight_halves(cout, cin)
    if n < 0:
        raise RuntimeError("larvanet_amd: no fp16 conv for %d -> %d channels" % (cin, cout))
    if out is None:
        out = torch.empty(n, device=w.device, dtype=torch.float16)
    if out.dtype != torch.float16 or out.numel() != n or not out.is_contiguous():
        raise RuntimeError("larvanet_amd: fp16 weight image must be %d contiguous halves" % n)
    hip_lib.check(lib.larva_f16_pack_weights(w.data_ptr(), out.data_ptr(), cout, cin, _stream()), "larva_f16_pack_weights")
    return out


def f16_head(x, w, bias, flag, out=None):
    lib = hip_lib.load()
# ... 217 lines not shown
```

Baseline: 363.1 HR Mpixels/s.

## Fuse loss reduction into last exit-L1 conv batch and merge staging copies

The last batched L1 exit conv kernel now takes a ticket counter. The last workgroup to finish sums all the L1 partials into the scalar loss, so the separate loss-from-partials kernel launch is no longer needed. Partial stores become atomic relaxed stores so the last block sees coherent data, which adds an atomic, a barrier and a serial tail reduction in one wave. The two host-to-static-buffer staging copies are also merged into a single vectorized copy kernel, cutting a launch per step.

Result: slower. 359.3 HR Mpixels/s (-1.1%).

```diff
diff --git a/include/larva_hip.h b/include/larva_hip.h
--- a/include/larva_hip.h
+++ b/include/larva_hip.h
@@ -47,6 +47,13 @@
                                 const float* const* truth, float* const* out, float* const* grad,
                                 float* const* partial, float gval, int N, int cout, int H, int W, int pitch,
                                 void* stream);
+int larva_conv3x3_exit_l1_batch_finish(int njobs, const float* const* src, int n_src, int cin_per_src,
+                                       const float* const* wpk, const float* const* bias, const float* const* base,
+                                       const float* const* truth, float* const* out, float* const* grad,
+                                       float* const* partial, float gval, int N, int cout, int H, int W, int pitch,
+                                       unsigned* ticket, const float* const* terms, const int* count, const float* scale,
+                                       int n, float divisor, float* loss, float* host_cell, unsigned* dev_seq,
+                                       void* stream);
 
 int larva_strip_tile_table(int H, int W, int phase, unsigned* tab, int cap);
 int larva_conv3x3_fwd_strips(const float* const* src, int n_src, int cin_per_src, const float* wpk,
@@ -110,6 +117,8 @@
 int larva_loss_from_partials_to_host_seq(const float* const* terms, const int* count, const float* scale, int n,
                                          float divisor, float* out, float* host_cell, unsigned* dev_seq, void* stream);
 int larva_host_cell_alloc(float** cell);
+int larva_stage_batch(float* dst_in, const float* src_in, long long n_in, float* dst_truth, const float* src_truth,
+                      long long n_truth, void* stream);
 int larva_host_cell_free(float* cell);
 int larva_l1_partial_grad(const float* a, const float* b, float gvalue, float gscale, float* partial,
                           int* blocks_out, float* grad, int N, int C, int H, int W, void* stream);
diff --git a/larvanet_amd/autograd.py b/larvanet_amd/autograd.py
--- a/larvanet_amd/autograd.py
+++ b/larvanet_amd/autograd.py
@@ -442,6 +442,7 @@
         StepScope.depth += 1
         StepScope.seed_grad = self.seed_grad_value
         StepScope.early_loss = self.early_loss_value
+        FinishedLoss.pending = None
         return self
 
     def __exit__(self, exc_type, *exc):
@@ -459,6 +460,7 @@
             StepScope.depth -= 1
             StepScope.seed_grad = None
             StepScope.early_loss = False
+            FinishedLoss.pending = None
             DeferredWgrad._pending = {}
             DualChain.enabled = DualChain.lazy_fwd = DualChain.lazy_bwd = False
             DeferredWgrad.active = False
@@ -765,16 +767,26 @@
                         for i in range(M)]
         outs, parts, third = [None] * M, [None] * M, [None] * M
         fused = ctx.have_dyl
+        ticket = None
+        if fused and StepScope.early_loss and StepScope.depth > 0 and M == int(divisor) and M <= 8:
+            ticket = K.loss_ticket(truth.device, create=not torch.cuda.is_current_stream_capturing())
+        scale = 1.0 / float(truth.numel())
         if fused:
             i = 0
             while i < M and fused:
                 n = 3 if M - i == 5 else min(4, M - i)
+                finish = None
+                if ticket is not None and i + n == M:
+                    finish = {"ticket": ticket, "earlier": parts[:i], "scale": scale, "divisor": float(M),
+                              "cell": StepScope.early_loss if isinstance(StepScope.early_loss, K.HostCell) else None}
                 res = K.conv3x3_exit_l1_batch(shuffle_jobs[i:i + n], c2, truth, StepScope.seed_grad, ctx.gscale,
-                                              [i + k == M - 1 for k in range(n)]) if n > 1 else None
+                                              [i + k == M - 1 for k in range(n)], finish=finish) if n > 1 else None
                 if res is None:
                     fused = False
                 else:
-                    outs[i:i + n], parts[i:i + n], third[i:i + n] = res
+                    outs[i:i + n], parts[i:i + n], third[i:i + n] = res[:3]
+                    if finish is not None:
+                        FinishedLoss.pending = (tuple(parts), scale, float(M), res[3])
                     i += n
         if not fused:
             outs = _conv_group(shuffle_jobs, c2, shuffle=True)
@@ -830,6 +842,24 @@
         return (None, None, None, None) + tuple(dfeas) + tuple(grads)
 
 
+class FinishedLoss:
+
+    pending = None
+
+    @classmethod
+    def take(cls, tensors, scales):
+        job, cls.pending = cls.pending, None
+        if job is None:
+            return None
+        parts, scale, divisor, loss = job
+        same = (len(parts) == len(tensors) and float(len(tensors)) == divisor
+                and all(t.data_ptr() == p.data_ptr() and t.numel() == p.numel() for t, p in zip(tensors, parts))
+                and all(float(s) == scale for s in scales))
+        if not same:
+            raise RuntimeError("larvanet_amd: the exits finished a loss that is not the mean the step asks for")
+        return loss
+
+
 class LossTerm:
 
     __slots__ = ("tensor", "scale", "prescaled")
@@ -850,6 +880,9 @@
             out = torch.empty((), device=ts[0].device, dtype=torch.float32)
             DeferredWgrad.pending_loss = (ts, scales, float(len(ts)), out)
             return out
+        done = FinishedLoss.take(ts, scales)
+        if done is not None:
+            return done
         cell = StepScope.early_loss if isinstance(StepScope.early_loss, K.HostCell) else None
         if len(ts) <= 8:
             return K.loss_from_partials(ts, scales, float(len(ts)), host_cell=cell)
diff --git a/larvanet_amd/captured_step.py b/larvanet_amd/captured_step.py
--- a/larvanet_amd/captured_step.py
+++ b/larvanet_amd/captured_step.py
@@ -2,6 +2,7 @@
 
 import torch
 
+from . import kernels as K
 from .autograd import DeferredWgrad, DualChain
 
 
@@ -37,6 +38,8 @@
                 DeferredWgrad.flush_late()
         torch.cuda.current_stream().wait_stream(side)
         plugin._zero_grad()
+        if mode:
+            K.loss_ticket(x.device)
         graph = torch.cuda.CUDAGraph()
         back = torch.cuda.CUDAGraph() if mode == "split" else None
         with contextlib.ExitStack() as capturing:
@@ -59,9 +62,12 @@
         self.loss, self.out, self.early_lo = loss, out, early_lo
 
     def stage(self, input_tensor, truth_tensor):
-        for dst, src in ((self.static_in, input_tensor), (self.static_truth, truth_tensor)):
-            if src.data_ptr() != dst.data_ptr():
-                dst.copy_(src)
+        pairs = [(dst, src) for dst, src in ((self.static_in, input_tensor), (self.static_truth, truth_tensor))
+                 if src.data_ptr() != dst.data_ptr()]
+        if len(pairs) == 2 and K.stage_batch(self.static_in, input_tensor, self.static_truth, truth_tensor):
+            return
+        for dst, src in pairs:
+            dst.copy_(src)
 
     def replay(self):
         if self.mode == "poll":
diff --git a/larvanet_amd/csrc/conv3x3_mfma.hip b/larvanet_amd/csrc/conv3x3_mfma.hip
--- a/larvanet_amd/csrc/conv3x3_mfma.hip
+++ b/larvanet_amd/csrc/conv3x3_mfma.hip
@@ -1,5 +1,6 @@
 #include "larva_common.h"
 #include "larva_bicubic.h"
+#include "larva_loss.h"
 #include <hip/hip_ext.h>
 #include <cstdlib>
 #include <type_traits>
@@ -396,7 +397,7 @@
   y0 = ty * G::ROWS;
 }
 
-template <int COUT, typename G, bool VEC, int EPI, int NCT, int PG0, int NPG, bool PERSIST = false>
+template <int COUT, typename G, bool VEC, int EPI, int NCT, int PG0, int NPG, bool PERSIST = false, bool FINISH = false>
 __device__ __forceinline__ void run_role(const ConvArgs& a, float* smem, int ct0, int wave, int n, int y0, int x0, int tid) {
   using C = ConvCfg<COUT, G>;
   static_assert(!VEC || C::LOADER, "the 16-byte path runs with a loader wave (2 * PIECES <= 63 for every instantiated shape)");
@@ -630,7 +631,10 @@
       }
 #pragma unroll
     for (int o = 32; o > 0; o >>= 1) s += __shfl_xor(s, o);
-    if (lane == 0) a.partial[4 * blockIdx.x + wave] = s;
+    if (lane == 0) {
+      if constexpr (FINISH) __hip_atomic_store(&a.partial[4 * blockIdx.x + wave], s, __ATOMIC_RELAXED, __HIP_MEMORY_SCOPE_AGENT);
+      else a.partial[4 * blockIdx.x + wave] = s;
+    }
   } else if constexpr (EPI == kEpiShuffle || EPI == kEpiShuffleBase) {
     const int HH = 4 * k.H, WW = 4 * k.W;
 #pragma unroll
@@ -733,8 +737,31 @@
                "s"(a.tab16[0]), "s"(a.tab16[16]));
 }
 
-template <int COUT, bool VEC, int EPI, typename G = GeoWide>
-__device__ __forceinline__ void conv_tile(const ConvArgs& a, float* smem) {
+struct LossFinish {
+  unsigned* ticket;
+  TermList terms;
+  float divisor;
+  float* out;
+  float* host_cell;
+  unsigned* dev_seq;
+};
+
+__device__ __forceinline__ void exit_loss_finish(const LossFinish& f, int wave) {
+  asm volatile("s_waitcnt vmcnt(0)" ::: "memory");
+  __builtin_amdgcn_s_barrier();
+  if (wave != 0) return;
+  unsigned t = 0u;
+  if ((threadIdx.x & 63) == 0) t = __hip_atomic_fetch_add(f.ticket, 1u, __ATOMIC_RELAXED, __HIP_MEMORY_SCOPE_AGENT);
+  t = (unsigned)__builtin_amdgcn_readfirstlane((int)t);
+  if (t != gridDim.x * gridDim.y - 1u) return;
+  __builtin_amdgcn_fence(__ATOMIC_ACQUIRE, "agent");
+  loss_terms_wave(f.terms, f.divisor, f.out, f.host_cell, f.dev_seq);
+  if ((threadIdx.x & 63) == 0) __hip_atomic_store(f.ticket, 0u, __ATOMIC_RELAXED, __HIP_MEMORY_SCOPE_AGENT);
+}
+
+template <int COUT, bool VEC, int EPI, typename G = GeoWide, bool FINISH = false>
+__device__ __forceinline__ void conv_tile(const ConvArgs& a, float* smem, const LossFinish* fin = nullptr) {
+  static_assert(!FINISH || (VEC && EPI == kEpiShuffleL1 && COUT == 48 && G::ROWS == 3), "the loss finish rides on the batched L1 exits");
   if constexpr ((LARVA_DIAG & 8) != 0) return;
   stamp(0);
   fetch_args(a);
@@ -751,6 +778,7 @@
   if constexpr (VEC) {
     if (wave == 4) {
       if constexpr (!(LARVA_DIAG & 2)) run_loader<COUT, G>(a, smem, tid & 63, n, y0, x0);
+      if constexpr (FINISH) exit_loss_finish(*fin, wave);
       return;
     }
   }
@@ -764,8 +792,9 @@
       else run_role<COUT, G, VEC, EPI, 1, 6, 6>(a, smem, wave - 2, wave, n, y0, x0, tid);
     }
   } else if constexpr (COUT == 48) {
-    if (wave < 3) run_role<COUT, G, VEC, EPI, 1, 0, 7>(a, smem, wave, wave, n, y0, x0, tid);
-    else run_role<COUT, G, VEC, EPI, 3, 7, 2>(a, smem, 0, wave, n, y0, x0, tid);
+    if (wave < 3) run_role<COUT, G, VEC, EPI, 1, 0, 7, false, FINISH>(a, smem, wave, wave, n, y0, x0, tid);
+    else run_role<COUT, G, VEC, EPI, 3, 7, 2, false, FINISH>(a, smem, 0, wave, n, y0, x0, tid);
+    if constexpr (FINISH) exit_loss_finish(*fin, wave);
   } else if constexpr (COUT == 32) {
     if (wave < 2) run_role<COUT, G, VEC, EPI, 1, 0, 5>(a, smem, wave, wave, n, y0, x0, tid);
     else run_role<COUT, G, VEC, EPI, 1, 5, 4>(a, smem, wave - 2, wave, n, y0, x0, tid);
@@ -919,6 +948,15 @@
 __global__ __launch_bounds__(ConvCfg<COUT>::THREADS_DMA, kWgPerCu) void conv3x3_mfma_batch_kernel(ConvBatch b) {
   extern __shared__ __attribute__((aligned(16))) float smem[];
   conv_tile<COUT, true, EPI>(b.job[blockIdx.y], smem);
+}
+
+struct ExitFinishBatch {
+  ConvBatch b;
+  LossFinish f;
+};
+__global__ __launch_bounds__(ConvCfg<48>::THREADS_DMA, kWgPerCu) void conv3x3_exit_l1_finish_kernel(ExitFinishBatch e) {
+  extern __shared__ __attribute__((aligned(16))) float smem[];
+  conv_tile<48, true, kEpiShuffleL1, GeoWide, true>(e.b.job[blockIdx.y], smem, &e.f);
 }
 
 constexpr int kMaxPackJobs = 64;
@@ -1343,15 +1381,15 @@
   return 4 * N * ((pitch + kTileCols - 1) / kTileCols) * ((H + kTileRows - 1) / kTileRows);
 }
 
-int larva_conv3x3_exit_l1_batch(int njobs, const float* const* src, int n_src, int cin_per_src,
-                                const float* const* wpk, const float* const* bias, const float* const* base,
-                                const float* const* truth, float* const* out, float* const* grad,
-                                float* const* partial, float gval, int N, int cout, int H, int W, int pitch,
-                                void* stream) {
-  if (njobs < 2 || njobs > kMaxConvJobs || !src || !wpk || !base || !truth || !out || !grad || !partial)
+static int exit_l1_batch(int min_jobs, int njobs, const float* const* src, int n_src, int cin_per_src,
+                         const float* const* wpk, const float* const* bias, const float* const* base,
+                         const float* const* truth, float* const* out, float* const* grad, float* const* partial,
+                         float gval, int N, int cout, int H, int W, int pitch, const LossFinish* fin, void* stream) {
+  if (njobs < min_jobs || njobs > kMaxConvJobs || !src || !wpk || !base || !truth || !out || !grad || !partial)
     return (int)hipErrorInvalidValue;
   if (cout != 48) return (int)hipErrorNotSupported;
-  ConvBatch b{};
+  ExitFinishBatch e{};
+  ConvBatch& b = e.b;
   for (int j = 0; j < njobs; ++j) {
     bool aligned;
     int epi;
@@ -1367,7 +1405,51 @@
     b.job[j].partial = partial[j];
     b.job[j].gval = gval;
   }
-  return (int)launch_batch<48>(b, njobs, kEpiShuffleL1, (hipStream_t)stream);
+  if (!fin) return (int)launch_batch<48>(b, njobs, kEpiShuffleL1, (hipStream_t)stream);
+  using C = ConvCfg<48>;
+  const ConvArgs& a = b.job[0];
+  e.f = *fin;
+  return (int)launch<conv3x3_exit_l1_finish_kernel>(dim3(a.N * a.tiles_x * a.tiles_y, njobs), dim3(C::THREADS_DMA),
+                                                    C::LDS_BYTES_DMA, (hipStream_t)stream, nullptr, e);
+}
+
+int larva_conv3x3_exit_l1_batch(int njobs, const float* const* src, int n_src, int cin_per_src,
+                                const float* const* wpk, const float* const* bias, const float* const* base,
+                                const float* const* truth, float* const* out, float* const* grad,
+                                float* const* partial, float gval, int N, int cout, int H, int W, int pitch,
+                                void* stream) {
+  return exit_l1_batch(2, njobs, src, n_src, cin_per_src, wpk, bias, base, truth, out, grad, partial, gval, N, cout, H, W,
+                       pitch, nullptr, stream);
+}
+
+int larva_conv3x3_exit_l1_batch_finish(int njobs, const float* const* src, int n_src, int cin_per_src,
+                                       const float* const* wpk, const float* const* bias, const float* const* base,
+                                       const float* const* truth, float* const* out, float* const* grad,
+                                       float* const* partial, float gval, int N, int cout, int H, int W, int pitch,
+                                       unsigned* ticket, const float* const* terms, const int* count, const float* scale,
+                                       int n, float divisor, float* loss, float* host_cell, unsigned* dev_seq,
+                                       void* stream) {
+  if (!ticket)
+    return exit_l1_batch(1, njobs, src, n_src, cin_per_src, wpk, bias, base, truth, out, grad, partial, gval, N, cout, H, W,
+                         pitch, nullptr, stream);
+  if (!terms || !count || !scale || n < 1 || n > 8 || !loss || (dev_seq && !host_cell) ||
+      (reinterpret_cast<uintptr_t>(ticket) & 3))
+    return (int)hipErrorInvalidValue;
+  LossFinish f{};
+  for (int i = 0; i < n; ++i) {
+    if (!terms[i] || count[i] < 1) return (int)hipErrorInvalidValue;
+    f.terms.p[i] = terms[i];
+    f.terms.count[i] = count[i];
+    f.terms.scale[i] = scale[i];
+  }
+  f.terms.n = n;
+  f.ticket = ticket;
+  f.divisor = divisor;
+  f.out = loss;
+  f.host_cell = host_cell;
+  f.dev_seq = dev_seq;
+  return exit_l1_batch(1, njobs, src, n_src, cin_per_src, wpk, bias, base, truth, out, grad, partial, gval, N, cout, H, W,
+                       pitch, &f, stream);
 }
 
 int larva_strip_tile_table(int H, int W, int phase, unsigned* tab, int cap) {
diff --git a/larvanet_amd/csrc/larva_loss.h b/larvanet_amd/csrc/larva_loss.h
--- a/larvanet_amd/csrc/larva_loss.h
+++ b/larvanet_amd/csrc/larva_loss.h
@@ -10,25 +10,53 @@
   int n;
 };
 
+
+template <bool COHERENT>
+__device__ __forceinline__ float loss_term_share(const TermList& l, int i, int t) {
+  float s_ = 0.f;
+  for (int k = t; k < l.count[i]; k += 256) {
+    if constexpr (COHERENT) s_ += __hip_atomic_load(l.p[i] + k, __ATOMIC_RELAXED, __HIP_MEMORY_SCOPE_AGENT);
+    else s_ += l.p[i][k];
+  }
+  return s_;
+}
+
+__device__ __forceinline__ float loss_wave_sum(float v) {
+#pragma unroll
+  for (int o = 32; o > 0; o >>= 1) v += __shfl_xor(v, o);
+  return v;
+}
+
+__device__ __forceinline__ float loss_add_term(float total, float w0, float w1, float w2, float w3, float scale) {
+  return total + ((w0 + w1) + (w2 + w3)) * scale;
+}
+
+__device__ __forceinline__ unsigned long long loss_cell_seq(const float* host_cell, const unsigned* dev_seq) {
+  if (dev_seq) return dev_seq[0];
+  return __hip_atomic_load(reinterpret_cast<const unsigned long long*>(host_cell), __ATOMIC_RELAXED, __HIP_MEMORY_SCOPE_SYSTEM) >> 32;
+}
+
+__device__ __forceinline__ void loss_store(float total, float divisor, float* __restrict__ out, float* __restrict__ host_cell,
+                                           unsigned* __restrict__ dev_seq, unsigned long long seq) {
+  const float v = total / divisor;
+  out[0] = v;
+  if (host_cell) {
+    if (dev_seq) dev_seq[0] = (unsigned)(seq + 1ull);
+    __hip_atomic_store(reinterpret_cast<unsigned long long*>(host_cell),
+                       ((seq + 1ull) << 32) | (unsigned long long)__float_as_uint(v), __ATOMIC_RELAXED,
+                       __HIP_MEMORY_SCOPE_SYSTEM);
+  }
+}
+
 __device__ __forceinline__ void loss_terms_block(const TermList& l, float divisor, float* __restrict__ out,
                                                  float* __restrict__ host_cell = nullptr, unsigned* __restrict__ dev_seq = nullptr) {
   unsigned long long seq = 0ull;
-  if (host_cell && threadIdx.x == 0) {
-    if (dev_seq) seq = dev_seq[0];
-    else seq = __hip_atomic_load(reinterpret_cast<unsigned long long*>(host_cell), __ATOMIC_RELAXED, __HIP_MEMORY_SCOPE_SYSTEM) >> 32;
-  }
+  if (host_cell && threadIdx.x == 0) seq = loss_cell_seq(host_cell, dev_seq);
   float sv[8];
 #pragma unroll
-  for (int i = 0; i < 8; ++i) {
-    float s_ = 0.f;
-    if (i < l.n)
-      for (int k = threadIdx.x; k < l.count[i]; k += 256) s_ += l.p[i][k];
-    sv[i] = s_;
-  }
+  for (int i = 0; i < 8; ++i) sv[i] = i < l.n ? loss_term_share<false>(l, i, threadIdx.x) : 0.f;
 #pragma unroll
-  for (int i = 0; i < 8; ++i)
-#pragma unroll
-    for (int o = 32; o > 0; o >>= 1) sv[i] += __shfl_xor(sv[i], o);
+  for (int i = 0; i < 8; ++i) sv[i] = loss_wave_sum(sv[i]);
   __shared__ float wsa[8][4];
   if ((threadIdx.x & 63) == 0) {
 #pragma unroll
@@ -36,17 +64,28 @@
   }
   __syncthreads();
   float total = 0.f;
-  for (int i = 0; i < l.n; ++i) total += ((wsa[i][0] + wsa[i][1]) + (wsa[i][2] + wsa[i][3])) * l.scale[i];
-  if (threadIdx.x == 0) {
-    const float v = total / divisor;
-    out[0] = v;
-    if (host_cell) {
-      if (dev_seq) dev_seq[0] = (unsigned)(seq + 1ull);
-      __hip_atomic_store(reinterpret_cast<unsigned long long*>(host_cell),
-                         ((seq + 1ull) << 32) | (unsigned long long)__float_as_uint(v), __ATOMIC_RELAXED,
-                         __HIP_MEMORY_SCOPE_SYSTEM);
-    }
+  for (int i = 0; i < l.n; ++i) total = loss_add_term(total, wsa[i][0], wsa[i][1], wsa[i][2], wsa[i][3], l.scale[i]);
+  if (threadIdx.x == 0) loss_store(total, divisor, out, host_cell, dev_seq, seq);
+}
+
+__device__ __forceinline__ void loss_terms_wave(const TermList& l, float divisor, float* __restrict__ out,
+                                                float* __restrict__ host_cell = nullptr, unsigned* __restrict__ dev_seq = nullptr) {
+  const int lane = threadIdx.x & 63;
+  unsigned long long seq = 0ull;
+  if (host_cell && lane == 0) seq = loss_cell_seq(host_cell, dev_seq);
+  float sv[8][4];
+#pragma unroll
+  for (int i = 0; i < 8; ++i)
+#pragma unroll
+    for (int w = 0; w < 4; ++w) sv[i][w] = i < l.n ? loss_term_share<true>(l, i, 64 * w + lane) : 0.f;
+  float total = 0.f;
+#pragma unroll
+  for (int i = 0; i < 8; ++i) {
+#pragma unroll
+    for (int w = 0; w < 4; ++w) sv[i][w] = loss_wave_sum(sv[i][w]);
+    if (i < l.n) total = loss_add_term(total, sv[i][0], sv[i][1], sv[i][2], sv[i][3], l.scale[i]);
   }
+  if (lane == 0) loss_store(total, divisor, out, host_cell, dev_seq, seq);
 }
 
 }
diff --git a/larvanet_amd/csrc/larva_pointwise.hip b/larvanet_amd/csrc/larva_pointwise.hip
--- a/larvanet_amd/csrc/larva_pointwise.hip
+++ b/larvanet_amd/csrc/larva_pointwise.hip
@@ -577,6 +577,22 @@
   }
 }
 
+struct StagePart {
+  float* dst;
+  const float* src;
+  long long n;
+};
+__global__ __launch_bounds__(256) void stage_batch_kernel(StagePart a, StagePart b, int blocks_a) {
+  const bool first = (int)blockIdx.x < blocks_a;
+  const StagePart p = first ? a : b;
+  const long long nthr = 256ll * (first ? blocks_a : (int)gridDim.x - blocks_a);
+  const long long t = 256ll * (first ? (int)blockIdx.x : (int)blockIdx.x - blocks_a) + threadIdx.x;
+  const long long nv = p.n >> 2;
+  for (long long i = t; i < nv; i += nthr)
+    reinterpret_cast<f32x4*>(p.dst)[i] = reinterpret_cast<const f32x4*>(p.src)[i];
+  for (long long k = 4 * nv + t; k < p.n; k += nthr) p.dst[k] = p.src[k];
+}
+
 static inline bool u8_vec_ok(const void* a, const void* b, long long HW) {
   return HW % 4 == 0 && ((reinterpret_cast<uintptr_t>(a) | reinterpret_cast<uintptr_t>(b)) & 15u) == 0;
 }
@@ -690,6 +706,24 @@
   return (int)hipGetLastError();
 }
 
+int larva_stage_batch(float* dst_in, const float* src_in, long long n_in, float* dst_truth, const float* src_truth,
+                      long long n_truth, void* stream) {
+  if (!dst_in || !src_in || !dst_truth || !src_truth || n_in < 0 || n_truth < 0) return (int)hipErrorInvalidValue;
+  if ((reinterpret_cast<uintptr_t>(dst_in) | reinterpret_cast<uintptr_t>(src_in) | reinterpret_cast<uintptr_t>(dst_truth) |
+       reinterpret_cast<uintptr_t>(src_truth)) & 15)
+    return (int)hipErrorInvalidValue;
+  StagePart a{dst_in, src_in, src_in == dst_in ? 0 : n_in}, b{dst_truth, src_truth, src_truth == dst_truth ? 0 : n_truth};
+  if (a.n + b.n == 0) return 0;
+  const long long va = (a.n + 3) / 4, vb = (b.n + 3) / 4;
+  const int blocks = grid_for(va + vb, 256) < 2 ? 2 : grid_for(va + vb, 256);
+  int blocks_a = (int)((va * blocks + (va + vb) / 2) / (va + vb));
+  if (a.n > 0 && blocks_a < 1) blocks_a = 1;
+  if (b.n > 0 && blocks_a > blocks - 1) blocks_a = blocks - 1;
+  if (a.n == 0) blocks_a = 0;
+  hipLaunchKernelGGL(stage_batch_kernel, dim3(blocks), dim3(256), 0, (hipStream_t)stream, a, b, blocks_a);
+  return (int)hipGetLastError();
+}
+
 int larva_loss_from_partials_to_host_seq(const float* const* terms, const int* count, const float* scale, int n,
                                          float divisor, float* out, float* host_cell, unsigned* dev_seq, void* stream) {
   if (!terms || !count || !scale || n < 1 || n > 8 || !out || (dev_seq && !host_cell)) return (int)hipErrorInvalidValue;
diff --git a/larvanet_amd/hip_lib.py b/larvanet_amd/hip_lib.py
--- a/larvanet_amd/hip_lib.py
+++ b/larvanet_amd/hip_lib.py
@@ -45,6 +45,14 @@
     "larva_conv3x3_exit_l1_batch": (ctypes.c_int, [ctypes.c_int, _c_pp, ctypes.c_int, ctypes.c_int, _c_pp, _c_pp, _c_pp, _c_pp,
                                                    _c_pp, _c_pp, _c_pp, ctypes.c_float, ctypes.c_int, ctypes.c_int,
                                                    ctypes.c_int, ctypes.c_int, ctypes.c_int, ctypes.c_void_p]),
+    "larva_conv3x3_exit_l1_batch_finish": (ctypes.c_int, [ctypes.c_int, _c_pp, ctypes.c_int, ctypes.c_int, _c_pp, _c_pp, _c_pp,
+                                                          _c_pp, _c_pp, _c_pp, _c_pp, ctypes.c_float, ctypes.c_int,
+                                                          ctypes.c_int, ctypes.c_int, ctypes.c_int, ctypes.c_int,
+                                                          ctypes.c_void_p, _c_pp, _c_int_p, _c_float_p, ctypes.c_int,
+                                                          ctypes.c_float, _c_float_p, _c_float_p, ctypes.c_void_p,
+                                                          ctypes.c_void_p]),
+    "larva_stage_batch": (ctypes.c_int, [_c_float_p, _c_float_p, ctypes.c_longlong, _c_float_p, _c_float_p,
+                                         ctypes.c_longlong, ctypes.c_void_p]),
     "larva_strip_tile_table": (ctypes.c_int, [ctypes.c_int, ctypes.c_int, ctypes.c_int, ctypes.POINTER(ctypes.c_uint),
                                               ctypes.c_int]),
     "larva_wgrad_partial_floats": (ctypes.c_longlong, [ctypes.c_int, ctypes.c_int, ctypes.c_int]),
diff --git a/larvanet_amd/kernels.py b/larvanet_amd/kernels.py
--- a/larvanet_amd/kernels.py
+++ b/larvanet_amd/kernels.py
@@ -237,9 +237,20 @@
     return out
 
 
-def conv3x3_exit_l1_batch(jobs, cout, truth, gvalue, gscale, want_image):
-    lib = hip_lib.load()
-    if not 2 <= len(jobs) <= 4 or cout != 48:
+_LOSS_TICKETS = {}
+
+
+def loss_ticket(device, create=True):
+    key = torch.device(device).index if torch.device(device).index is not None else torch.cuda.current_device()
+    t = _LOSS_TICKETS.get(key)
+    if t is None and create:
+        t = _LOSS_TICKETS[key] = torch.zeros(4, dtype=torch.int32, device=device)
+    return t
+
+
+def conv3x3_exit_l1_batch(jobs, cout, truth, gvalue, gscale, want_image, finish=None):
+    lib = hip_lib.load()
+    if not (1 if finish is not None else 2) <= len(jobs) <= 4 or cout != 48:
         return None
     norm = [dict(j, srcs=[j["srcs"]] if isinstance(j["srcs"], torch.Tensor) else list(j["srcs"])) for j in jobs]
     n_src = len(norm[0]["srcs"])
@@ -261,16 +272,30 @@
         outs.append(torch.empty(hr, device=truth.device, dtype=torch.float32) if want else None)
         grads.append(torch.empty((N, cout, H, P), device=truth.device, dtype=torch.float32))
         parts.append(torch.empty(npart, device=truth.device, dtype=torch.float32))
-    code = lib.larva_conv3x3_exit_l1_batch(
-        len(norm), hip_lib.ptr_array(src_ptrs), n_src, cps, hip_lib.ptr_array([j["wpk"].data_ptr() for j in norm]),
-        hip_lib.ptr_array([j["bias"].data_ptr() for j in norm]), hip_lib.ptr_array([j["base"].data_ptr() for j in norm]),
-        hip_lib.ptr_array([truth.data_ptr()] * len(norm)), hip_lib.ptr_array([None if o is None else o.data_ptr() for o in outs]),
-        hip_lib.ptr_array([g.data_ptr() for g in grads]), hip_lib.ptr_array([p.data_ptr() for p in parts]),
-        gval, N, cout, H, P, P, _stream())
+    args = (len(norm), hip_lib.ptr_array(src_ptrs), n_src, cps, hip_lib.ptr_array([j["wpk"].data_ptr() for j in norm]),
+            hip_lib.ptr_array([j["bias"].data_ptr() for j in norm]), hip_lib.ptr_array([j["base"].data_ptr() for j in norm]),
+            hip_lib.ptr_array([truth.data_ptr()] * len(norm)), hip_lib.ptr_array([None if o is None else o.data_ptr() for o in outs]),
+            hip_lib.ptr_array([g.data_ptr() for g in grads]), hip_lib.ptr_array([p.data_ptr() for p in parts]),
+            gval, N, cout, H, P, P)
+    if finish is None:
+        code = lib.larva_conv3x3_exit_l1_batch(*args, _stream())
+        if code == 801:
+            return None
+        hip_lib.check(code, "larva_conv3x3_exit_l1_batch")
+        return outs, parts, grads
+    terms = list(finish["earlier"]) + parts
+    if not 1 <= len(terms) <= 8:
+        raise RuntimeError("larvanet_amd: 1..8 loss terms")
+    cell = finish.get("cell")
+    loss = torch.empty((), device=truth.device, dtype=torch.float32)
+    code = lib.larva_conv3x3_exit_l1_batch_finish(
+        *args, finish["ticket"].data_ptr(), *_loss_terms(terms, [finish["scale"]] * len(terms)), len(terms),
+        float(finish["divisor"]), loss.data_ptr(), cell.ptr if cell is not None else None,
+        cell.dev_seq.data_ptr() if cell is not None and cell.dev_seq is not None else None, _stream())
     if code == 801:
         return None
-    hip_lib.check(code, "larva_conv3x3_exit_l1_batch")
-    return outs, parts, grads
+    hip_lib.check(code, "larva_conv3x3_exit_l1_batch_finish")
+    return outs, parts, grads, loss
 
 
 def wgrad_partial_floats(cout, cin, splits):
@@ -657,6 +682,17 @@
     return out
 
 
+def stage_batch(dst_in, src_in, dst_truth, src_truth):
+    for d, s in ((dst_in, src_in), (dst_truth, src_truth)):
+        if (tuple(d.shape) != tuple(s.shape) or d.dtype != torch.float32 or s.dtype != torch.float32
+                or not d.is_contiguous() or not s.is_contiguous() or d.device != s.device or not d.is_cuda
+                or (d.data_ptr() | s.data_ptr()) & 15):
+            return False
+    hip_lib.check(hip_lib.load().larva_stage_batch(dst_in.data_ptr(), src_in.data_ptr(), dst_in.numel(), dst_truth.data_ptr(),
+                                                   src_truth.data_ptr(), dst_truth.numel(), _stream()), "larva_stage_batch")
+    return True
+
+
 def l1_bwd_unshuffle4(a, b, gout, gscale=1.0):
     lib = hip_lib.load()
     _chk(a, "a")
```
